# CuzImSlymi/Apertis-LLM

Hardware: AMD Instinct MI355X
Metric: train tokens/sec/node (seq=4096) (higher is better)
Workload: dtype bf16

## Files before the change

apertis_llm_amd/_lib.py:

```python
import ctypes
import os
import threading

_HERE = os.path.dirname(os.path.abspath(__file__))
LIB_PATH = os.environ.get("APERTIS_HIP_LIB") or os.path.join(_HERE, "libapertis_hip.so")

F32, BF16 = 0, 1
ACT_NONE, ACT_GELU, ACT_RELU, ACT_SILU = 0, 1, 2, 3
ACT_SAVE_GRAD, ACT_MUL_SAVED = 0x100, 0x200
ACT_INTERLEAVED = 0x400


class ApertisHipError(RuntimeError):
    pass


_lock = threading.Lock()
_lib = None

_vp, _i64, _i32, _f32, _u64 = ctypes.c_void_p, ctypes.c_int64, ctypes.c_int, ctypes.c_float, ctypes.c_uint64
_f64 = ctypes.c_double

ABI_VERSION = (4 << 16) | 12
SIGNATURES = {
    "apertis_abi_version": (ctypes.c_int, []),
    "apertis_arch": (ctypes.c_char_p, []),
    "apertis_strerror": (ctypes.c_char_p, [_i32]),
    "apertis_scan_chunk_len": (_i64, [_i64, _i64, _i64]),
    "apertis_scan_num_chunks": (_i64, [_i64, _i64, _i64]),
    "apertis_selective_scan_fwd": (_i32, [_vp, _vp, _vp, _i64, _vp, _i64, _vp, _vp, _i64, _vp, _vp, _vp,
                                          _i64, _i64, _i64, _i64, _i32, _i32, _i32, _vp]),
    "apertis_selective_scan_bwd": (_i32, [_vp, _vp, _vp, _i64, _vp, _i64, _vp, _i64, _vp, _vp, _i64, _vp, _i64,
                                          _vp, _vp, _vp, _vp, _vp, _i64, _i64, _i64, _i64, _i32, _i32, _i32, _vp]),
    "apertis_ssm_gate_fwd": (_i32, [_vp, _i64, _vp, _i64, _vp, _i64, _vp, _vp, _i64, _i64, _i64, _i32, _i32, _vp]),
    "apertis_ssm_gate_bwd": (_i32, [_vp, _i64, _vp, _i64, _vp, _i64, _vp, _i64, _vp, _vp, _i64, _vp, _i64, _vp, _i64,
                                    _vp, _vp, _i64, _i64, _i32, _i32, _vp]),
    "apertis_ssm_gate_bwd_blocks": (_i64, [_i64, _i64]),
    "apertis_scan_gate_workspace_bytes": (_i64, [_i64, _i64, _i64]),
    "apertis_scan_gate_chunk_len": (_i64, []),
    "apertis_scan_gate_fwd": (_i32, [_vp, _vp, _vp, _i64, _vp, _i64, _vp, _i64, _vp, _i64, _vp, _vp, _vp, _i64, _vp, _vp, _vp,
                                     _vp, ctypes.c_uint32, _i64, _i64, _i64, _i64, _i32, _i32, _i32, _vp]),
    "apertis_scan_gate_bwd": (_i32, [_vp, _vp, _vp, _i64, _vp, _i64, _vp, _i64, _vp, _i64, _vp, _vp, _i64, _vp, _vp, _i64, _vp,
                                     _i64, _i64, _vp, _i64, _vp, _i64, _vp, _vp, _vp, _vp, _vp, _vp, ctypes.c_uint32, _i64, _i64,
                                     _i64, _i64, _i32, _i32, _i32, _vp]),
    "apertis_scan_lean_fwd": (_i32, [_vp, _vp, _vp, _i64, _vp, _i64, _vp, _i64, _vp, _i64, _vp, _vp, _vp, _i64, _vp, _vp, _vp, _vp,
                                     _i64, _i64, _i64, _i64, _i32, _vp]),
    "apertis_scan_lean_fwd_dt": (_i32, [_vp, _i64, _vp, _vp, _i64, _vp, _vp, _vp, _i64, _vp, _i64, _vp, _i64, _vp, _i64, _vp, _vp, _vp,
                                        _i64, _vp, _vp, _vp, _vp, _i64, _i64, _i64, _i64, _i32, _vp]),
    "apertis_scan_lean_bwd": (_i32, [_vp, _vp, _vp, _i64, _vp, _i64, _vp, _i64, _vp, _i64, _vp, _vp, _i64, _vp, _vp, _i64, _vp, _i64,
                                     _i64, _vp, _i64, _vp, _i64, _vp, _vp, _vp, _vp, _vp, _vp, _i64, _i64, _i64, _i64, _i32, _vp]),
    "apertis_scan_lookback_workspace_bytes": (_i64, [_i64, _i64, _i64]),
    "apertis_scan_lookback_fwd": (_i32, [_vp, _vp, _vp, _i64, _vp, _i64, _vp, _i64, _vp, _i64, _vp, _vp, _vp, _i64, _vp, _vp, _vp, _vp,
                                         ctypes.c_uint32, _i64, _i64, _i64, _i64, _i32, _vp]),
    "apertis_scan_lookback_bwd": (_i32, [_vp, _vp, _vp, _i64, _vp, _i64, _vp, _i64, _vp, _i64, _vp, _vp, _i64, _vp, _vp, _i64, _vp,
                                         _i64, _i64, _vp, _i64, _vp, _i64, _vp, _vp, _vp, _vp, _vp, ctypes.c_uint32, _i64, _i64, _i64,
                                         _i64, _i32, _vp]),
    "apertis_ssm_decode_conv": (_i32, [_vp, _i64, _vp, _vp, _vp, _vp, _vp, _i64, _i64, _i64, _i32, _vp]),
    "apertis_ssm_decode_state": (_i32, [_vp, _vp, _vp, _i64, _vp, _i64, _vp, _vp, _i64, _vp, _vp, _vp, _i64, _i64, _i64, _i32,
                                        _i32, _vp]),
    "apertis_ssm_decode_state_dt": (_i32, [_vp, _i64, _vp, _vp, _i64, _vp, _vp, _i64, _vp, _i64, _vp, _vp, _i64, _vp, _vp, _vp, _i64,
                                           _i64, _i64, _i32, _i32, _vp]),
    "apertis_dropout_add_fwd": (_i32, [_vp, _vp, _vp, _i64, _f32, _u64, _i32, _i32, _vp]),
    "apertis_dropout_bwd": (_i32, [_vp, _vp, _i64, _f32, _u64, _i32, _i32, _vp]),
    "apertis_dwconv_silu_fwd": (_i32, [_vp, _i64, _vp, _vp, _vp, _i64, _i64, _i64, _i64, _i64, _i32, _vp]),
    "apertis_dwconv_silu_bwd": (_i32, [_vp, _i64, _vp, _vp, _vp, _i64, _vp, _i64, _vp, _vp, _vp, _vp, _i64, _i64, _i64,
                                       _i64, _i32, _vp]),
    "apertis_dwconv_silu_bwd2": (_i32, [_vp, _i64, _vp, _vp, _vp, _i64, _vp, _i64, _vp, _i64, _vp, _vp, _vp, _vp, _i64, _i64, _i64,
                                        _i64, _i32, _vp]),
    "apertis_dwconv_bwd_blocks": (_i64, [_i64, _i64, _i64]),
    "apertis_moe_gate_topk_fwd": (_i32, [_vp, _vp, _vp, _vp, _i64, _i64, _i64, _vp]),
    "apertis_decode_pre_conv": (_i32, [_vp, _vp, _vp, _vp, _i64, _i64, _i64, _i64, _i32, _vp]),
    "apertis_decode_pre_state": (_i32, [_vp, _i64, _i64, _i64, _i64, _vp, _vp, _i64, _vp, _vp, _vp, _vp, _vp, _i64, _i64, _i64, _i64,
                                        _i32, _i32, _vp]),
    "apertis_decode_dense_gemv": (_i32, [_vp, _vp, _i64, _vp, _vp, _i64, _i64, _i64, _vp]),
    "apertis_decode_post": (_i32, [_vp, _vp, _i64, _vp, _vp, _i64, _i64, _i64, _i32, _vp]),
    "apertis_decode_inproj": (_i32, [_vp, _vp, _vp, _i64, _vp, _vp, _vp, _f32, _vp, _vp, _vp, _i64, _vp, _vp, _vp, _i64, _vp, _i64, _i64, _i64,
                                     _i64, _vp]),
    "apertis_moe_enter_small": (_i32, [_vp, _vp, _vp, _vp, _f32, _vp, _vp, _vp, _vp, _f32, _vp, _vp, _vp, _vp, _vp, _vp, _vp, _vp, _vp, _vp,
                                       _vp, _vp, _f32, _vp, _vp, _vp, _i64, _i64, _i64, _i64, _i32, _i32, _vp]),
    "apertis_moe_route_small": (_i32, [_vp, _vp, _vp, _vp, _vp, _vp, _vp, _vp, _vp, _vp, _vp, _f32, _vp, _vp, _vp, _i64, _i64, _i64, _i64,
                                       _i32, _i32, _vp]),
    "apertis_moe_gate_topk_bwd": (_i32, [_vp, _vp, _vp, _vp, _vp, _i64, _i64, _i64, _vp]),
    "apertis_skinny_linear_fwd": (_i32, [_vp, _vp, _vp, _vp, _i64, _i64, _i64, _i32, _vp]),
    "apertis_skinny_linear_bwd": (_i32, [_vp, _vp, _vp, _vp, _vp, _vp, _i64, _i64, _i64, _i32, _vp]),
    "apertis_skinny_linear_bwd_blocks": (_i64, [_i64]),
    "apertis_moe_plan_workspace_bytes": (_i64, [_i64, _i64, _i64]),
    "apertis_moe_plan": (_i32, [_vp, _vp, _vp, _i64, _vp, _vp, _vp, _vp, _vp, _i64, _i64, _i64, _vp]),
    "apertis_moe_gather_ln_fwd": (_i32, [_vp, _vp, _vp, _vp, _vp, _f32, _vp, _vp, _vp, _i64, _i64, _i64, _i32, _i32, _vp]),
    "apertis_moe_gather_ln_bwd": (_i32, [_vp, _vp, _vp, _vp, _vp, _vp, _vp, _vp, _vp, _vp, _vp, _vp, _i64, _i64, _i64,
                                         _i32, _i32, _vp]),
    "apertis_moe_gather_ln_bwd_blocks": (_i64, [_i64]),
    "apertis_layernorm_fwd": (_i32, [_vp, _vp, _vp, _f32, _vp, _vp, _vp, _i64, _i64, _i32, _i32, _vp]),
    "apertis_layernorm_bwd": (_i32, [_vp, _vp, _vp, _vp, _vp, _vp, _vp, _vp, _f32, _u64, _vp, _vp, _vp, _i64, _i64, _i32, _i32, _vp]),
    "apertis_layernorm_combine_bwd": (_i32, [_vp, _vp, _vp, _vp, _vp, _vp, _vp, _f32, _u64, _vp, _vp, _vp, _vp, _vp, _vp, _vp, _vp,
                                             _i64, _i64, _i64, _i32, _i32, _vp]),
    "apertis_dropout_add_layernorm_fwd": (_i32, [_vp, _vp, _vp, _i64, _vp, _vp, _vp, _f32, _vp, _vp, _vp, _vp, _i64, _i64, _f32,
                                                 _u64, _i32, _i32, _vp]),
    "apertis_dropout_add_layernorm_router_fwd": (_i32, [_vp, _vp, _vp, _vp, _f32, _vp, _vp, _vp, _vp, _vp, _vp, _f32, _vp, _vp, _vp,
                                                        _vp, _vp, _i64, _i64, _i64, _f32, _u64, _i32, _i32, _vp]),
    "apertis_layernorm_bwd_blocks": (_i64, [_i64, _i64]),
    "apertis_moe_combine_fwd": (_i32, [_vp, _vp, _vp, _vp, _i64, _i64, _i64, _i32, _i32, _i32, _vp]),
    "apertis_moe_combine_bwd": (_i32, [_vp, _vp, _vp, _vp, _vp, _vp, _vp, _vp, _i64, _i64, _i64, _i64, _i64,
                                       _i32, _i32, _vp]),
    "apertis_grouped_gemm_nt": (_i32, [_vp, _vp, _vp, _vp, _vp, _vp, _vp, _i64, _i64, _i64, _i64, _i64, _i32, _f32, _u64,
                                       _i32, _i32, _vp]),
    "apertis_grouped_gemm_nt_saves_grad": (_i32, [_i64, _i64, _i64, _i64, _i64, _i32, _i32, _i32]),
    "apertis_grouped_gemm_nt_q": (_i32, [_vp, _vp, _vp, _vp, _vp, _vp, _vp, _i64, _i64, _i64, _i64, _i64, _i32, _f32, _u64,
                                         _i32, _i32, _vp, _vp]),
    "apertis_grouped_gemm_tn_workspace_bytes": (_i64, [_i64, _i32]),
    "apertis_grouped_gemm_tn_dense_variant": (_i32, [_i64, _i64]),
    "apertis_grouped_gemm_tn_pair": (_i32, [_vp, _vp, _vp, _vp, _i64, _i64, _vp, _vp, _vp, _vp, _i64, _i64, _vp, _i64, _i64,
                                            _vp, _i64, _i32, _vp]),
    "apertis_grouped_gemm_tn_pair_q": (_i32, [_vp, _vp, _vp, _vp, _i64, _i64, _vp, _vp, _vp, _vp, _i64, _i64, _vp, _i64, _i64,
                                              _vp, _i64, _i32, _i32, _vp]),
    "apertis_grouped_gemm_tn_q": (_i32, [_vp, _vp, _vp, _vp, _vp, _i64, _i64, _i64, _i64, _vp, _i64, _i32, _i32, _vp]),
    "apertis_cast_transpose": (_i32, [_vp, _vp, _vp, _i64, _i64, _i64, _i64, _i64, _i32, _vp]),
    "apertis_weight_prep_entry_bytes": (_i64, []),
    "apertis_weight_prep": (_i32, [_vp, _i64, _i64, _vp]),
    "apertis_grouped_gemm_tn": (_i32, [_vp, _vp, _vp, _vp, _vp, _i64, _i64, _i64, _i64, _vp, _i64, _i32, _vp]),
    "apertis_moe_gate_topk_aux_fwd": (_i32, [_vp, _vp, _vp, _vp, _vp, _vp, _vp, _i64, _i64, _i64, _f32, _f32, _vp]),
    "apertis_moe_gate_topk_aux_bwd": (_i32, [_vp, _vp, _vp, _vp, _vp, _vp, _vp, _f32, _f32, _vp, _i64, _i64, _i64, _vp]),
    "apertis_moe_gate_topk_noisy_aux_fwd": (_i32, [_vp, _vp, _f32, _u64, _vp, _vp, _vp, _vp, _vp, _vp, _i64, _i64, _i64, _f32,
                                                   _f32, _vp]),
    "apertis_moe_gate_topk_noisy_aux_bwd": (_i32, [_vp, _vp, _vp, _vp, _vp, _vp, _vp, _f32, _f32, _vp, _f32, _u64, _vp, _vp, _vp,
                                                   _i64, _i64, _i64, _vp]),
    "apertis_moe_gate_aux_blocks": (_i64, [_i64]),
    "apertis_router_fwd": (_i32, [_vp, _vp, _vp, _f32, _vp, _vp, _vp, _vp, _vp, _i64, _i64, _i64, _i32, _vp]),
    "apertis_router_bwd": (_i32, [_vp, _vp, _vp, _vp, _vp, _vp, _vp, _vp, _vp, _vp, _vp, _i64, _i64, _i64, _i32, _vp]),
    "apertis_router_bwd_rows": (_i32, [_vp, _vp, _vp, _vp, _vp, _vp, _vp, _vp, _vp, _vp, _i64, _vp, _vp, _vp, _i64, _i64, _i64,
                                       _i32, _vp]),
    "apertis_router_bwd_blocks": (_i64, [_i64]),
    "apertis_boundary_router_bwd": (_i32, [_vp, _vp, _vp, _vp, _vp, _vp, _vp, _f32, _u64, _vp, _vp, _vp, _vp, _vp, _vp, _vp, _vp, _vp,
                                           _i64, _vp, _vp, _vp, _vp, _i64, _i64, _i64, _i32, _i32, _vp]),
    "apertis_tiny_linear_fwd": (_i32, [_vp, _i64, _vp, _vp, _vp, _i64, _i64, _i64, _i32, _vp]),
    "apertis_tiny_linear_bwd": (_i32, [_vp, _i64, _vp, _vp, _vp, _i64, _vp, _vp, _i64, _i64, _i64, _i32, _vp]),
    "apertis_tiny_linear_bwd_pad": (_i32, [_vp, _i64, _vp, _vp, _vp, _i64, _vp, _vp, _i64, _i64, _i64, _i64, _i32, _vp]),
    "apertis_tiny_linear_bwd_blocks": (_i64, [_i64]),
    "apertis_cross_entropy_fwd": (_i32, [_vp, _vp, _vp, _vp, _i64, _i64, _i64, _i64, _i64, _i64, _i32, _vp]),
    "apertis_cross_entropy_bwd": (_i32, [_vp, _vp, _vp, _vp, _vp, _i64, _i64, _i64, _i64, _i64, _i64, _i32, _vp]),
    "apertis_cross_entropy_fwd_bwd": (_i32, [_vp, _vp, _vp, _vp, _vp, _vp, _i64, _i64, _i64, _i64, _i64, _i64, _i32, _vp]),
    "apertis_colsum_f32": (_i32, [_vp, _vp, _i64, _i64, _vp]),
    "apertis_act_dropout_bwd": (_i32, [_vp, _vp, _vp, _vp, _i64, _i64, _i64, _i32, _f32, _u64, _i32, _vp]),
    "apertis_opt_chunk_elems": (_i64, []),
    "apertis_grad_sumsq": (_i32, [_vp, _vp, _vp, _i64, _vp, _vp]),
    "apertis_clip_coef": (_i32, [_vp, _i64, _f32, _vp, _vp, _vp]),
    "apertis_adamw_step": (_i32, [_vp, _vp, _vp, _i64, _f64, _f64, _f64, _f64, _f64, _i64, _vp, _vp]),
    "apertis_rope_qk_fwd": (_i32, [_vp, _i64, _vp, _i64, _vp, _i64, _vp, _vp, _i64, _vp, _vp, _i64, _i64, _i64, _i32, _vp]),
    "apertis_rope_qk_bwd": (_i32, [_vp, _i64, _vp, _i64, _vp, _i64, _vp, _vp, _i64, _vp, _vp, _i64, _i64, _i64, _i32, _vp]),
    "apertis_attention_fwd": (_i32, [_vp, _i64, _vp, _i64, _vp, _i64, _vp, _vp, _i64, _vp, _i64, _i64, _i64, _i64, _f32, _u64,
                                     _i32, _vp]),
    "apertis_attention_bwd_workspace_bytes": (_i64, [_i64, _i64, _i64]),
    "apertis_attention_bwd": (_i32, [_vp, _i64, _vp, _i64, _vp, _i64, _vp, _i64, _vp, _i64, _vp, _vp, _vp, _vp, _vp, _vp, _i64,
                                     _i64, _i64, _i64, _i64, _f32, _u64, _i32, _vp]),
    "apertis_rope_kv_append": (_i32, [_vp, _i64, _vp, _i64, _vp, _i64, _vp, _vp, _i64, _i64, _vp, _i64, _vp, _i64, _i64, _vp, _i64,
                                      _i64, _i64, _i64, _i64, _i64, _i32, _vp]),
    "apertis_attention_decode_splits": (_i64, [_i64, _i64, _i64, _i64]),
    "apertis_attention_decode_workspace_bytes": (_i64, [_i64, _i64, _i64, _i64]),
    "apertis_attention_decode": (_i32, [_vp, _i64, _vp, _i64, _i64, _vp, _i64, _i64, _i64, _vp, _i64, _vp, _i64, _vp, _i64, _i64,
                                        _i64, _i64, _i64, _i32, _vp]),
    "apertis_rope_kv_append_at": (_i32, [_vp, _i64, _vp, _i64, _vp, _i64, _vp, _vp, _i64, _vp, _i64, _vp, _vp, _i64, _vp, _i64, _i64,
                                         _vp, _i64, _i64, _i64, _i64, _i64, _i32, _vp]),
    "apertis_attention_decode_at": (_i32, [_vp, _i64, _vp, _i64, _i64, _vp, _i64, _i64, _i64, _vp, _vp, _i64, _vp, _i64, _vp, _i64,
                                           _i64, _i64, _i64, _i32, _vp]),
    "apertis_rope_kv_append_chunk": (_i32, [_vp, _i64, _i64, _vp, _i64, _i64, _vp, _i64, _i64, _vp, _vp, _i64, _i64, _vp, _vp, _i64,
                                            _i64, _vp, _i64, _i64, _i64, _i64, _i64, _i64, _i64, _i32, _vp]),
    "apertis_attention_chunk_splits": (_i64, [_i64, _i64, _i64, _i64, _i64]),
    "apertis_attention_chunk_workspace_bytes": (_i64, [_i64, _i64, _i64, _i64, _i64]),
    "apertis_attention_chunk": (_i32, [_vp, _i64, _vp, _i64, _i64, _vp, _i64, _i64, _i64, _vp, _i64, _vp, _i64, _vp, _i64, _i64,
                                       _i64, _i64, _i64, _i64, _i32, _vp]),
    "apertis_token_counts": (_i32, [_vp, _i64, _i64, _i64, _i64, _vp, _vp, _vp]),
    "apertis_sample_next": (_i32, [_vp, _i64, _i32, _i64, _i64, _vp, _f32, _i32, _f32, _i64, _f32, _u64, _vp, _i64, _vp, _vp, _vp,
                                   _i64, _i64, _vp, _vp, _i64, _i64, _vp, _vp, _vp, _vp, _vp]),
}


class _Lib:

    def __init__(self, cdll):
        self._cdll = cdll

    def __getattr__(self, name):
        if name not in SIGNATURES:
            raise AttributeError(name)
        try:
            fn = getattr(self._cdll, name)
        except AttributeError:
            raise ApertisHipError(f"{LIB_PATH} does not export {name}: rebuild with "
                                  "`python -m apertis_llm_amd.build --force`") from None
        fn.restype, fn.argtypes = SIGNATURES[name]
        setattr(self, name, fn)
        return fn


def load():
    global _lib
    if _lib is not None:
        return _lib
    with _lock:
        if _lib is not None:
            return _lib
        if not os.path.exists(LIB_PATH):
            raise ApertisHipError(
                f"{LIB_PATH} not found: build it with `python -m apertis_llm_amd.build` "
                "(hipcc --offload-arch=gfx950). There is no CPU or eager fallback.")
        cdll = ctypes.CDLL(LIB_PATH)
        try:
            got = int(cdll.apertis_abi_version())
        except AttributeError:
            got = -1
        if got != ABI_VERSION:
            raise ApertisHipError(f"{LIB_PATH} has ABI version {got >> 16}.{got & 0xffff} but this binding needs "
                                  f"{ABI_VERSION >> 16}.{ABI_VERSION & 0xffff}: rebuild with `python -m apertis_llm_amd.build --force`")
        _lib = _Lib(cdll)
    return _lib


def check(rc, what):
    if rc != 0:
        msg = load().apertis_strerror(int(rc)).decode()
        raise ApertisHipError(f"{what} failed: {msg} (code {rc})")


def ptr(t):
    return None if t is None else t.data_ptr()


_raw_stream = None


def stream_ptr():
    global _raw_stream
    if _raw_stream is None:
        import torch
        get_dev, get_raw = getattr(torch._C, "_cuda_getDevice", None), getattr(torch._C, "_cuda_getCurrentRawStream", None)
        if get_dev is not None and get_raw is not None:
            _raw_stream = lambda: get_raw(get_dev())
        else:
            _raw_stream = lambda: torch.cuda.current_stream().cuda_stream
    return _raw_stream()


def dtype_code(t):
    import torch
    if t.dtype == torch.float32:
        return F32
    if t.dtype == torch.bfloat16:
        return BF16
    raise ApertisHipError(f"unsupported dtype {t.dtype}: kernels take float32 or bfloat16")
```

apertis_llm_amd/csrc/layernorm.hip:

```cpp
#include "row_common.h"

namespace {

template <typename TX, typename TO, int IT>
__global__ void __launch_bounds__(256)
gather_ln_fwd_k(const TX *__restrict__ x, const int32_t *__restrict__ row_token,
                const int32_t *__restrict__ offsets, const float *__restrict__ gamma,
                const float *__restrict__ beta, float eps, TO *__restrict__ xg,
                float *__restrict__ mean_o, float *__restrict__ rstd_o, int64_t max_rows, int H, int E) {
  if constexpr (IT <= 4) __builtin_assume(H > 256 * (IT - 1));
  const int lane = threadIdx.x & 63;
  const int64_t r = (int64_t)blockIdx.x * 4 + (threadIdx.x >> 6);
  if (r >= max_rows || (offsets && r >= offsets[E])) return;
  const int e = offsets ? expert_of_row(offsets, E, (int)r) : 0;
  const TX *src = x + (row_token ? (int64_t)row_token[r] : r) * H;
  float4 v[IT];
#pragma unroll
  for (int i = 0; i < IT; ++i) {
    int c = (lane + 64 * i) * 4;
    v[i] = c < H ? load4s<TX>(src + c) : make_float4(0.f, 0.f, 0.f, 0.f);
  }
  float mean, rstd;
  row_stats<IT>(v, lane, H, eps, mean, rstd);
  const float *ga = gamma + (int64_t)e * H, *be = beta + (int64_t)e * H;
// ... 511 lines not shown
    g4[i] = c < H ? load4<float>(gamma + c) : make_float4(0, 0, 0, 0);
    b4[i] = c < H ? load4<float>(beta + c) : make_float4(0, 0, 0, 0);
  }
  __syncthreads();
  typedef typename raw4<TX>::type raw_t;
  raw_t cur[IT], nxt[IT];
  auto fetch = [&](raw_t (&o)[IT], int64_t r) {
#pragma unroll
    for (int i = 0; i < IT; ++i) {
      const int c = (lane + 64 * i) * 4;
      o[i] = (c < H && r < T) ? raw_load(x + r * H + c) : raw_t{};
    }
  };
  if (wave < T) fetch(cur, wave);
  for (int64_t r = wave; r < T; r += nw) {
    fetch(nxt, r + nw);
    float4 v[IT];
#pragma unroll
    for (int i = 0; i < IT; ++i) {
      v[i] = raw_to_f4(cur[i]);
    }
    float mean, rstd;
    row_stats<IT>(v, lane, H, eps, mean, rstd);
#pragma unroll
    for (int i = 0; i < IT; ++i) cur[i] = nxt[i];
#pragma unroll
    for (int i = 0; i < IT; ++i)
      v[i] = make_float4((v[i].x - mean) * rstd * g4[i].x + b4[i].x, (v[i].y - mean) * rstd * g4[i].y + b4[i].y,
                         (v[i].z - mean) * rstd * g4[i].z + b4[i].z, (v[i].w - mean) * rstd * g4[i].w + b4[i].w);
    float acc[NN];
#pragma unroll
    for (int n = 0; n < NN; ++n) {
      float a = 0.f;
#pragma unroll
      for (int i = 0; i < IT; ++i) {
        const float4 wn = lane + 64 * i < Q ? sW[n * Q + lane + 64 * i] : make_float4(0, 0, 0, 0);
        a += (v[i].x * wn.x + v[i].y * wn.y) + (v[i].z * wn.z + v[i].w * wn.w);
      }
      acc[n] = wave_sum(a);
    }
    if (lane < NN) {
      float o = 0.f;
#pragma unroll
      for (int n = 0; n < NN; ++n) if (lane == n) o = acc[n];
      logits[r * NN + lane] = o + (b ? b[lane] : 0.f);
    }
    if (lane == 0) { mean_o[r] = mean; rstd_o[r] = rstd; }
  }
}

template <typename TX, typename TO, int IT, int NN>
__global__ void __launch_bounds__(256)
dropadd_ln_router_fwd_k(const TO *__restrict__ blk, const TX *__restrict__ res, const float *__restrict__ gamma,
                        const float *__restrict__ beta, float eps, TX *__restrict__ y, TO *__restrict__ xn,
                        float *__restrict__ mean_o, float *__restrict__ rstd_o, const float *__restrict__ rgamma,
                        const float *__restrict__ rbeta, float reps, const float *__restrict__ W, const float *__restrict__ rb,
                        float *__restrict__ logits, float *__restrict__ rmean_o, float *__restrict__ rrstd_o, int64_t T, int H,
                        float drop_p, uint64_t seed) {
  if constexpr (IT <= 4) __builtin_assume(H > 256 * (IT - 1));
  extern __shared__ __attribute__((aligned(16))) char smem[];
  const int Q = H / 4;
  float4 *sW = reinterpret_cast<float4 *>(smem);
  float4 *sG = sW + NN * Q, *sB = sG + Q, *sRG = sB + Q, *sRB = sRG + Q;
  const int lane = threadIdx.x & 63;
  for (int i = threadIdx.x; i < NN * Q; i += 256) sW[i] = reinterpret_cast<const float4 *>(W)[i];
  for (int i = threadIdx.x; i < Q; i += 256) {
    sG[i] = reinterpret_cast<const float4 *>(gamma)[i]; sB[i] = reinterpret_cast<const float4 *>(beta)[i];
    sRG[i] = reinterpret_cast<const float4 *>(rgamma)[i]; sRB[i] = reinterpret_cast<const float4 *>(rbeta)[i];
  }
  __syncthreads();
  const float ks = drop_p > 0.f ? 1.f / (1.f - drop_p) : 1.f;
  const uint32_t th = (uint32_t)(drop_p * 65536.f);
  typedef typename raw4<TO>::type rawo_t;
  typedef typename raw4<TX>::type rawx_t;
  const int64_t wave = (int64_t)blockIdx.x * 4 + (threadIdx.x >> 6), nw = (int64_t)gridDim.x * 4;
  rawo_t bc[IT], bn[IT];
  rawx_t rc[IT], rn[IT];
  auto fetch = [&](rawo_t (&bo)[IT], rawx_t (&ro)[IT], int64_t r) {
#pragma unroll
    for (int i = 0; i < IT; ++i) {
      const int c = (lane + 64 * i) * 4;
      const bool ok = c < H && r < T;
      bo[i] = ok ? *reinterpret_cast<const rawo_t *>(blk + r * H + c) : rawo_t{};
      ro[i] = ok ? *reinterpret_cast<const rawx_t *>(res + r * H + c) : rawx_t{};
    }
  };
  if (wave < T) fetch(bc, rc, wave);
  for (int64_t r = wave; r < T; r += nw) {
    fetch(bn, rn, r + nw);
    float4 v[IT];
#pragma unroll
    for (int i = 0; i < IT; ++i) {
      const int c = (lane + 64 * i) * 4;
      if (c < H) {
        const float4 a = raw_to_f4(bc[i]), rr = raw_to_f4(rc[i]);
        float e[4] = {a.x, a.y, a.z, a.w};
        if (drop_p > 0.f) {
          bool keep[4];
          drop_keep4(seed, (uint64_t)r * (uint64_t)H + (uint64_t)c, th, keep);
#pragma unroll
          for (int j = 0; j < 4; ++j) e[j] = keep[j] ? e[j] * ks : 0.f;
        }
        v[i] = make_float4(rr.x + e[0], rr.y + e[1], rr.z + e[2], rr.w + e[3]);
        store4<TX>(y + r * H + c, v[i]);
        v[i] = make_float4(to_f32(from_f32<TX>(v[i].x)), to_f32(from_f32<TX>(v[i].y)), to_f32(from_f32<TX>(v[i].z)), to_f32(from_f32<TX>(v[i].w)));
      } else {
        v[i] = make_float4(0.f, 0.f, 0.f, 0.f);
      }
    }
    float mean, rstd;
    row_stats<IT>(v, lane, H, eps, mean, rstd);
#pragma unroll
    for (int i = 0; i < IT; ++i) {
      const int c = (lane + 64 * i) * 4;
      if (c < H) {
        const float4 g4 = sG[lane + 64 * i], b4 = sB[lane + 64 * i];
        const float4 o = make_float4((v[i].x - mean) * rstd * g4.x + b4.x, (v[i].y - mean) * rstd * g4.y + b4.y,
                                     (v[i].z - mean) * rstd * g4.z + b4.z, (v[i].w - mean) * rstd * g4.w + b4.w);
        store4<TO>(xn + r * H + c, o);
        v[i] = make_float4(to_f32(from_f32<TO>(o.x)), to_f32(from_f32<TO>(o.y)), to_f32(from_f32<TO>(o.z)), to_f32(from_f32<TO>(o.w)));
      }
    }
    if (lane == 0) { mean_o[r] = mean; rstd_o[r] = rstd; }
    float rmean, rrstd;
    row_stats<IT>(v, lane, H, reps, rmean, rrstd);
#pragma unroll
    for (int i = 0; i < IT; ++i) {
      const bool in = lane + 64 * i < Q;
      const float4 g4 = in ? sRG[lane + 64 * i] : make_float4(0, 0, 0, 0), b4 = in ? sRB[lane + 64 * i] : make_float4(0, 0, 0, 0);
      v[i] = make_float4((v[i].x - rmean) * rrstd * g4.x + b4.x, (v[i].y - rmean) * rrstd * g4.y + b4.y,
                         (v[i].z - rmean) * rrstd * g4.z + b4.z, (v[i].w - rmean) * rrstd * g4.w + b4.w);
    }
    float acc[NN];
#pragma unroll
    for (int n = 0; n < NN; ++n) {
      float a = 0.f;
#pragma unroll
      for (int i = 0; i < IT; ++i) {
        const float4 wn = lane + 64 * i < Q ? sW[n * Q + lane + 64 * i] : make_float4(0, 0, 0, 0);
        a += (v[i].x * wn.x + v[i].y * wn.y) + (v[i].z * wn.z + v[i].w * wn.w);
      }
      acc[n] = wave_sum(a);
    }
    if (lane < NN) {
      float o = 0.f;
#pragma unroll
      for (int n = 0; n < NN; ++n) if (lane == n) o = acc[n];
      logits[r * NN + lane] = o + (rb ? rb[lane] : 0.f);
    }
    if (lane == 0) { rmean_o[r] = rmean; rrstd_o[r] = rrstd; }
#pragma unroll
    for (int i = 0; i < IT; ++i) { bc[i] = bn[i]; rc[i] = rn[i]; }
  }
}

typedef float v2f __attribute__((ext_vector_type(2)));
__device__ __forceinline__ v2f pk_fma2(v2f a, v2f b, v2f c) { return __builtin_elementwise_fma(a, b, c); }

template <typename TX, int IT, int NN, int MODE>
__global__ void __launch_bounds__(256, MODE == 1 ? 2 : 1)
router_bwd3_k(const TX *__restrict__ x, const float *__restrict__ gamma, const float *__restrict__ beta,
              const float *__restrict__ mean_i, const float *__restrict__ rstd_i, const float *__restrict__ W,
              const float *__restrict__ dlogits, const TX *__restrict__ dres, const TX *__restrict__ grows,
              const int32_t *__restrict__ slot_of, int KS, TX *__restrict__ dx,
              float *__restrict__ part, int64_t T, int H) {
  if constexpr (IT <= 4) __builtin_assume(H > 256 * (IT - 1));
  typedef typename raw4<TX>::type raw_t;
  extern __shared__ __attribute__((aligned(16))) char smem[];
  float4 *sW = reinterpret_cast<float4 *>(smem);
  float4 *red = sW + NN * (H / 4);
  __shared__ float redb[4][SK_MAXN];
  const int lane = threadIdx.x & 63, wv = threadIdx.x >> 6, Q = H / 4;
  for (int i = threadIdx.x; i < NN * Q; i += 256) sW[i] = reinterpret_cast<const float4 *>(W)[i];
  float4 aw[NN][IT], ag[IT], ab[IT], g4[IT], b4[IT];
  float abias = 0.f;
#pragma unroll
  for (int i = 0; i < IT; ++i) {
    const int c = (lane + 64 * i) * 4;
    g4[i] = c < H ? load4<float>(gamma + c) : make_float4(0, 0, 0, 0);
    b4[i] = c < H ? load4<float>(beta + c) : make_float4(0, 0, 0, 0);
    ag[i] = make_float4(0, 0, 0, 0); ab[i] = make_float4(0, 0, 0, 0);
#pragma unroll
    for (int n = 0; n < NN; ++n) aw[n][i] = make_float4(0, 0, 0, 0);
  }
  __syncthreads();
  const int64_t wave = (int64_t)blockIdx.x * 4 + wv, nw = (int64_t)gridDim.x * 4;
  raw_t xc[IT], rc[IT], xn_[IT], rn_[IT];
  raw_t gc[2][IT], gn_[2][IT];
  int sc[2] = {-1, -1}, sn[2] = {-1, -1};
  const bool gath = MODE != 2 && grows != nullptr;
  auto fetch_slots = [&](int64_t r) -> int { return (gath && r < T && lane < KS) ? slot_of[r * KS + lane] : -1; };
  auto slots_of = [&](int v, int (&so)[2]) {
    so[0] = __builtin_amdgcn_readlane(v, 0);
    so[1] = __builtin_amdgcn_readlane(v, 1);
  };
  int slv_n = -1, slv_n2 = -1;
  auto fetch = [&](raw_t (&xo)[IT], raw_t (&ro)[IT], raw_t (&go)[2][IT], const int (&so)[2], int64_t r) {
#pragma unroll
    for (int i = 0; i < IT; ++i) {
      const int c = (lane + 64 * i) * 4;
      const bool ok = c < H && r < T;
      xo[i] = ok ? raw_load(x + r * H + c) : raw_t{};
      ro[i] = (MODE != 2 && ok && dres) ? raw_load(dres + r * H + c) : raw_t{};
#pragma unroll
      for (int k = 0; k < 2; ++k)
        go[k][i] = (gath && ok && so[k] >= 0) ? raw_load(grows + (int64_t)so[k] * H + c) : raw_t{};
    }
  };
  auto fetch_meta = [&](int64_t r) -> float {
    if (r >= T) return 0.f;
    const float *p = lane < NN ? dlogits + r * NN + lane : (lane == NN ? mean_i + r : rstd_i + r);
    return lane < NN + 2 ? *p : 0.f;
  };
  auto lane_val = [](float v, int l) { return __builtin_bit_cast(float, __builtin_amdgcn_readlane(__builtin_bit_cast(int, v), l)); };
  float meta = 0.f, meta_next = 0.f;
  if (wave < T) {
    slots_of(fetch_slots(wave), sc);
    slv_n = fetch_slots(wave + nw);
    fetch(xc, rc, gc, sc, wave);
    meta = fetch_meta(wave);
  }
  for (int64_t r = wave; r < T; r += nw) {
    slv_n2 = fetch_slots(r + 2 * nw);
    slots_of(slv_n, sn);
    fetch(xn_, rn_, gn_, sn, r + nw);
    meta_next = fetch_meta(r + nw);
    float g[NN];
#pragma unroll
    for (int n = 0; n < NN; ++n) g[n] = lane_val(meta, n);
    if (MODE != 1 && lane < NN) abias += meta;
    const float mean = lane_val(meta, NN), rstd = lane_val(meta, NN + 1);
    float4 xh[IT], dn[IT];
    float s1 = 0.f, s2 = 0.f;
#pragma unroll
    for (int i = 0; i < IT; ++i) {
      const bool in = lane + 64 * i < Q;
      const float4 xv = raw_to_f4(xc[i]);
      const v2f mm = {-mean, -mean}, rs = {rstd, rstd};
      v2f xh0 = in ? ((v2f){xv.x, xv.y} + mm) * rs : (v2f){0.f, 0.f}, xh1 = in ? ((v2f){xv.z, xv.w} + mm) * rs : (v2f){0.f, 0.f};
      xh[i] = make_float4(xh0.x, xh0.y, xh1.x, xh1.y);
      const v2f g0 = {g4[i].x, g4[i].y}, g1 = {g4[i].z, g4[i].w};
      const v2f xn0 = pk_fma2(xh0, g0, (v2f){b4[i].x, b4[i].y}), xn1 = pk_fma2(xh1, g1, (v2f){b4[i].z, b4[i].w});
      v2f d0 = {0.f, 0.f}, d1 = {0.f, 0.f};
#pragma unroll
      for (int n = 0; n < NN; ++n) {
        const float4 wn = in ? sW[n * Q + lane + 64 * i] : make_float4(0, 0, 0, 0);
        const v2f gn = {g[n], g[n]};
        if constexpr (MODE != 2) { d0 = pk_fma2(gn, (v2f){wn.x, wn.y}, d0); d1 = pk_fma2(gn, (v2f){wn.z, wn.w}, d1); }
        if constexpr (MODE != 1) {
          v2f a0 = {aw[n][i].x, aw[n][i].y}, a1 = {aw[n][i].z, aw[n][i].w};
          a0 = pk_fma2(gn, xn0, a0); a1 = pk_fma2(gn, xn1, a1);
          aw[n][i] = make_float4(a0.x, a0.y, a1.x, a1.y);
        }
      }
      if constexpr (MODE == 2) continue;
      v2f ag0 = pk_fma2(d0, xh0, (v2f){ag[i].x, ag[i].y}), ag1 = pk_fma2(d1, xh1, (v2f){ag[i].z, ag[i].w});
      ag[i] = make_float4(ag0.x, ag0.y, ag1.x, ag1.y);
      const v2f ab0 = (v2f){ab[i].x, ab[i].y} + d0, ab1 = (v2f){ab[i].z, ab[i].w} + d1;
      ab[i] = make_float4(ab0.x, ab0.y, ab1.x, ab1.y);
      const v2f dn0 = d0 * g0, dn1 = d1 * g1;
      dn[i] = make_float4(dn0.x, dn0.y, dn1.x, dn1.y);
      s1 += (dn[i].x + dn[i].y) + (dn[i].z + dn[i].w);
      s2 += (dn[i].x * xh[i].x + dn[i].y * xh[i].y) + (dn[i].z * xh[i].z + dn[i].w * xh[i].w);
    }
    if constexpr (MODE != 2) {
    const float m1 = wave_sum(s1) * inv_h(H), m2 = wave_sum(s2) * inv_h(H);
#pragma unroll
    for (int i = 0; i < IT; ++i) {
      const int c = (lane + 64 * i) * 4;
      if (c < H) {
        float4 rr = raw_to_f4(rc[i]);
        if (gath) {
          float4 ga = make_float4(0, 0, 0, 0);
#pragma unroll
          for (int k = 0; k < 2; ++k)
            if (sc[k] >= 0) { const float4 gv = raw_to_f4(gc[k][i]); ga.x += gv.x; ga.y += gv.y; ga.z += gv.z; ga.w += gv.w; }
          rr.x += to_f32(from_f32<TX>(ga.x)); rr.y += to_f32(from_f32<TX>(ga.y));
          rr.z += to_f32(from_f32<TX>(ga.z)); rr.w += to_f32(from_f32<TX>(ga.w));
        }
        store4<TX>(dx + r * H + c, make_float4(rstd * (dn[i].x - m1 - xh[i].x * m2) + rr.x, rstd * (dn[i].y - m1 - xh[i].y * m2) + rr.y,
                                                rstd * (dn[i].z - m1 - xh[i].z * m2) + rr.z, rstd * (dn[i].w - m1 - xh[i].w * m2) + rr.w));
      }
    }
    }
#pragma unroll
    for (int i = 0; i < IT; ++i) { xc[i] = xn_[i]; rc[i] = rn_[i]; gc[0][i] = gn_[0][i]; gc[1][i] = gn_[1][i]; }
    sc[0] = sn[0]; sc[1] = sn[1];
    slv_n = slv_n2;
    meta = meta_next;
  }
  if (MODE != 1 && lane < NN) redb[wv][lane] = abias;
  for (int turn = 1; turn < 4; ++turn) {
    __syncthreads();
    if (wv == turn) {
#pragma unroll
      for (int i = 0; i < IT; ++i) {
        const int cq = lane + 64 * i;
        if (cq < Q) {
          if constexpr (MODE != 1) {
#pragma unroll
            for (int n = 0; n < NN; ++n) red[n * Q + cq] = aw[n][i];
          }
          if constexpr (MODE != 2) { red[NN * Q + cq] = ag[i]; red[(NN + 1) * Q + cq] = ab[i]; }
        }
      }
    }
// ... 711 lines not shown
  const size_t lds3 = (size_t)(2 * N + 2) * H * sizeof(float);
  const bool split = N * ((H + 255) / 256) >= 16;
  if (dtype_x == APERTIS_BF16) {
#define ROUTER_BWD(TXT, MODE_) { launch_lds(router_bwd3_k<TXT, IT, NN, MODE_>, grid, block, lds3, st, (const TXT *)x, gamma, beta, mean, rstd, W, dlogits, (const TXT *)dres, (const TXT *)grows, slot_of, (int)KS, (TXT *)dx, part, T, (int)H); }
    SKINNY_N(N, SKINNY_IT(H, { if (split) { ROUTER_BWD(bf16_t, 1) ROUTER_BWD(bf16_t, 2) } else ROUTER_BWD(bf16_t, 0) }));
  } else if (dtype_x == APERTIS_F32) {
    SKINNY_N(N, SKINNY_IT(H, { if (split) { ROUTER_BWD(float, 1) ROUTER_BWD(float, 2) } else ROUTER_BWD(float, 0) }));
#undef ROUTER_BWD
  } else return APERTIS_ERR_ARG;
  const int64_t cols = N * H + N + 2 * H;
  hipLaunchKernelGGL(fold_rows_k, dim3((unsigned)ceil_div64(cols, 64)), dim3(1024), 0, st, part, grads, nblk, cols);
  return apertis_check_launch();
}

extern "C" int apertis_router_bwd(const void *x, const float *gamma, const float *beta, const float *mean, const float *rstd,
                                  const float *W, const float *dlogits, const void *dres, void *dx, float *part,
                                  float *grads, int64_t T, int64_t H, int64_t N, int dtype_x, void *stream) {
  return apertis_router_bwd_rows(x, gamma, beta, mean, rstd, W, dlogits, dres, nullptr, nullptr, 0, dx, part, grads, T, H, N,
                                 dtype_x, stream);
}

extern "C" int apertis_decode_inproj(const void *blk, const int32_t *slot_of, const float *wk, int64_t KK, const float *res,
                                     const float *gamma, const float *beta, float eps, float *y, const void *xn, const void *W,
                                     int64_t ldw, void *xz, const float *pre, void *conv_state, int64_t kconv, void *gated,
                                     int64_t S, int64_t H, int64_t N, int64_t Dn, void *stream) {
  if (!W) return APERTIS_ERR_ARG;
  if (xn ? false : (!blk || !res || !gamma || !beta || !y || (slot_of && (!wk || KK < 1)))) return APERTIS_ERR_ARG;
  if (pre ? (!conv_state || !gated || N != 2 * Dn || Dn < 1) : !xz) return APERTIS_ERR_ARG;
  if (S < 1 || S > 16 || H < 512 || H % 8 || H > 1024 || N < 4 || N % 4 || ldw < H || ldw % 8) return APERTIS_ERR_UNSUPPORTED;
  if (pre && (kconv < 2 || kconv > 16)) return APERTIS_ERR_UNSUPPORTED;
  hipStream_t st = (hipStream_t)stream;
  dim3 grid((unsigned)ceil_div64(N, 16)), block(256);
#define DL_GO(LN_) { launch_lds(decode_ln_inproj_k<IT, LN_>, grid, block, (LN_) ? (size_t)S * H * 2 : (size_t)0, st, (const bf16_t *)blk, \
                                        slot_of, wk, (int)KK, res, gamma, beta, eps, y, (const bf16_t *)xn, (const bf16_t *)W, (int)ldw, \
                                        (bf16_t *)xz, pre, (bf16_t *)conv_state, (int)kconv, (bf16_t *)gated, (int)Dn, (int)S, (int)H, (int)N); }
  if (xn) { SKINNY_IT(H, DL_GO(false)); }
  else { SKINNY_IT(H, DL_GO(true)); }
#undef DL_GO
  return apertis_check_launch();
}

extern "C" int apertis_moe_enter_small(const void *blk, const void *res, const float *gamma, const float *beta, float eps, void *y,
                                       void *xn, const float *rgamma, const float *rbeta, float reps, const float *W,
                                       const float *rb, float *logits, float *gates, int32_t *idx, float *w,
                                       int32_t *expert_offsets, int32_t *row_token, int32_t *row_k, int32_t *slot_of,
                                       const float *lgamma, const float *lbeta, float leps, void *xg, float *mean, float *rstd,
                                       int64_t S, int64_t H, int64_t E, int64_t K, int dtype_x, int dtype_y, void *stream) {
  if (!blk || !res || !gamma || !beta || !y || !rgamma || !rbeta || !W || !logits || !gates || !idx || !w || !expert_offsets ||
      !row_token || !row_k || !slot_of || !lgamma || !lbeta || !xg || !mean || !rstd)
    return APERTIS_ERR_ARG;
  if (S < 1 || S > 16 || (E != 4 && E != 8) || K < 1 || K > E || E * K > 16) return APERTIS_ERR_UNSUPPORTED;
  if (H <= 0 || H % 4 || H > 1024) return APERTIS_ERR_UNSUPPORTED;
  if (dtype_x != APERTIS_F32 || (dtype_y != APERTIS_BF16 && dtype_y != APERTIS_F32)) return APERTIS_ERR_UNSUPPORTED;
  hipStream_t st = (hipStream_t)stream;
  dim3 grid(1), block(64 * (unsigned)(E * K));
  const size_t lds = (size_t)(3 * E + 4) * H * sizeof(float) + (size_t)S * H * (dtype_y == APERTIS_BF16 ? 2 : 4);
  if (lds + 4096 > 160 * 1024) return APERTIS_ERR_UNSUPPORTED;
#define ES_GO(TOT, NN_) { launch_lds(moe_enter_small_k<float, TOT, IT, NN_>, grid, block, lds, st, (const TOT *)blk, (const float *)res, gamma, beta, eps, (float *)y, (TOT *)xn, rgamma, rbeta, \
                       reps, W, rb, logits, gates, idx, w, expert_offsets, row_token, row_k, slot_of, lgamma, lbeta, leps, (TOT *)xg, \
                       mean, rstd, (int)S, (int)K, (int)H); }
  if (dtype_y == APERTIS_BF16) { SKINNY_IT(H, { if (E == 4) ES_GO(bf16_t, 4) else ES_GO(bf16_t, 8) }); }
  else { SKINNY_IT(H, { if (E == 4) ES_GO(float, 4) else ES_GO(float, 8) }); }
#undef ES_GO
  return apertis_check_launch();
}

extern "C" int apertis_moe_route_small(const float *logits, float *gates, int32_t *idx, float *w, int32_t *expert_offsets,
                                       int32_t *row_token, int32_t *row_k, int32_t *slot_of, const void *x, const float *gamma,
                                       const float *beta, float eps, void *xg, float *mean, float *rstd, int64_t S, int64_t H,
                                       int64_t E, int64_t K, int dtype_x, int dtype_xg, void *stream) {
  if (!logits || !gates || !idx || !w || !expert_offsets || !row_token || !row_k || !slot_of || !x || !gamma || !beta || !xg ||
      !mean || !rstd || S < 0)
    return APERTIS_ERR_ARG;
  if (S < 1 || S > 64 || (E != 4 && E != 8 && E != 16) || K < 1 || K > E || K > MAXK || E * K > 16) return APERTIS_ERR_UNSUPPORTED;
  if (check_H(H) || H > 1024) return APERTIS_ERR_UNSUPPORTED;
  hipStream_t st = (hipStream_t)stream;
  dim3 grid(1), block(64 * (unsigned)(E * K));
#define RS_GO(EC_) hipLaunchKernelGGL((moe_route_small_k<TA, TB, IT, EC_>), grid, block, 0, st, logits, gates, idx, w, expert_offsets, \
                                      row_token, row_k, slot_of, (const TA *)x, gamma, beta, eps, (TB *)xg, mean, rstd, (int)S, (int)E, \
                                      (int)K, (int)H)
  DISPATCH_2T(dtype_x, dtype_xg, SKINNY_IT(H, { if (E == 4) RS_GO(4); else if (E == 8) RS_GO(8); else RS_GO(16); }));
#undef RS_GO
  return apertis_check_launch();
}

extern "C" int apertis_boundary_router_bwd(const void *y, const float *gamma, const float *mean, const float *rstd, const void *dres,
                                           void *dx, void *dblk, float drop_p, uint64_t seed, const void *xn, const float *rgamma,
                                           const float *rbeta, const float *rmean, const float *rrstd, const float *W,
                                           const float *dlogits, const void *grows, const int32_t *slot_of, int64_t KS,
                                           float *part, float *rgrads, float *dgamma, float *dbeta, int64_t T, int64_t H,
                                           int64_t N, int dtype_x, int dtype_g, void *stream) {
  if (!y || !gamma || !mean || !rstd || !dx || !dblk || !xn || !rgamma || !rbeta || !rmean || !rrstd || !W || !dlogits || !part ||
      !rgrads || !dgamma || !dbeta || T < 0)
    return APERTIS_ERR_ARG;
  if (drop_p < 0.f || drop_p >= 1.f) return APERTIS_ERR_ARG;
  if (grows && (!slot_of || KS < 1)) return APERTIS_ERR_ARG;
  if (grows && KS > 2) return APERTIS_ERR_UNSUPPORTED;
  if (H <= 0 || H % 4 || H > 1024 || N < 1 || N > 8) return APERTIS_ERR_UNSUPPORTED;
  if (dtype_x != APERTIS_F32 || (dtype_g != APERTIS_BF16 && dtype_g != APERTIS_F32)) return APERTIS_ERR_UNSUPPORTED;
  hipStream_t st = (hipStream_t)stream;
  const int64_t nblk = apertis_router_bwd_blocks(T), cols = N * H + N + 2 * H;
  float *part_ln = part + nblk * cols;
  dim3 grid((unsigned)nblk), block(256);
  const size_t ldsf = (size_t)(N + 2 + 8 + 2) * H * sizeof(float), lds3 = (size_t)(2 * N + 2) * H * sizeof(float);
#define BR_BWD(TGT) { \
    launch_lds(boundary_router_bwd_k<float, TGT, IT, NN>, grid, block, ldsf, st, (const float *)y, gamma, mean, rstd, (const float *)dres, (float *)dx, (TGT *)dblk, drop_p, seed, \
                       (const TGT *)xn, rgamma, rbeta, rmean, rrstd, W, dlogits, (const TGT *)grows, slot_of, (int)KS, part, part_ln, T, (int)H); \
    launch_lds(router_bwd3_k<TGT, IT, NN, 2>, grid, block, lds3, st, (const TGT *)xn, rgamma, rbeta, rmean, rrstd, W, dlogits, (const TGT *)nullptr, \
                       (const TGT *)nullptr, (const int32_t *)nullptr, 0, (TGT *)nullptr, part, T, (int)H); }
  if (dtype_g == APERTIS_BF16) { SKINNY_N(N, SKINNY_IT(H, BR_BWD(bf16_t))); }
  else { SKINNY_N(N, SKINNY_IT(H, BR_BWD(float))); }
#undef BR_BWD
  hipLaunchKernelGGL(fold_rows_k, dim3((unsigned)ceil_div64(cols, 64)), dim3(1024), 0, st, part, rgrads, nblk, cols);
  ln_fold(part_ln, nblk, H, false, dgamma, dbeta, st);
  return apertis_check_launch();
}

extern "C" int apertis_dropout_add_layernorm_fwd(const void *blk, const int32_t *slot_of, const float *wk, int64_t K,
                                                 const void *res, const float *gamma, const float *beta, float eps, void *y,
                                                 void *xn, float *mean, float *rstd, int64_t T, int64_t H, float drop_p,
                                                 uint64_t seed, int dtype_x, int dtype_y, void *stream) {
  if (!blk || !res || !gamma || !beta || !y || !xn || !mean || !rstd || T < 0 || drop_p < 0.f || drop_p >= 1.f)
    return APERTIS_ERR_ARG;
  if (slot_of && (!wk || K < 1 || K > MAXK)) return APERTIS_ERR_ARG;
  if (check_H(H)) return APERTIS_ERR_UNSUPPORTED;
  if (T == 0) return APERTIS_OK;
  hipStream_t st = (hipStream_t)stream;
  dim3 grid((unsigned)ceil_div64(T, 4)), block(256);
  DISPATCH_2T(dtype_x, dtype_y, DISPATCH_IT(H, hipLaunchKernelGGL((dropadd_ln_fwd_k<TA, TB, IT>), grid, block, 0, st,
      (const TB *)blk, slot_of, wk, (int)K, (const TA *)res, gamma, beta, eps, (TA *)y, (TB *)xn, mean, rstd, T, (int)H, drop_p,
      seed)));
  return apertis_check_launch();
}

extern "C" int apertis_dropout_add_layernorm_router_fwd(const void *blk, const void *res, const float *gamma, const float *beta,
                                                        float eps, void *y, void *xn, float *mean, float *rstd,
                                                        const float *rgamma, const float *rbeta, float reps, const float *W,
                                                        const float *rb, float *logits, float *rmean, float *rrstd, int64_t T,
                                                        int64_t H, int64_t N, float drop_p, uint64_t seed, int dtype_x,
                                                        int dtype_y, void *stream) {
  if (!blk || !res || !gamma || !beta || !y || !xn || !mean || !rstd || !rgamma || !rbeta || !W || !logits || !rmean || !rrstd ||
      T < 0 || drop_p < 0.f || drop_p >= 1.f)
    return APERTIS_ERR_ARG;
  if (H <= 0 || H % 4 || H > 1024 || (N != 2 && N != 4 && N != 8)) return APERTIS_ERR_UNSUPPORTED;
  if (T == 0) return APERTIS_OK;
  hipStream_t st = (hipStream_t)stream;
  const size_t lds = (size_t)(N + 4) * H * sizeof(float);
  dim3 grid((unsigned)std::min<int64_t>(ceil_div64(T, 4), 1024)), block(256);
#define BR_GO(NN_) { launch_lds(dropadd_ln_router_fwd_k<TA, TB, IT, NN_>, grid, block, lds, st, (const TB *)blk, (const TA *)res, gamma, beta, eps, (TA *)y, (TB *)xn, mean, rstd, rgamma, rbeta, reps, W, rb, logits, rmean, rrstd, T, (int)H, drop_p, seed); }
  DISPATCH_2T(dtype_x, dtype_y, SKINNY_IT(H, { if (N == 2) BR_GO(2) else if (N == 4) BR_GO(4) else BR_GO(8) }));
#undef BR_GO
  return apertis_check_launch();
}
```

apertis_llm_amd/model.py:

```python
import functools
import inspect
import json
import logging
import math
import os
from pathlib import Path
from typing import Any, Dict, List, Optional, Tuple, Union

import torch
import torch.nn as nn
import torch.nn.functional as F

from . import ops
from .multimodal import UnifiedMultimodalEncoder

logger = logging.getLogger(__name__)


def _on_input_device(fn):
    @functools.wraps(fn)
    def wrapper(self, *args, **kwargs):
        t = next((a for a in (*args, *kwargs.values()) if isinstance(a, torch.Tensor)), None)
        if t is None or not t.is_cuda or t.device.index == torch.cuda.current_device():
            return fn(self, *args, **kwargs)
        with ops.device_guard(t):
            return fn(self, *args, **kwargs)
    return wrapper


class ApertisConfig:

    def __init__(self, vocab_size: int = 32000, hidden_size: int = 768, num_hidden_layers: int = 12,
                 num_attention_heads: int = 12, intermediate_size: int = 3072, hidden_act: str = "gelu",
                 hidden_dropout_prob: float = 0.1, attention_probs_dropout_prob: float = 0.1,
                 max_position_embeddings: int = 2048, type_vocab_size: int = 2, initializer_range: float = 0.02,
                 layer_norm_eps: float = 1e-12, pad_token_id: int = 0, bos_token_id: int = 1, eos_token_id: int = 2,
                 unk_token_id: int = 3, position_embedding_type: str = "rotary", use_cache: bool = True,
                 classifier_dropout: float = None, model_type: str = "apertis", tie_word_embeddings: bool = True,
                 rope_theta: float = 10000.0, sliding_window: Optional[int] = None,
                 attention_type: str = "standard_mha", ssm_d_inner: Optional[int] = None, ssm_d_state: int = 16,
                 ssm_dt_rank: Union[int, str] = "auto", ssm_conv_kernel: int = 4, use_flash_attention: bool = False,
                 use_expert_system: bool = False, num_experts: int = 8, experts_per_token: int = 2,
                 multimodal: bool = False, image_size: int = 224, vision_embed_dim: int = 768,
                 vision_patch_size: int = 16, vision_layers: int = 12, vision_heads: int = 12,
                 output_attentions: bool = False, output_hidden_states: bool = False,
                 load_balancing_loss_coef: float = 0.01, expert_capacity_factor: float = 1.25,
                 noisy_routing_alpha: float = 0.1, expert_dropout_prob: float = 0.1,
                 router_z_loss_coef: float = 0.001, expert_output_gating: bool = False,
                 use_noisy_top_k_routing: bool = True, use_expert_capacity_limit: bool = True,
                 use_expert_dropout: bool = True, use_router_z_loss: bool = True,
                 use_load_balancing_loss: bool = True, use_rmsnorm: bool = False, use_swiglu: bool = False,
                 **kwargs):
        given = dict(locals())
        for name in ("vocab_size", "hidden_size", "num_hidden_layers", "num_attention_heads", "hidden_act",
                     "intermediate_size", "hidden_dropout_prob", "attention_probs_dropout_prob",
                     "max_position_embeddings", "type_vocab_size", "initializer_range", "layer_norm_eps",
                     "pad_token_id", "bos_token_id", "eos_token_id", "unk_token_id", "position_embedding_type",
                     "use_cache", "classifier_dropout", "model_type", "tie_word_embeddings", "rope_theta",
                     "sliding_window", "attention_type", "ssm_d_state"):
            setattr(self, name, given[name])
        derived = num_attention_heads * ssm_d_state
        if attention_type == "selective_ssm":
            if ssm_d_inner is not None and ssm_d_inner != derived:
                logger.warning("ssm_d_inner=%s overridden by num_attention_heads*ssm_d_state=%s", ssm_d_inner, derived)
            self.ssm_d_inner = derived
        else:
            self.ssm_d_inner = 2 * hidden_size if ssm_d_inner is None else ssm_d_inner
        self.ssm_dt_rank = math.ceil(hidden_size / 16) if ssm_dt_rank == "auto" else int(ssm_dt_rank)
        for name in ("ssm_conv_kernel", "use_flash_attention", "use_expert_system", "num_experts",
                     "experts_per_token", "multimodal", "image_size", "vision_embed_dim", "vision_patch_size",
                     "vision_layers", "vision_heads", "output_attentions", "output_hidden_states",
                     "load_balancing_loss_coef", "expert_capacity_factor", "noisy_routing_alpha",
                     "expert_dropout_prob", "router_z_loss_coef", "expert_output_gating", "use_noisy_top_k_routing",
                     "use_expert_capacity_limit", "use_expert_dropout", "use_router_z_loss",
                     "use_load_balancing_loss", "use_rmsnorm", "use_swiglu"):
            setattr(self, name, given[name])
        if not use_expert_system:
            self.num_experts = 0
            self.experts_per_token = 0
        else:
            self.experts_per_token = min(num_experts, experts_per_token) if num_experts > 0 else 0
        for key, value in kwargs.items():
            if not hasattr(self, key):
                logger.warning("Ignoring unknown config parameter: %s=%s", key, value)

    @classmethod
    def from_dict(cls, config_dict: Dict[str, Any]):
        params = inspect.signature(cls.__init__).parameters
        keep = {k: v for k, v in config_dict.items() if (k in params and k != "self") or k == "kwargs"}
        if keep.get("ssm_dt_rank") == "auto":
            keep["ssm_dt_rank"] = math.ceil(keep.get("hidden_size", 768) / 16)
        return cls(**keep)

    def to_dict(self) -> Dict[str, Any]:
        return self.__dict__

    @classmethod
    def from_pretrained(cls, model_name_or_path: str):
        if os.path.isfile(model_name_or_path) and model_name_or_path.endswith(".json"):
            path = model_name_or_path
        else:
            path = os.path.join(model_name_or_path, "config.json")
            if not os.path.exists(path) and os.path.isdir(model_name_or_path):
                parent = os.path.join(Path(model_name_or_path).parent, "config.json")
                if os.path.exists(parent):
                    path = parent
        if not os.path.exists(path):
            raise FileNotFoundError(f"Config file not found. Looked for: '{path}' based on input '{model_name_or_path}'")
        with open(path, "r", encoding="utf-8") as f:
            return cls.from_dict(json.load(f))

    def save_pretrained(self, save_directory: str):
        os.makedirs(save_directory, exist_ok=True)
        with open(os.path.join(save_directory, "config.json"), "w", encoding="utf-8") as f:
            json.dump(self.to_dict(), f, indent=2)


def _activation_module(name: str) -> nn.Module:
    if name == "relu":
        return nn.ReLU()
    if name in ("silu", "swish"):
        return nn.SiLU()
    if name != "gelu":
        logger.warning("Unsupported activation %s; using GELU", name)
    return nn.GELU()


def _activation_name(name: str) -> str:
    return name if name in ("gelu", "relu", "silu", "swish") else "gelu"


def _compute_dtype(t: torch.Tensor) -> torch.dtype:
    if torch.is_autocast_enabled():
        dt = torch.get_autocast_dtype("cuda")
        return torch.bfloat16 if dt in (torch.bfloat16, torch.float16) else dt
    return t.dtype if t.dtype in (torch.float32, torch.bfloat16) else torch.float32


class HipLayerNorm(nn.LayerNorm):

    def forward(self, x):
        H = x.shape[-1]
        if x.is_cuda and H % 4 == 0 and H <= 4096 and x.dtype in (torch.float32, torch.bfloat16):
            return ops.layer_norm(x, self.weight, self.bias, self.eps, out_dtype=_compute_dtype(x))
        return super().forward(x)

    def forward_pass(self, x):
        H = x.shape[-1]
        if x.is_cuda and H % 4 == 0 and H <= 4096 and x.dtype in (torch.float32, torch.bfloat16):
            return ops.layer_norm_pass(x, self.weight, self.bias, self.eps, out_dtype=_compute_dtype(x))
        return self.forward(x), x


def _norm_pass(norm, x):
    return norm.forward_pass(x) if isinstance(norm, HipLayerNorm) else (norm(x), x)


class _LazyCombine:
    __slots__ = ("yr", "w", "plan", "shape", "dtype")

    def __init__(self, yr, w, plan, shape, dtype):
        self.yr, self.w, self.plan, self.shape, self.dtype = yr, w, plan, shape, dtype

    def materialise(self):
        return ops.moe_combine(self.yr, self.w, self.plan, out_dtype=self.dtype).reshape(self.shape)


class _StackedPast(list):

    def __init__(self, conv_all, state_all, heads, d_state):
        NL, B = conv_all.shape[0], conv_all.shape[1]
        super().__init__((conv_all[l], state_all[l].view(B, heads, d_state)) for l in range(NL))
        self.conv_all, self.state_all = conv_all, state_all
        self._offs = None

    def offsets(self, NL, B):
        if self._offs is None:
            self._offs = (torch.arange(NL + 1, device=self.conv_all.device, dtype=torch.int32) * B).contiguous()
        return self._offs


class _Pending:
    __slots__ = ("out", "res", "drop")

    def __init__(self, out, res, drop):
        self.out, self.res, self.drop = out, res, drop

    def resolve(self):
        out = self.out.materialise() if isinstance(self.out, _LazyCombine) else self.out
        return _dropout_add(self.drop, out, self.res)


def _enter_block(norm, h, router=None):
    if isinstance(h, _Pending):
        out, res = h.out, h.res
        H = res.shape[-1]
        cd = _compute_dtype(res)
        lazy = out if isinstance(out, _LazyCombine) else None
        if (isinstance(norm, HipLayerNorm) and res.is_cuda and tuple(out.shape) == tuple(res.shape) and H % 4 == 0 and
                H <= 4096 and res.dtype in (torch.float32, torch.bfloat16) and
                (res.dtype == torch.float32 or cd == res.dtype) and (lazy is None or lazy.dtype == lazy.yr.dtype == cd)):
            if (router is not None and lazy is None and isinstance(router[0], nn.LayerNorm) and H <= 1024 and
                    router[1].weight.shape[0] in (2, 4, 8) and cd in (torch.float32, torch.bfloat16)):
                rn, rl = router
                y, xn, logits = ops.dropout_add_layer_norm_router(out, res, norm.weight, norm.bias, norm.eps, h.drop.p,
                                                                  h.drop.training, rn.weight, rn.bias, rn.eps, rl.weight,
                                                                  rl.bias, out_dtype=cd)
                xn._apertis_router_logits = logits
                return xn, y
            if lazy is not None:
                y, xn = ops.dropout_add_layer_norm(lazy.yr, res, norm.weight, norm.bias, norm.eps, h.drop.p,
                                                   h.drop.training, out_dtype=cd, combine=(lazy.w, lazy.plan))
            else:
                y, xn = ops.dropout_add_layer_norm(out, res, norm.weight, norm.bias, norm.eps, h.drop.p,
                                                   h.drop.training, out_dtype=cd)
            return xn, y
        h = h.resolve()
    return _norm_pass(norm, h)


def _dropout_add(drop: nn.Dropout, out, residual):
    if out.is_cuda and out.numel() % 4 == 0 and out.shape == residual.shape and \
            out.dtype in (torch.float32, torch.bfloat16) and residual.dtype in (torch.float32, torch.bfloat16) and \
            (residual.dtype == torch.float32 or out.dtype == residual.dtype):
        return ops.dropout_add(out, residual, drop.p, drop.training)
    return drop(out) + residual


DECODE_GRAPH = os.environ.get("APERTIS_DECODE_GRAPH", "1") == "1"
DECODE_GRAPH_MIN_STEPS = 24
DECODE_PREPASS = os.environ.get("APERTIS_DECODE_PREPASS", "1") == "1"


def _mfma_linear(x, weight, bias=None):
    K = weight.shape[1]
    if x.is_cuda and K % 8 == 0 and weight.shape[0] % 8 == 0:
        return ops.linear_mfma(x, weight, bias, compute_dtype=_compute_dtype(x))
    if getattr(weight, "_apertis_prep", None) is not None:
        raise ops.ApertisHipError(f"prepared-weight placeholder {tuple(weight.shape)} on the stock linear path")
    return F.linear(x, weight, bias)


class RMSNorm(nn.Module):

    def __init__(self, hidden_size: int, eps: float = 1e-6):
        super().__init__()
        self.hidden_size, self.eps = hidden_size, eps
        self.scale = nn.Parameter(torch.ones(hidden_size))

    def forward(self, x):
        rms = x.norm(p=2, dim=-1, keepdim=True) * (self.hidden_size ** -0.5)
        return self.scale * (x / (rms + self.eps))


class RotaryEmbedding(nn.Module):

    def __init__(self, dim: int, max_position_embeddings: int = 2048, base: float = 10000):
        super().__init__()
        if dim % 2:
            raise ValueError(f"RoPE dimension must be even, got {dim}")
        self.dim, self.max_position_embeddings, self.base = dim, max_position_embeddings, base
        inv = 1.0 / (base ** (torch.arange(0, dim, 2, dtype=torch.float32) / dim))
        ang = torch.outer(torch.arange(max_position_embeddings, dtype=torch.float32), inv)
        self.register_buffer("inv_freq", inv, persistent=False)
        self.register_buffer("cos_cached", ang.cos(), persistent=False)
        self.register_buffer("sin_cached", ang.sin(), persistent=False)

    def forward(self, x, position_ids=None):
        B, L, _ = x.shape
        if position_ids is None:
            position_ids = torch.arange(L, device=x.device).unsqueeze(0)
        cos, sin = self.cos_cached[position_ids], self.sin_cached[position_ids]
        pairs = x.float().reshape(B, L, -1, 2)
        a, b = pairs[..., 0], pairs[..., 1]
        return torch.stack((a * cos - b * sin, a * sin + b * cos), dim=-1).reshape(B, L, self.dim).type_as(x)


class SelectiveLinearAttention(nn.Module):

    def __init__(self, config: ApertisConfig):
        super().__init__()
        self.hidden_size = config.hidden_size
        self.num_heads = config.num_attention_heads
        self.d_state = config.ssm_d_state
        self.d_inner = self.num_heads * self.d_state
        self.dt_rank = config.ssm_dt_rank
        self.conv_kernel_size = config.ssm_conv_kernel
        self.in_proj_x = nn.Linear(self.hidden_size, self.d_inner, bias=False)
        self.in_proj_z = nn.Linear(self.hidden_size, self.d_inner, bias=False)
        self.conv1d = nn.Conv1d(self.d_inner, self.d_inner, self.conv_kernel_size, groups=self.d_inner,
                                padding=self.conv_kernel_size - 1)
        self.x_param_proj = nn.Linear(self.d_inner, self.dt_rank + 2 * self.d_inner, bias=False)
        self.dt_proj_head = nn.Linear(self.dt_rank, self.num_heads, bias=True)
        nn.init.uniform_(self.dt_proj_head.bias, a=math.log(1e-3), b=math.log(1e-2))
        self.A_log = nn.Parameter(torch.empty(self.num_heads, self.d_state).uniform_(math.log(0.5), math.log(0.99)))
        self.D = nn.Parameter(torch.ones(self.d_inner))
        self.out_proj = nn.Linear(self.d_inner, self.hidden_size, bias=False)
        self.use_cache = False
        self._pad_idx = None
        self._inplace_cache = False
        self._decode_pre = None

    def _pad_index(self, device):
        Dn, R = self.d_inner, self.dt_rank
        Wb = -(-Dn // 64) * 64
        idx = self._pad_idx
        if idx is None or idx.device != device:
            i = torch.arange(R + 2 * Dn)
            dst = torch.where(i < R, 2 * Wb + i, torch.where(i < R + Dn, i - R, Wb + i - R - Dn))
            idx = self._pad_idx = dst.to(device)
        return idx

    def register_train_prep(self, prep):
        Dn, R = self.d_inner, self.dt_rank
        Wb, Wr = -(-Dn // 64) * 64, -(-R // 64) * 64
        prep.add_stack(("in_proj_xz", id(self)), (self.in_proj_x.weight, self.in_proj_z.weight))
        prep.add_rowmap(("x_param_padded", id(self)), self.x_param_proj.weight, self._pad_index(self.x_param_proj.weight.device),
                        2 * Wb + Wr)
        prep.add_plain(self.out_proj.weight)

    def _padded_param_weight(self):
        w, Dn, R = self.x_param_proj.weight, self.d_inner, self.dt_rank
        Wb, Wr = -(-Dn // 64) * 64, -(-R // 64) * 64
        if w.is_cuda:
            return ops.scatter_rows(w, self._pad_index(w.device), 2 * Wb + Wr), Wb, Wr
        zb = w.new_zeros(Wb - Dn, Dn)
        zr = w.new_zeros(Wr - R, Dn)
        return torch.cat([w[R:R + Dn], zb, w[R + Dn:], zb, w[:R], zr], dim=0), Wb, Wr

    def _stacked_in_proj(self):
        w_xz = ops.prepared_weight(("in_proj_xz", id(self)), (self.in_proj_x.weight, self.in_proj_z.weight))
        if w_xz is None:
            w_xz = ops.cached_prep("in_proj_xz", (self.in_proj_x.weight, self.in_proj_z.weight),
                                   lambda: torch.cat([self.in_proj_x.weight, self.in_proj_z.weight], dim=0))
        return w_xz

    def decode_finish(self, gated, past_key_value):
        self._decode_pre = None
        B = gated.shape[0]
        out = ops.decode_dense_gemv(gated, self.out_proj.weight, self.out_proj.bias)
        if out is None:
            out = _mfma_linear(gated.reshape(B, 1, self.d_inner), self.out_proj.weight, self.out_proj.bias)
        return out.reshape(B, 1, -1), None, tuple(past_key_value)

    @_on_input_device
    def forward(self, hidden_states, attention_mask=None, position_ids=None, past_key_value=None,
                output_attentions: bool = False, use_cache: bool = False):
        self.use_cache = use_cache
        B, L, _ = hidden_states.shape
        Dn, R, kw = self.d_inner, self.dt_rank, self.conv_kernel_size
        conv_prev = ssm_prev = None
        if past_key_value is not None:
            conv_prev, ssm_prev = past_key_value
        have_window = (conv_prev is not None and use_cache and conv_prev.shape[1] == Dn and conv_prev.shape[2] == kw - 1)
        if (self._decode_pre is not None and L == 1 and have_window and hidden_states.is_cuda and hidden_states.dtype == torch.bfloat16
                and not torch.is_grad_enabled() and not output_attentions):
            gated = ops.decode_inproj(self._stacked_in_proj(), self._decode_pre, conv_prev, xn=hidden_states)
            if gated is not None:
                return self.decode_finish(gated, past_key_value)
        xz = _mfma_linear(hidden_states, self._stacked_in_proj())
        if self._decode_pre is not None and not (L == 1 and have_window and ssm_prev is not None and not output_attentions
                                                  and not torch.is_grad_enabled() and hidden_states.is_cuda and kw > 1):
            self._decode_pre = None
            raise ops.ApertisHipError("SelectiveLinearAttention: the model ran this step's cache-only half ahead (_decode_prepass: the "
                                      "SSM state is already updated) but the layer is not on its single-token path")
        Wb, Wr = -(-Dn // 64) * 64, -(-R // 64) * 64
        wp = ops.prepared_weight(("x_param_padded", id(self)), (self.x_param_proj.weight,))
        if wp is None:
            wp, Wb, Wr = ops.cached_prep("x_param_padded", (self.x_param_proj.weight,), self._padded_param_weight)
        if (L == 1 and have_window and ssm_prev is not None and not output_attentions and not torch.is_grad_enabled()
                and hidden_states.is_cuda and kw > 1):
            xz2 = xz.reshape(B, 2 * Dn)
            pre, self._decode_pre = self._decode_pre, None
            if pre is not None:
                gated = ops.decode_post(pre, xz2, conv_prev)
                out = _mfma_linear(gated.reshape(B, 1, Dn), self.out_proj.weight, self.out_proj.bias)
                return out, None, (conv_prev, ssm_prev)
            xc, conv_state = ops.ssm_decode_step(xz2[:, :Dn], conv_prev, self.conv1d.weight, self.conv1d.bias,
                                                 inplace=self._inplace_cache)
            p = _mfma_linear(xc, wp)
            dt_in = p[:, 2 * Wb:2 * Wb + R]
            state = ssm_prev.reshape(B, Dn).float()
            if not (self._inplace_cache and state.data_ptr() == ssm_prev.data_ptr()):
                state = state.clone()
            if ops.tiny_linear_supported(dt_in, R, self.num_heads):
                gated = ops.ssm_decode_state_dt(dt_in, self.dt_proj_head.weight, self.dt_proj_head.bias, self.A_log, p[:, :Dn],
                                                p[:, Wb:Wb + Dn], xc, xz2[:, Dn:], self.D, state)
            else:
                dt_logits = self.dt_proj_head(dt_in).float()
                gated = ops.ssm_decode_state(dt_logits, self.A_log, p[:, :Dn], p[:, Wb:Wb + Dn], xc, xz2[:, Dn:], self.D, state)
            out = _mfma_linear(gated.reshape(B, 1, Dn), self.out_proj.weight)
            return out, None, (conv_state, state.reshape(B, self.num_heads, self.d_state))
        xp, z = ops.split_cols(xz, (Dn, Dn))
        conv_in = xp
        if have_window:
            conv_in = torch.cat([conv_prev.transpose(1, 2).to(xp.dtype), xp], dim=1)
        conv_state = conv_in[:, -(kw - 1):].transpose(1, 2).detach() if use_cache else None
        if hidden_states.is_cuda and ops.DWCONV_PAIR:
            xc_p, xc = ops.dwconv_silu_pair(conv_in, self.conv1d.weight, self.conv1d.bias)
        else:
            xc_p = xc = ops.dwconv_silu(conv_in, self.conv1d.weight, self.conv1d.bias)
        if have_window:
            xc_p, xc = xc_p[:, :L], xc[:, :L]
        p = _mfma_linear(xc_p, wp)
        Btp, Cp, dt_in = ops.split_cols(p, (Wb, Wb, R, Wr - R))[:3]
        h0 = ssm_prev.reshape(B, Dn) if (use_cache and ssm_prev is not None) else None
        two_op = output_attentions or not hidden_states.is_cuda
        tiny = ops.tiny_linear_supported(dt_in, R, self.num_heads)
        if tiny and not two_op:
            res = ops.scan_gate_dt(dt_in, self.dt_proj_head.weight, self.dt_proj_head.bias, self.A_log, Btp, Cp, xc, z, self.D,
                                   h0=h0, delta_softplus=True, return_last=use_cache)
            (gated, h_last), y = (res if use_cache else (res, None)), None
            out = _mfma_linear(gated, self.out_proj.weight)
            cache = (conv_state, h_last.reshape(B, self.num_heads, self.d_state)) if use_cache else None
            return out, None, cache
        if tiny:
            dt_logits = ops.tiny_linear(dt_in, self.dt_proj_head.weight, self.dt_proj_head.bias)
        else:
            dt_logits = self.dt_proj_head(dt_in).float()
        if two_op:
            res = ops.selective_scan(dt_logits, self.A_log, Btp[..., :Dn], Cp[..., :Dn], h0=h0,
                                     delta_softplus=True, y_dtype=torch.float32, return_last=use_cache)
            y, h_last = res if use_cache else (res, None)
            gated = ops.ssm_gate(y, xc, z, self.D)
        else:
            res = ops.scan_gate(dt_logits, self.A_log, Btp, Cp, xc, z, self.D, h0=h0, delta_softplus=True,
                                return_last=use_cache)
            (gated, h_last), y = (res if use_cache else (res, None)), None
        out = _mfma_linear(gated, self.out_proj.weight)
        cache = (conv_state, h_last.reshape(B, self.num_heads, self.d_state)) if use_cache else None
        return out, (y if output_attentions else None), cache


_ZERO_SCALARS = {}


def _zero_scalar(device, dtype):
    key = (device, dtype)
    z = _ZERO_SCALARS.get(key)
    if z is None:
        z = _ZERO_SCALARS[key] = torch.zeros((), device=device, dtype=dtype)
    return z


class AdaptiveExpertSystem(nn.Module):

    _STACKED = (("0.weight", "expert_ln_weight"), ("0.bias", "expert_ln_bias"), ("1.weight", "expert_w1"),
                ("1.bias", "expert_b1"), ("4.weight", "expert_w2"), ("4.bias", "expert_b2"))

    def register_train_prep(self, prep):
        prep.add_plain(self.expert_w1)
        prep.add_plain(self.expert_w2)

    def __init__(self, config: ApertisConfig, activation_function_override: Optional[str] = None):
        super().__init__()
        self.config = config
        self.hidden_size = config.hidden_size
        self.intermediate_size = config.intermediate_size
        self.num_experts = config.num_experts
        self.experts_per_token = config.experts_per_token
        self.load_balancing_loss_coef = config.load_balancing_loss_coef if self.num_experts > 0 else 0.0
        self.expert_capacity_factor = config.expert_capacity_factor
        self.router_z_loss_coef = config.router_z_loss_coef if self.num_experts > 0 else 0.0
        self.noisy_routing_alpha = config.noisy_routing_alpha if self.num_experts > 0 else 0.0
        self.expert_dropout_prob = config.expert_dropout_prob if self.num_experts > 0 else 0.0
        on = self.num_experts > 0
        self.use_noisy_top_k_routing = config.use_noisy_top_k_routing and on
        self.use_expert_capacity_limit = config.use_expert_capacity_limit and on
        self.use_expert_dropout = config.use_expert_dropout and on
        self.use_router_z_loss = config.use_router_z_loss and on
        self.use_load_balancing_loss = config.use_load_balancing_loss and on
        self.router = self.experts = self.w_noise = None
        if not on:
            return
        E, H, I = self.num_experts, self.hidden_size, self.intermediate_size
        self.activation = _activation_name(activation_function_override or config.hidden_act)
        self.hidden_dropout_prob = config.hidden_dropout_prob
        self.router_norm = HipLayerNorm(H, eps=config.layer_norm_eps)
        self.router = nn.Linear(H, E)
        self.experts = True
        k1, k2 = 1.0 / math.sqrt(H), 1.0 / math.sqrt(I)
        self.expert_ln_weight = nn.Parameter(torch.ones(E, H))
        self.expert_ln_bias = nn.Parameter(torch.zeros(E, H))
        self.expert_w1 = nn.Parameter(torch.empty(E, I, H).uniform_(-k1, k1))
        self.expert_b1 = nn.Parameter(torch.empty(E, I).uniform_(-k1, k1))
        self.expert_w2 = nn.Parameter(torch.empty(E, H, I).uniform_(-k2, k2))
        self.expert_b2 = nn.Parameter(torch.empty(E, H).uniform_(-k2, k2))
        if config.use_noisy_top_k_routing:
            self.w_noise = nn.Parameter(torch.zeros(E))
        self._register_state_dict_hook(self._split_experts)
        self._register_load_state_dict_pre_hook(self._stack_experts)

    @staticmethod
    def _split_experts(module, state_dict, prefix, local_metadata):
        for suffix, name in module._STACKED:
            stacked = state_dict.pop(prefix + name)
            for e in range(module.num_experts):
                state_dict[f"{prefix}experts.{e}.{suffix}"] = stacked[e]
        return state_dict

    def _stack_experts(self, state_dict, prefix, *args):
        for suffix, name in self._STACKED:
            keys = [f"{prefix}experts.{e}.{suffix}" for e in range(self.num_experts)]
            if all(k in state_dict for k in keys):
                state_dict[prefix + name] = torch.stack([state_dict.pop(k) for k in keys])

    def init_expert_weights(self, std: float):
        with torch.no_grad():
            self.expert_w1.normal_(0.0, std)
            self.expert_w2.normal_(0.0, std)
            self.expert_b1.zero_()
            self.expert_b2.zero_()
            self.expert_ln_weight.fill_(1.0)
            self.expert_ln_bias.zero_()

    @_on_input_device
    def forward(self, hidden_states, lazy_combine=False, aux_dtype=None):
        aux_dtype = aux_dtype or hidden_states.dtype
        if self.num_experts <= 0 or self.router is None:
            zero = _zero_scalar(hidden_states.device, aux_dtype)
            return hidden_states, zero, zero
        B, L, H = hidden_states.shape
        S, E, K = B * L, self.num_experts, self.experts_per_token
        xf = hidden_states.reshape(S, H)
        pre_logits = getattr(hidden_states, "_apertis_router_logits", None)
        if pre_logits is not None:
            logits = pre_logits.reshape(S, E)
            xf._apertis_rows_link = getattr(hidden_states, "_apertis_rows_link", None)
        elif ops.router_ln_linear_supported(xf, H, E):
            logits, xf = ops.router_ln_linear(xf, self.router_norm.weight, self.router_norm.bias, self.router_norm.eps,
                                              self.router.weight, self.router.bias)
        else:
            xn = self.router_norm(xf)
            if xn.is_cuda and ops.skinny_linear_supported(H, E):
                logits = ops.skinny_linear(xn, self.router.weight, self.router.bias)
            else:
                logits = self.router(xn).float()
        lb_loss = rz_loss = None
        lb_coef = self.load_balancing_loss_coef if (self.use_load_balancing_loss and self.training) else 0.0
        rz_coef = self.router_z_loss_coef if (self.use_router_z_loss and self.training) else 0.0
        noisy = self.use_noisy_top_k_routing and self.training
        cd = _compute_dtype(xf)
        if (not self.training and lb_coef == 0 and rz_coef == 0 and not noisy and logits.is_cuda
                and ops.moe_route_small_supported(logits, xf, K)):
            _g, idx, w, plan, xg = ops.moe_route_small(logits, xf, self.expert_ln_weight, self.expert_ln_bias,
                                                       self.config.layer_norm_eps, K, out_dtype=cd)
            yr = ops.expert_mlp(xg, self.expert_w1, self.expert_b1, self.expert_w2, self.expert_b2, plan.offsets,
                                plan.max_rows, act=self.activation, drop_p=0.0, seed=0, compute_dtype=cd)
            out = _LazyCombine(yr, w, plan, (B, L, H), xf.dtype)
            if not lazy_combine:
                out = out.materialise()
            zero = _zero_scalar(hidden_states.device, aux_dtype)
            return out, zero, zero
        fused_gate = logits.is_cuda and S > 0 and (lb_coef > 0 or rz_coef > 0)
        if noisy and not fused_gate:
            logits = logits + torch.randn_like(logits) * (F.softplus(self.w_noise) * self.noisy_routing_alpha)
        if fused_gate:
            nseed = int(torch.empty((), dtype=torch.int64).random_().item()) if noisy else 0
            idx, w, lb, rz = ops.moe_gate_topk_aux(logits, K, lb_coef, rz_coef, self.w_noise if noisy else None,
                                                   self.noisy_routing_alpha, nseed)
            lb_loss = lb if lb_coef > 0 else None
            rz_loss = rz if rz_coef > 0 else None
        else:
            gates, idx, w = ops.moe_gate_topk(logits, K)
            if lb_coef > 0:
                frac = torch.zeros(E, device=xf.device).index_add_(0, idx.reshape(-1).long(),
                                                                   torch.ones(S * K, device=xf.device)) / S
                lb_loss = lb_coef * E * torch.sum(frac * gates.mean(dim=0))
            if rz_coef > 0:
                rz_loss = rz_coef * torch.mean(torch.logsumexp(logits, dim=-1) ** 2)
        capacity = None
        if self.use_expert_capacity_limit and self.training:
            capacity = max(1, math.floor((S / E) * self.expert_capacity_factor)) if S > 0 else 0
        active = None
        if self.use_expert_dropout and self.training and self.expert_dropout_prob > 0:
            n_drop = min(math.floor(E * self.expert_dropout_prob), E - 1)
            if n_drop > 0:
                active = torch.ones(E, dtype=torch.bool)
                active[torch.randperm(E)[:n_drop]] = False
                active = active.to(xf.device)
        cd = _compute_dtype(xf)
        plan = ops.moe_plan(idx, w, E, capacity, active)
        xg = ops.moe_gather_ln(xf, self.expert_ln_weight, self.expert_ln_bias, plan, self.config.layer_norm_eps,
                               out_dtype=cd)
        p_drop = self.hidden_dropout_prob if self.training else 0.0
        seed = int(torch.empty((), dtype=torch.int64).random_().item()) if p_drop > 0 else 0
        yr = ops.expert_mlp(xg, self.expert_w1, self.expert_b1, self.expert_w2, self.expert_b2, plan.offsets,
                            plan.max_rows, act=self.activation, drop_p=p_drop, seed=seed,
                            compute_dtype=cd)
        out = _LazyCombine(yr, w, plan, (B, L, H), xf.dtype)
        if not lazy_combine:
            out = out.materialise()
        if lb_loss is None or rz_loss is None:
            zero = _zero_scalar(hidden_states.device, aux_dtype)
            lb_loss = zero if lb_loss is None else lb_loss
            rz_loss = zero if rz_loss is None else rz_loss
        return out, lb_loss.to(aux_dtype), rz_loss.to(aux_dtype)


class StateTrackingRecurrentCell(nn.Module):

    def __init__(self, hidden_size: int):
        super().__init__()
        raise NotImplementedError("StateTrackingRecurrentCell is dead code in the reference and is not part of "
                                  "the MI355X hot path")


class ApertisAttention(nn.Module):
    def __init__(self, config: ApertisConfig):
        super().__init__()
        self.config = config
        self.hidden_size = config.hidden_size
        self.num_attention_heads = config.num_attention_heads
        self.attention_head_size = self.hidden_size // self.num_attention_heads
        if config.attention_type in ("selective_ssm", "selective_linear"):
            self.attention_mechanism_impl = SelectiveLinearAttention(config)
            self._ssm = True
        else:
            if config.attention_type != "standard_mha":
                logger.error("Unsupported attention_type '%s'; using 'standard_mha'", config.attention_type)
                config.attention_type = "standard_mha"
            bias = config.attention_probs_dropout_prob == 0.0
            self.q_proj = nn.Linear(self.hidden_size, self.hidden_size, bias=bias)
            self.k_proj = nn.Linear(self.hidden_size, self.hidden_size, bias=bias)
            self.v_proj = nn.Linear(self.hidden_size, self.hidden_size, bias=bias)
            self.out_proj = nn.Linear(self.hidden_size, self.hidden_size, bias=bias)
            self.attention_mechanism_impl = None
            self._ssm = False
        norm = RMSNorm if config.use_rmsnorm else HipLayerNorm
        self.pre_norm = norm(config.hidden_size, eps=config.layer_norm_eps)
        self.output_dropout = nn.Dropout(config.hidden_dropout_prob)
        self.attention_dropout = nn.Dropout(config.attention_probs_dropout_prob)
        self.rope = None
        if config.position_embedding_type == "rotary" and not self._ssm:
            self.rope = RotaryEmbedding(config.hidden_size, config.max_position_embeddings, config.rope_theta)

    def _decode_entry(self, h, past_kv, use_c, output_att):
        impl = self.attention_mechanism_impl
        if (impl._decode_pre is None or not isinstance(h, _Pending) or past_kv is None or not use_c or output_att
                or not isinstance(self.pre_norm, HipLayerNorm) or torch.is_grad_enabled() or self.training):
            return None
        out, res = h.out, h.res
        if res.shape[1] != 1 or not res.is_cuda:
            return None
        lazy = out if isinstance(out, _LazyCombine) else None
        conv_prev = past_kv[0]
        if lazy is not None:
            if not (lazy.yr.dtype == torch.bfloat16 == lazy.dtype):
                return None
            bnd = (lazy.yr, res, self.pre_norm.weight, self.pre_norm.bias, self.pre_norm.eps, (lazy.w, lazy.plan))
        elif isinstance(out, torch.Tensor) and tuple(out.shape) == tuple(res.shape) and out.dtype == torch.bfloat16:
            bnd = (out, res, self.pre_norm.weight, self.pre_norm.bias, self.pre_norm.eps, None)
        else:
            return None
        if res.shape[0] > 4 or conv_prev.dim() != 3:
            return None
        r = ops.decode_inproj(impl._stacked_in_proj(), impl._decode_pre, conv_prev, boundary=bnd)
        if r is None:
            return None
        y, gated = r
        return y, impl.decode_finish(gated, past_kv)

    def _fused_ok(self, q, att_mask, past_kv, output_att):
        if not (ops.ATTN_FUSED and q.is_cuda and past_kv is None and not output_att
                and ops.attention_supported(q, self.num_attention_heads)):
            return False
        if att_mask is None:
            return True
        if not isinstance(att_mask, _AttnMask):
            return False
        kv = att_mask.key_valid
        return att_mask.fused_ok and (kv is None or tuple(kv.shape) == tuple(q.shape[:2]))

    def _fused_attention(self, q, k, v, att_mask, pos_ids, use_c):
        key_valid, default_pos = (att_mask.key_valid, att_mask.default_pos) if att_mask is not None else (None, False)
        if self.rope is not None:
            q, k = ops.rope_qk(q, k, None if default_pos else pos_ids, self.rope.cos_cached, self.rope.sin_cached)
        cache = (k, v) if use_c else None
        ctxv = ops.causal_attention(q, k, v, self.num_attention_heads, key_valid, self.attention_dropout.p, self.training)
        return self.out_proj(ctxv), cache

    def _decode_ok(self, q, att_mask, past_kv, output_att, use_c):
        step = isinstance(past_kv, ops.KVLayer) and past_kv.cache.step_active
        ok = (isinstance(past_kv, ops.KVLayer) and ops.ATTN_FUSED and ops.ATTN_DECODE_FUSED and q.is_cuda
              and q.shape[1] == 1 and use_c and not output_att and not self.training and not torch.is_grad_enabled()
              and isinstance(att_mask, _AttnMask) and att_mask.decode_ok
              and (att_mask.step_cache is past_kv.cache if step else att_mask.pos_host is not None)
              and ops.attention_decode_supported(q, self.num_attention_heads))
        if step:
            cache = past_kv.cache
            if not (ok and q.dtype == cache.dtype and q.shape[0] == cache.k[0].shape[0]):
                raise ops.ApertisHipError("a KVCache whose device step state is active takes single-token inference steps on the "
                                          "decode kernels only (its host lengths are stale): KVCache.step_state_end() first")
            return True
        if not ok:
            return False
        cache, kv = past_kv.cache, att_mask.key_valid
        n = cache.lengths[past_kv.layer]
        return (q.dtype == cache.dtype and n < cache.capacity and q.shape[0] == cache.k[0].shape[0]
                and (kv is None or tuple(kv.shape) == (q.shape[0], n + 1)))

    def _decode_attention(self, q, k, v, att_mask, past_kv):
        cache, layer = past_kv.cache, past_kv.layer
        cos, sin = (self.rope.cos_cached, self.rope.sin_cached) if self.rope is not None else (None, None)
        if cache.step_active:
            q = ops.kv_append_rope_at(q, k, v, cache, layer, cos, sin)
            ctxv = ops.attention_decode_at(q, cache, layer, self.num_attention_heads)
        else:
            q = ops.kv_append_rope(q, k, v, cache, layer, att_mask.pos_host, cos, sin)
            ctxv = ops.attention_decode(q, cache, layer, self.num_attention_heads, att_mask.key_valid)
        return self.out_proj(ctxv.unsqueeze(1)), cache

    def _chunk_ok(self, q, att_mask, past_kv, output_att, use_c):
        if not (isinstance(past_kv, ops.KVLayer) and past_kv.cache.multi_token and not past_kv.cache.step_active
                and ops.ATTN_FUSED and ops.ATTN_DECODE_FUSED and q.is_cuda and q.shape[1] > 1 and use_c and not output_att
                and not self.training and not torch.is_grad_enabled()
                and isinstance(att_mask, _AttnMask) and att_mask.decode_ok and att_mask.pos_host is not None
                and ops.attention_decode_supported(q, self.num_attention_heads)):
            return False
        cache, kv = past_kv.cache, att_mask.key_valid
        n = cache.lengths[past_kv.layer]
        return (q.dtype == cache.dtype and n + q.shape[1] <= cache.capacity and q.shape[0] == cache.k[0].shape[0]
                and att_mask.pos_host == n and (kv is None or tuple(kv.shape) == (q.shape[0], n + q.shape[1])))

    def _chunk_attention(self, q, k, v, att_mask, past_kv):
        cache, layer = past_kv.cache, past_kv.layer
        cos, sin = (self.rope.cos_cached, self.rope.sin_cached) if self.rope is not None else (None, None)
        q = ops.kv_append_rope_chunk(q, k, v, cache, layer, att_mask.pos_host, cos, sin)
        ctxv = ops.attention_chunk(q, cache, layer, self.num_attention_heads, att_mask.key_valid)
        return self.out_proj(ctxv), cache

    def _heads(self, t):
        B, L, _ = t.shape
        return t.view(B, L, self.num_attention_heads, self.attention_head_size).transpose(1, 2)

    def forward(self, hidden_s, att_mask=None, pos_ids=None, past_kv=None, output_att=False, use_c=False, defer=False):
        fused = self._decode_entry(hidden_s, past_kv, use_c, output_att) if self._ssm else None
        if fused is not None:
            hidden_s, (out, proxy, cache) = fused
        else:
            x, hidden_s = _enter_block(self.pre_norm, hidden_s)
        if fused is not None:
            pass
        elif self._ssm:
            out, proxy, cache = self.attention_mechanism_impl(x, attention_mask=att_mask, position_ids=pos_ids,
                                                              past_key_value=past_kv, output_attentions=output_att,
                                                              use_cache=use_c)
        elif self._decode_ok(q := self.q_proj(x), att_mask, past_kv, output_att, use_c):
            out, cache = self._decode_attention(q, self.k_proj(x), self.v_proj(x), att_mask, past_kv)
            proxy = None
        elif self._chunk_ok(q, att_mask, past_kv, output_att, use_c):
            out, cache = self._chunk_attention(q, self.k_proj(x), self.v_proj(x), att_mask, past_kv)
            proxy = None
        elif self._fused_ok(q, att_mask, past_kv, output_att):
            out, cache = self._fused_attention(q, self.k_proj(x), self.v_proj(x), att_mask, pos_ids, use_c)
            proxy = None
        else:
            if isinstance(att_mask, _AttnMask):
                att_mask = att_mask.additive()
            k, v = self.k_proj(x), self.v_proj(x)
            if self.rope is not None:
                q, k = self.rope(q, pos_ids), self.rope(k, pos_ids)
            if use_c and past_kv is not None:
                k, v = torch.cat([past_kv[0], k], dim=1), torch.cat([past_kv[1], v], dim=1)
            cache = (k, v) if use_c else None
            qh, kh, vh = self._heads(q), self._heads(k), self._heads(v)
            Lq, Lk = qh.shape[2], kh.shape[2]
            if att_mask is None and Lq > 1:
                i = torch.arange(Lq, device=x.device).unsqueeze(1) + (Lk - Lq)
                att_mask = torch.zeros(Lq, Lk, device=x.device, dtype=qh.dtype).masked_fill_(
                    i < torch.arange(Lk, device=x.device).unsqueeze(0), torch.finfo(qh.dtype).min)
            if output_att:
                scores = qh @ kh.transpose(-1, -2) / math.sqrt(self.attention_head_size)
                probs = F.softmax(scores + att_mask if att_mask is not None else scores, dim=-1)
                proxy = probs
                ctxv = self.attention_dropout(probs) @ vh
            else:
                proxy = None
                ctxv = F.scaled_dot_product_attention(qh, kh, vh, attn_mask=att_mask,
                                                      dropout_p=self.attention_dropout.p if self.training else 0.0)
            out = self.out_proj(ctxv.transpose(1, 2).reshape(x.shape[0], Lq, self.hidden_size))
        if defer:
            return _Pending(out, hidden_s, self.output_dropout), proxy, cache
        return _dropout_add(self.output_dropout, out, hidden_s), proxy, cache


class SwiGLUFFN(nn.Module):

    def __init__(self, config: ApertisConfig, intermediate_size: Optional[int] = None):
        super().__init__()
        self.config = config
        self.hidden_size = config.hidden_size
        self.intermediate_size = intermediate_size if intermediate_size is not None else config.intermediate_size
        self.ffn_dim = max(256, -(-int(self.intermediate_size * 2 / 3) // 256) * 256)
        self.w_gate = nn.Linear(self.hidden_size, self.ffn_dim, bias=False)
        self.w_up = nn.Linear(self.hidden_size, self.ffn_dim, bias=False)
        self.w_down = nn.Linear(self.ffn_dim, self.hidden_size, bias=False)
        self.dropout = nn.Dropout(config.hidden_dropout_prob)

    def forward(self, x):
        return self.dropout(self.w_down(F.silu(self.w_gate(x)) * self.w_up(x)))


class ApertisFeedForward(nn.Module):
    def __init__(self, config: ApertisConfig):
        super().__init__()
        self.config = config
        norm = RMSNorm if config.use_rmsnorm else HipLayerNorm
        self.pre_norm = norm(config.hidden_size, eps=config.layer_norm_eps)
        self.is_expert_system = False
        if config.use_swiglu:
            self.ffn = SwiGLUFFN(config)
        elif config.use_expert_system and config.num_experts > 0:
            self.ffn = AdaptiveExpertSystem(config, activation_function_override=config.hidden_act)
            self.is_expert_system = True
        else:
            self.ffn = nn.Sequential(nn.Linear(config.hidden_size, config.intermediate_size),
                                     _activation_module(config.hidden_act), nn.Dropout(config.hidden_dropout_prob),
                                     nn.Linear(config.intermediate_size, config.hidden_size))
        self.output_dropout = nn.Dropout(config.hidden_dropout_prob)

    def register_train_prep(self, prep):
        if isinstance(self.ffn, nn.Sequential):
            prep.add_plain(self.ffn[0].weight)
            prep.add_plain(self.ffn[3].weight)

    def _dense_ffn(self, x):
        if isinstance(self.ffn, nn.Sequential) and x.is_cuda and x.dtype in (torch.float32, torch.bfloat16):
            lin1, _act, drop, lin2 = self.ffn
            H = x.shape[-1]
            xf = x.reshape(-1, H)
            T = xf.shape[0]
            if T >= 1 and lin1.bias is not None and lin2.bias is not None:
                cd = _compute_dtype(xf)
                p_drop = drop.p if self.training else 0.0
                seed = int(torch.empty((), dtype=torch.int64).random_().item()) if p_drop > 0 else 0
                out = ops.expert_mlp(xf.to(cd), lin1.weight.unsqueeze(0), lin1.bias.unsqueeze(0), lin2.weight.unsqueeze(0),
                                     lin2.bias.unsqueeze(0), ops.dense_offsets(T, xf.device), T,
                                     act=_activation_name(self.config.hidden_act), drop_p=p_drop, seed=seed, compute_dtype=cd)
                return out.reshape(*x.shape[:-1], lin2.weight.shape[0])
        return self.ffn(x)

    def forward(self, hidden_s, defer=False):
        router = None
        if self.is_expert_system and self.ffn.router is not None and self.ffn.num_experts > 0:
            router = (self.ffn.router_norm, self.ffn.router)
            small = self._small_entry(hidden_s, defer)
            if small is not None:
                return small
        x, hidden_s = _enter_block(self.pre_norm, hidden_s, router=router)
        if self.is_expert_system:
            out, lb, rz = self.ffn(x, lazy_combine=defer and not os.environ.get("APERTIS_NO_LAZY_COMBINE"),
                                   aux_dtype=hidden_s.dtype)
        else:
            out = self._dense_ffn(x)
            lb = rz = _zero_scalar(hidden_s.device, hidden_s.dtype)
        if defer:
            return _Pending(out, hidden_s, self.output_dropout), lb, rz
        return _dropout_add(self.output_dropout, out, hidden_s), lb, rz


def _ffn_small_entry(self, h, defer):
    f = self.ffn
    if not (isinstance(h, _Pending) and not isinstance(h.out, _LazyCombine) and not self.training and not f.training
            and isinstance(self.pre_norm, HipLayerNorm) and isinstance(f.router_norm, nn.LayerNorm)
            and h.res.is_cuda and _compute_dtype(h.res) == h.out.dtype
            and ops.moe_enter_small_supported(h.out, h.res, f.num_experts, f.experts_per_token)):
        return None
    B, L, H = h.res.shape
    cd = h.out.dtype
    y, _logits, w, plan, xg = ops.moe_enter_small(h.out, h.res, self.pre_norm.weight, self.pre_norm.bias, self.pre_norm.eps,
                                                  f.router_norm.weight, f.router_norm.bias, f.router_norm.eps, f.router.weight,
                                                  f.router.bias, f.expert_ln_weight, f.expert_ln_bias, f.config.layer_norm_eps,
                                                  f.experts_per_token)
    yr = ops.expert_mlp(xg, f.expert_w1, f.expert_b1, f.expert_w2, f.expert_b2, plan.offsets, plan.max_rows, act=f.activation,
                        drop_p=0.0, seed=0, compute_dtype=cd)
    out = _LazyCombine(yr, w, plan, (B, L, H), cd)
    zero = _zero_scalar(y.device, y.dtype)
    if defer and not os.environ.get("APERTIS_NO_LAZY_COMBINE"):
        return _Pending(out, y, self.output_dropout), zero, zero
    out = out.materialise()
    if defer:
        return _Pending(out, y, self.output_dropout), zero, zero
    return _dropout_add(self.output_dropout, out, y), zero, zero


ApertisFeedForward._small_entry = _ffn_small_entry


class _AttnMask:
    __slots__ = ("key_valid", "fused_ok", "default_pos", "_make", "_additive", "decode_ok", "pos_host", "step_cache")

    def __init__(self, key_valid, fused_ok, default_pos, make_additive, decode_ok=False, pos_host=None, step_cache=None):
        self.key_valid, self.fused_ok, self.default_pos = key_valid, fused_ok, default_pos
        self._make, self._additive = make_additive, None
        self.decode_ok, self.pos_host, self.step_cache = decode_ok, pos_host, step_cache

    def additive(self):
        if self._make is not None:
            self._additive, self._make = self._make(), None
        return self._additive


class ApertisLayer(nn.Module):
    def __init__(self, config: ApertisConfig):
        super().__init__()
        self.config = config
        self.attention = ApertisAttention(config)
        self.feed_forward = ApertisFeedForward(config)

    def forward(self, hidden_s, att_mask=None, pos_ids=None, past_kv=None, output_att=False, use_c=False, defer=False):
        x, att_w, cache = self.attention(hidden_s, att_mask, pos_ids, past_kv, output_att, use_c, defer=True)
        x, lb, rz = self.feed_forward(x, defer=defer)
        return x, att_w, cache, lb, rz


class ApertisModel(nn.Module):
    def __init__(self, config: ApertisConfig):
        super().__init__()
        self.config = config
        self.padding_idx = config.pad_token_id
        self.vocab_size = config.vocab_size
        self.token_embeddings = nn.Embedding(config.vocab_size, config.hidden_size, self.padding_idx)
        self.abs_pos_embeddings = None
        if config.position_embedding_type == "absolute":
            self.abs_pos_embeddings = nn.Embedding(config.max_position_embeddings, config.hidden_size)
        self.multimodal_encoder = None
        self.vision_projection = nn.Identity()
        if config.multimodal:
            self.multimodal_encoder = UnifiedMultimodalEncoder(config)
            if config.vision_embed_dim != config.hidden_size:
                self.vision_projection = nn.Linear(config.vision_embed_dim, config.hidden_size)
        self.layers = nn.ModuleList([ApertisLayer(config) for _ in range(config.num_hidden_layers)])
        norm = RMSNorm if config.use_rmsnorm else HipLayerNorm
        self.final_post_norm = norm(config.hidden_size, eps=config.layer_norm_eps)
        self.embed_dropout = nn.Dropout(config.hidden_dropout_prob)
        self.apply(self._init_weights)
        self.gradient_checkpointing = False

    def _init_weights(self, module):
        std = self.config.initializer_range
        if isinstance(module, nn.Linear):
            module.weight.data.normal_(0.0, std)
            if module.bias is not None:
                module.bias.data.zero_()
        elif isinstance(module, nn.Embedding):
            module.weight.data.normal_(0.0, std)
            if module.padding_idx is not None:
                module.weight.data[module.padding_idx].zero_()
        elif isinstance(module, nn.LayerNorm):
            if module.bias is not None:
                module.bias.data.zero_()
            if module.weight is not None:
                module.weight.data.fill_(1.0)
        elif isinstance(module, RMSNorm):
            module.scale.data.fill_(1.0)
        elif isinstance(module, AdaptiveExpertSystem) and module.router is not None:
            module.init_expert_weights(std)
        if isinstance(module, SelectiveLinearAttention):
            nn.init.uniform_(module.dt_proj_head.bias, a=math.log(1e-3), b=math.log(1e-2))

    def gradient_checkpointing_enable(self):
        self.gradient_checkpointing = True

    def get_input_embeddings(self):
        return self.token_embeddings

    def set_input_embeddings(self, embs):
        self.token_embeddings = embs

    def resize_token_embeddings(self, new_num_tokens: int) -> nn.Embedding:
        old = self.token_embeddings
        new = nn.Embedding(new_num_tokens, self.config.hidden_size, self.padding_idx, device=old.weight.device,
                           dtype=old.weight.dtype)
        self._init_weights(new)
        n = min(old.num_embeddings, new_num_tokens)
        new.weight.data[:n] = old.weight.data[:n]
        self.token_embeddings = new
        self.config.vocab_size = self.vocab_size = new_num_tokens
        if self.padding_idx is not None and self.padding_idx >= new_num_tokens:
            self.padding_idx = 0
            self.token_embeddings.padding_idx = 0
        return self.token_embeddings

    def _prepare_decoder_attention_mask(self, attention_mask, input_shape, inputs_embeds, past_len):
        if attention_mask is None or bool(torch.all(attention_mask.bool())):
            return None
        B, Lq = input_shape
        allow = None
        if Lq > 1:
            Lk = past_len + Lq
            causal = torch.ones(Lk, Lk, dtype=torch.bool, device=inputs_embeds.device).tril()[past_len:]
            allow = causal[None, None] & attention_mask[:, None, None, :].bool()
        elif past_len > 0:
            allow = attention_mask[:, None, None, :].bool()
        if allow is None:
            return None
        return (1.0 - allow.to(inputs_embeds.dtype)) * torch.finfo(inputs_embeds.dtype).min

    def _attention_mask(self, attention_mask, input_shape, inputs_embeds, past_len, default_pos, pos_host=None, step_cache=None):
        if step_cache is not None:
            return _AttnMask(None, False, False, None, True, None, step_cache)
        default_pos = default_pos and past_len == 0
        if attention_mask is None:
            return _AttnMask(None, True, default_pos, None, True, pos_host)
        valid = attention_mask.bool()
        all_valid, col0 = torch.stack((valid.all(), valid[:, 0].all())).tolist()
        if all_valid:
            return _AttnMask(None, True, default_pos, None, True, pos_host)
        return _AttnMask(attention_mask, bool(col0) and past_len == 0, default_pos,
                         lambda: self._prepare_decoder_attention_mask(attention_mask, input_shape, inputs_embeds, past_len),
                         bool(col0), pos_host)

    @_on_input_device
    def forward(self, input_ids=None, attention_mask=None, position_ids=None, past_key_values=None,
                inputs_embeds=None, pixel_values=None, use_cache=None, output_attentions=None,
                output_hidden_states=None, return_dict=None):
        cfg = self.config
        use_c = cfg.use_cache if use_cache is None else use_cache
# ... 677 lines not shown
```

apertis_llm_amd/ops/__init__.py:

```python
import sys as _sys
import types as _types

from . import _base, prep, gemm, norm, ssm, scan, decode, moe, loss, attention, sample

_MODULES = (_base, prep, gemm, norm, ssm, scan, decode, moe, loss, attention, sample)
_FORWARDED = {
    "SCAN_SINGLE_PASS": scan, "SCAN_LEAN": scan, "SCAN_LEAN_BWD": scan, "SCAN_LOOKBACK": scan, "SCAN_DT_FUSED": scan,
    "SCAN_LOOKBACK_MIN_WGS": scan,
    "DWCONV_PAIR": ssm,
    "FUSE_ACT_BWD": moe, "SAVE_ACT_GRAD": moe, "ROWS_GRADIENT": moe, "NT2I": moe,
    "FUSE_ROUTER_BOUNDARY_BWD": norm, "FUSED_ROUTER_BWD_CALLS": norm, "FUSE_COMBINE_BWD": norm,
    "GEMM_DYNAMIC_QUEUE": gemm, "TN_DYNAMIC_QUEUE": gemm, "DENSE_WGRAD_WIDE": gemm, "_splitk_depth": gemm,
    "TRAIN_PREP": prep, "WEIGHT_EPOCH": prep, "_ACTIVE_TRAIN_PREP": prep, "_prep_scope_depth": prep,
    "_TIMER": _base,
    "ATTN_FUSED": attention, "ATTN_DECODE_FUSED": attention, "ATTN_DECODE_GRAPH": attention,
    "SAMPLE_FUSED": sample, "SAMPLE_UNIFORMS": sample,
}
for _m in _MODULES:
    for _k, _v in vars(_m).items():
        if _k.startswith("__") or _k in _FORWARDED or isinstance(_v, _types.ModuleType):
            continue
        globals()[_k] = _v
from .._lib import ApertisHipError, check, dtype_code, ptr, stream_ptr


class _OpsPackage(_types.ModuleType):
    def __getattr__(self, name):
        owner = _FORWARDED.get(name)
        if owner is not None:
            return getattr(owner, name)
        raise AttributeError(f"module {self.__name__!r} has no attribute {name!r}")

    def __setattr__(self, name, value):
        owner = _FORWARDED.get(name)
        if owner is not None:
            setattr(owner, name, value)
        else:
            super().__setattr__(name, value)

    def __dir__(self):
        return sorted(set(super().__dir__()) | set(_FORWARDED))


_sys.modules[__name__].__class__ = _OpsPackage
```

apertis_llm_amd/ops/gemm.py:

```python
import os as _os

import torch

from .. import _lib
from .._lib import ApertisHipError, check, dtype_code, ptr, stream_ptr
from ._base import _apply, _f32, _grad_wanted, _launch, _require_gpu, _rows, _slot_of
from .prep import cast_transpose


class _SkinnyLinear(torch.autograd.Function):
    @staticmethod
    def forward(ctx, x, weight, bias):
        _require_gpu(x, weight, bias)
        lib = _lib.load()
        x = x.contiguous()
        T, K = x.shape
        N = weight.shape[0]
        w = _f32(weight)
        b = None if bias is None else _f32(bias)
        y = torch.empty(T, N, device=x.device, dtype=torch.float32)
        check(lib.apertis_skinny_linear_fwd(ptr(x), ptr(w), ptr(b), ptr(y), T, K, N, dtype_code(x), stream_ptr()),
              "apertis_skinny_linear_fwd")
        ctx.save_for_backward(x, w)
        ctx.cfg = (weight.dtype, None if bias is None else bias.dtype)
# ... 18 lines not shown

class _TinyLinear(torch.autograd.Function):
    @staticmethod
    def forward(ctx, x, weight, bias):
        _require_gpu(x, weight, bias)
        lib = _lib.load()
        K, N = x.shape[-1], weight.shape[0]
        ctx.slot = _slot_of(x)
        x3 = x if x.dim() == 3 else x.reshape(1, -1, K)
        xr, ldx = _rows(x3, K)
        T = x.numel() // K
        w = _f32(weight)
        b = None if bias is None else _f32(bias)
        y = torch.empty(*x.shape[:-1], N, device=x.device, dtype=torch.float32)
        check(lib.apertis_tiny_linear_fwd(ptr(xr), ldx, ptr(w), ptr(b), ptr(y), T, K, N, dtype_code(xr), stream_ptr()),
              "apertis_tiny_linear_fwd")
        ctx.save_for_backward(xr, w)
        ctx.cfg = (ldx, T, tuple(x.shape), weight.dtype, None if bias is None else bias.dtype)
        return y

    @staticmethod
    def backward(ctx, dy):
        lib = _lib.load()
        xr, w = ctx.saved_tensors
        ldx, T, xshape, wdt, bdt = ctx.cfg
        N, K = w.shape
        dy = dy.float().contiguous()
        if ctx.slot is not None and ctx.slot[0].widths[ctx.slot[1]] == K:
            dx, Kp = ctx.slot[0].out(ctx.slot[1], xshape[:-1], xr.dtype, xr.device)
            dxp = dx
        else:
            Kp = -(-K // 8) * 8
            dxp = torch.empty(*xshape[:-1], Kp, device=xr.device, dtype=xr.dtype)
            dx = dxp[..., :K]
        nblk = lib.apertis_tiny_linear_bwd_blocks(T)
        part = torch.empty(nblk, N * K + N, device=xr.device, dtype=torch.float32)
        out = torch.empty(N * K + N, device=xr.device, dtype=torch.float32)
        check(lib.apertis_tiny_linear_bwd(ptr(xr), ldx, ptr(w), ptr(dy), ptr(dxp), Kp, ptr(part), ptr(out), T, K, N,
                                          dtype_code(xr), stream_ptr()), "apertis_tiny_linear_bwd")
        return dx, out[:N * K].reshape(N, K).to(wdt), (out[N * K:].to(bdt) if bdt is not None else None)


def tiny_linear_supported(x, K, N):
    return x.is_cuda and x.dtype in (torch.float32, torch.bfloat16) and 1 <= K <= 64 and 1 <= N <= 16


def tiny_linear(x, weight, bias=None):
    return _TinyLinear.apply(x, weight, bias)


def skinny_linear_supported(K, N):
    return N in (2, 4, 8, 16) and K % 4 == 0 and K <= 1024 and (N <= 8 or K <= 256)


def skinny_linear(x, weight, bias=None):
    return _SkinnyLinear.apply(x, weight, bias)


_SPLITK_ROWS = 1024


_splitk_cache = {}


DENSE_WGRAD_WIDE = _os.environ.get("APERTIS_DENSE_WGRAD_WIDE", "1") == "1"


def _splitk_depth(N, K):
    tiles = -(-N // 128) * -(-K // 128)
    return _SPLITK_ROWS if tiles <= 8 else 2 * _SPLITK_ROWS


def _splitk_offsets(rows, G, depth, device):
    key = (rows, G, depth, str(device))
    t = _splitk_cache.get(key)
    if t is None:
        t = torch.tensor([min(i * depth, rows) for i in range(G + 1)], dtype=torch.int32, device=device)
        _splitk_cache[key] = t
    return t


_dense_offsets_cache = {}


def _dense_offsets(rows, device):
    key = (rows, str(device))
    t = _dense_offsets_cache.get(key)
    if t is None:
        t = torch.tensor([0, rows], dtype=torch.int32, device=device)
        _dense_offsets_cache[key] = t
    return t


class _RowsWork:
    __slots__ = ("offsets", "E", "per_row")

    def __init__(self, offsets, E, per_row):
        self.offsets, self.E, self.per_row = offsets, E, per_row

    def __call__(self):
        return float(self.offsets[self.E].item()) * self.per_row


GEMM_DYNAMIC_QUEUE = False


TN_DYNAMIC_QUEUE = _os.environ.get("APERTIS_TN_QUEUE", "0") == "1"


_NT_QUEUE = {}


def _nt_queue(device):
    key = (device, torch.cuda.current_stream(device).cuda_stream)
    q = _NT_QUEUE.get(key)
    if q is None:
        q = _NT_QUEUE[key] = torch.zeros(512, device=device, dtype=torch.int32)
    return q


def _launch_nt(name, lib, args, work, device, detail=None, nbytes=0.0):
    if GEMM_DYNAMIC_QUEUE:
        _launch(name, lib.apertis_grouped_gemm_nt_q, args[:-1] + (ptr(_nt_queue(device)), args[-1]), work, detail, nbytes)
    else:
        _launch(name, lib.apertis_grouped_gemm_nt, args, work, detail, nbytes)


_ACTS = {None: _lib.ACT_NONE, "none": _lib.ACT_NONE, "gelu": _lib.ACT_GELU, "relu": _lib.ACT_RELU,
         "silu": _lib.ACT_SILU, "swish": _lib.ACT_SILU}


_TN_WS = {}


def _tn_workspace(E, n_problems, device, max_rows=None):
    if max_rows is not None and max_rows // max(E, 1) < 2048:
        return None, 0
    nbytes = _lib.load().apertis_grouped_gemm_tn_workspace_bytes(E, n_problems)
    if nbytes <= 0:
        return None, 0
    key = (device, torch.cuda.current_stream(device).cuda_stream)
    buf = _TN_WS.get(key)
    if buf is None or buf.numel() < nbytes:
        buf = _TN_WS[key] = torch.empty(nbytes, device=device, dtype=torch.uint8)
    return buf, nbytes


def _dense_tag(E, rows, N, K, esize):
    if E != 1:
        return None, 0.0
    return f"rows={rows} N={N} K={K}", float(rows) * (N + K) * esize + float(N) * K * esize


class _GroupedLinear(torch.autograd.Function):
    @staticmethod
    def forward(ctx, x, weight, bias, offsets, max_rows, act, drop_p, seed, compute_dtype):
        _require_gpu(x, weight, bias, offsets)
        lib = _lib.load()
        E, N, K = weight.shape
        if x.dtype != compute_dtype:
            x = x.to(compute_dtype)
        x = x.contiguous()
        if x.shape[1] != K:
            raise ApertisHipError(f"grouped_linear: x {tuple(x.shape)} vs weight {tuple(weight.shape)}")
        need_grad = _grad_wanted(ctx, 3)
        if compute_dtype == torch.float32 and weight.dtype == torch.float32 and weight.is_contiguous():
            wc = weight.detach()
            wt = cast_transpose(weight, compute_dtype, want_plain=False)[1] if need_grad else None
        else:
            wc, wt = cast_transpose(weight, compute_dtype, want_transposed=need_grad, cache=not need_grad)
        bf = None if bias is None else _f32(bias)
        code = dtype_code(x)
        act_code = _ACTS[act]
        out = torch.empty(x.shape[0], N, device=x.device, dtype=compute_dtype)
        pre = torch.empty_like(out) if (act_code != _lib.ACT_NONE and need_grad) else None
        _launch_nt("apertis_grouped_gemm_nt" if E > 1 else "apertis_grouped_gemm_nt[dense]", lib,
                (ptr(x), ptr(wc), ptr(bf), ptr(offsets), ptr(out), ptr(pre), None, max_rows, N, K, wc.shape[-1], E, act_code,
                 float(drop_p), int(seed), code, code, stream_ptr()), _RowsWork(offsets, E, 2.0 * N * K), x.device,
                *_dense_tag(E, max_rows, N, K, x.element_size()))
        ctx.save_for_backward(x, wt, pre, offsets)
        ctx.cfg = (E, N, K, max_rows, act_code, float(drop_p), int(seed), bias is not None, weight.dtype)
        return out

    @staticmethod
    def backward(ctx, dout):
        lib = _lib.load()
        x, wt, pre, offsets = ctx.saved_tensors
        E, N, K, max_rows, act_code, drop_p, seed, has_bias, wdtype = ctx.cfg
        code = dtype_code(x)
        dout = dout.to(x.dtype).contiguous()
        if act_code != _lib.ACT_NONE:
            dpre = torch.empty_like(dout)
            check(lib.apertis_act_dropout_bwd(ptr(dout), ptr(pre), ptr(dpre), ptr(offsets), max_rows, N, E, act_code,
                                              drop_p, seed, code, stream_ptr()), "apertis_act_dropout_bwd")
        else:
            dpre = dout
        dx = dw = db = None
        if ctx.needs_input_grad[0]:
            dx = torch.empty_like(x)
            _launch_nt("apertis_grouped_gemm_nt" if E > 1 else "apertis_grouped_gemm_nt[dense]", lib,
                    (ptr(dpre), ptr(wt), None, ptr(offsets), ptr(dx), None, None, max_rows, K, N, wt.shape[-1], E, _lib.ACT_NONE,
                     0.0, 0, code, code, stream_ptr()), _RowsWork(offsets, E, 2.0 * N * K), dpre.device,
                    *_dense_tag(E, max_rows, K, N, x.element_size()))
        if ctx.needs_input_grad[1] or ctx.needs_input_grad[2]:
            if (E == 1 and max_rows >= 4 * _SPLITK_ROWS and DENSE_WGRAD_WIDE and x.dtype == torch.bfloat16 and not has_bias
                    and lib.apertis_grouped_gemm_tn_dense_variant(N, K) >= 0):
                dw = torch.empty(1, N, K, device=x.device, dtype=torch.float32)
                ws, ws_bytes = _tn_workspace(1, 1, x.device, max_rows)
                _launch("apertis_grouped_gemm_tn[dense]", lib.apertis_grouped_gemm_tn,
                        (ptr(dpre), ptr(x), ptr(offsets), ptr(dw), None, max_rows, N, K, 1, ptr(ws), ws_bytes, code, stream_ptr()),
                        2.0 * max_rows * N * K, f"rows={max_rows} M={N} N={K}", float(max_rows) * (N + K) * x.element_size())
                db = None
            elif E == 1 and max_rows >= 4 * _SPLITK_ROWS:
                depth = _splitk_depth(N, K)
                G = -(-max_rows // depth)
                soffs = _splitk_offsets(max_rows, G, depth, x.device)
                part = torch.empty(G, N, K, device=x.device, dtype=torch.float32)
                bpart = torch.empty(G, N, device=x.device, dtype=torch.float32) if has_bias else None
                _launch("apertis_grouped_gemm_tn[dense]", lib.apertis_grouped_gemm_tn,
                        (ptr(dpre), ptr(x), ptr(soffs), ptr(part), ptr(bpart), max_rows, N, K, G, None, 0, code, stream_ptr()),
                        2.0 * max_rows * N * K, f"rows={max_rows} M={N} N={K}",
                        float(max_rows) * (N + K) * x.element_size() + 4.0 * G * N * K)
                dw = torch.empty(1, N, K, device=x.device, dtype=torch.float32)
                check(lib.apertis_colsum_f32(ptr(part), ptr(dw), G, N * K, stream_ptr()), "apertis_colsum_f32")
                db = None
                if has_bias:
                    db = torch.empty(1, N, device=x.device, dtype=torch.float32)
                    check(lib.apertis_colsum_f32(ptr(bpart), ptr(db), G, N, stream_ptr()), "apertis_colsum_f32")
            else:
                dw = torch.empty(E, N, K, device=x.device, dtype=torch.float32)
                db = torch.empty(E, N, device=x.device, dtype=torch.float32) if has_bias else None
                ws, ws_bytes = _tn_workspace(E, 1, x.device, max_rows)
                _launch("apertis_grouped_gemm_tn" if E > 1 else "apertis_grouped_gemm_tn[dense]", lib.apertis_grouped_gemm_tn_q,
                        (ptr(dpre), ptr(x), ptr(offsets), ptr(dw), ptr(db), max_rows, N, K, E, ptr(ws), ws_bytes, code,
                         int(GEMM_DYNAMIC_QUEUE and TN_DYNAMIC_QUEUE), stream_ptr()), _RowsWork(offsets, E, 2.0 * N * K))
            dw = dw.to(wdtype)
        return dx, dw, db, None, None, None, None, None, None


def grouped_linear(x, weight, bias, offsets, max_rows, act=None, drop_p=0.0, seed=0, compute_dtype=None):
    return _apply(_GroupedLinear, x, weight, bias, offsets, max_rows, act, drop_p, seed, compute_dtype or x.dtype)


class _ScatterRows(torch.autograd.Function):
    @staticmethod
    def forward(ctx, w, dst_idx, rows_out):
        out = w.new_zeros(rows_out, *w.shape[1:])
        out.index_copy_(0, dst_idx, w.detach())
        ctx.save_for_backward(dst_idx)
        return out

    @staticmethod
    def backward(ctx, g):
        (dst_idx,) = ctx.saved_tensors
        return g.index_select(0, dst_idx), None, None


def scatter_rows(w, dst_idx, rows_out):
    return _ScatterRows.apply(w, dst_idx, rows_out)


def dense_offsets(rows, device):
    return _dense_offsets(rows, device)


def linear_mfma(x, weight, bias=None, act=None, compute_dtype=None):
    lead = x.shape[:-1]
    x2 = x.reshape(-1, x.shape[-1])
    M = x2.shape[0]
    offsets = _dense_offsets(M, x.device)
    out = grouped_linear(x2, weight.unsqueeze(0), None if bias is None else bias.unsqueeze(0), offsets, M, act, 0.0, 0,
                         compute_dtype or x.dtype)
    return out.reshape(*lead, weight.shape[0])
```

apertis_llm_amd/ops/norm.py:

```python
import os as _os

import torch

from .. import _lib
from .._lib import check, dtype_code, ptr, stream_ptr
from ._base import _RowsGrad, _f32, _require_gpu


class _RouterLN(torch.autograd.Function):

    @staticmethod
    def forward(ctx, x, ln_w, ln_b, eps, weight, bias):
        _require_gpu(x, ln_w, ln_b, weight, bias)
        lib = _lib.load()
        x = x.contiguous()
        T, H = x.shape
        N = weight.shape[0]
        g, be = _f32(ln_w), _f32(ln_b)
        w = _f32(weight)
        b = None if bias is None else _f32(bias)
        logits = torch.empty(T, N, device=x.device, dtype=torch.float32)
        mean = torch.empty(T, device=x.device, dtype=torch.float32)
        rstd = torch.empty(T, device=x.device, dtype=torch.float32)
        check(lib.apertis_router_fwd(ptr(x), ptr(g), ptr(be), float(eps), ptr(w), ptr(b), ptr(logits), ptr(mean), ptr(rstd),
                                     T, H, N, dtype_code(x), stream_ptr()), "apertis_router_fwd")
        ctx.save_for_backward(x, g, be, mean, rstd, w)
        ctx.cfg = (ln_w.dtype, ln_b.dtype, weight.dtype, None if bias is None else bias.dtype)
        ctx.link = _RowsGrad()
        return logits, x.view_as(x), ctx.link

    @staticmethod
    def backward(ctx, dlogits, dpass, _dlink=None):
        lib = _lib.load()
        x, g, be, mean, rstd, w = ctx.saved_tensors
        T, H = x.shape
        N = w.shape[0]
        rows, slot_of, KS = ctx.link.take()
        if dpass is not None and rows is not None and dpass.stride() == (0,) * dpass.dim():
            dpass = None
        if dlogits is None:
            if rows is not None:
                dense = torch.empty_like(x)
                check(lib.apertis_moe_combine_fwd(ptr(rows), ptr(slot_of), None, ptr(dense), T, H, KS, 0, dtype_code(rows),
                                                  dtype_code(dense), stream_ptr()), "apertis_moe_combine_fwd(scatter)")
                dpass = dense if dpass is None else dpass + dense
            return dpass, None, None, None, None, None
        dlogits = dlogits.float().contiguous()
        if dpass is not None:
            dpass = dpass.to(x.dtype).contiguous()
        dx = torch.empty_like(x)
        nblk = lib.apertis_router_bwd_blocks(T)
        cols = N * H + N + 2 * H
        part = torch.empty(nblk, cols, device=x.device, dtype=torch.float32)
        out = torch.empty(cols, device=x.device, dtype=torch.float32)
        check(lib.apertis_router_bwd_rows(ptr(x), ptr(g), ptr(be), ptr(mean), ptr(rstd), ptr(w), ptr(dlogits), ptr(dpass),
                                          ptr(rows), ptr(slot_of), KS, ptr(dx), ptr(part), ptr(out), T, H, N, dtype_code(x),
                                          stream_ptr()), "apertis_router_bwd_rows")
        gdt, bedt, wdt, bdt = ctx.cfg
        dW, db = out[:N * H].reshape(N, H), out[N * H:N * H + N]
        dg, dbe = out[N * H + N:N * H + N + H], out[N * H + N + H:]
        return dx, dg.to(gdt), dbe.to(bedt), None, dW.to(wdt), (db.to(bdt) if bdt is not None else None)


def router_ln_linear_supported(x, H, N):
    return x.is_cuda and x.dtype in (torch.float32, torch.bfloat16) and N in (2, 4, 8) and H % 4 == 0 and H <= 1024


def router_ln_linear(x, ln_weight, ln_bias, eps, weight, bias=None):
    logits, xp, link = _RouterLN.apply(x, ln_weight, ln_bias, eps, weight, bias)
    xp._apertis_rows_link = link
    return logits, xp


class _LayerNorm(torch.autograd.Function):
    @staticmethod
    def forward(ctx, x, weight, bias, eps, out_dtype):
        _require_gpu(x, weight, bias)
        lib = _lib.load()
        shape = x.shape
        H = shape[-1]
        x2 = x.reshape(-1, H).contiguous()
        T = x2.shape[0]
        g = _f32(weight)
        b = _f32(bias)
        y = torch.empty(T, H, device=x.device, dtype=out_dtype)
        mean = torch.empty(T, device=x.device, dtype=torch.float32)
        rstd = torch.empty(T, device=x.device, dtype=torch.float32)
        check(lib.apertis_layernorm_fwd(ptr(x2), ptr(g), ptr(b), float(eps), ptr(y), ptr(mean), ptr(rstd), T, H,
                                        dtype_code(x2), dtype_code(y), stream_ptr()), "apertis_layernorm_fwd")
        ctx.save_for_backward(x2, g, mean, rstd)
        ctx.shape = shape
        ctx.pdtypes = (weight.dtype, bias.dtype)
        return y.reshape(shape)

    @staticmethod
    def backward(ctx, dy, dres=None):
        lib = _lib.load()
        x2, g, mean, rstd = ctx.saved_tensors
        T, H = x2.shape
        if dy is None:
            return dres, None, None, None, None
        dy2 = dy.reshape(T, H).contiguous()
        if dres is not None:
            dres = dres.reshape(T, H).to(x2.dtype).contiguous()
        dx = torch.empty(T, H, device=x2.device, dtype=x2.dtype)
        nw = lib.apertis_layernorm_bwd_blocks(T, H)
        part = torch.empty(nw, 2, H, device=x2.device, dtype=torch.float32)
        dg = torch.empty(H, device=x2.device, dtype=torch.float32)
        db = torch.empty(H, device=x2.device, dtype=torch.float32)
        check(lib.apertis_layernorm_bwd(ptr(x2), ptr(g), ptr(mean), ptr(rstd), ptr(dy2), ptr(dres), ptr(dx), None, 0.0, 0,
                                        ptr(part), ptr(dg), ptr(db), T, H, dtype_code(x2), dtype_code(dy2), stream_ptr()),
              "apertis_layernorm_bwd")
        return dx.reshape(ctx.shape), dg.to(ctx.pdtypes[0]), db.to(ctx.pdtypes[1]), None, None


class _LayerNormPass(_LayerNorm):

    @staticmethod
    def forward(ctx, x, weight, bias, eps, out_dtype):
        y = _LayerNorm.forward(ctx, x, weight, bias, eps, out_dtype)
        return y, x.view_as(x)


class _DropoutAddLN(torch.autograd.Function):

    @staticmethod
    def forward(ctx, blk, res, weight, bias, eps, p, seed, out_dtype, wk=None, plan=None):
        _require_gpu(blk, res, weight, bias)
        lib = _lib.load()
        shape = res.shape
        H = shape[-1]
        blk2 = blk.reshape(-1, H).to(out_dtype).contiguous()
        res2 = res.reshape(-1, H).contiguous()
        T = res2.shape[0]
        wf = None if plan is None else wk.float().contiguous()
        g = _f32(weight)
        b = _f32(bias)
        y = torch.empty_like(res2)
        xn = torch.empty(T, H, device=res.device, dtype=out_dtype)
        mean = torch.empty(T, device=res.device, dtype=torch.float32)
        rstd = torch.empty(T, device=res.device, dtype=torch.float32)
        check(lib.apertis_dropout_add_layernorm_fwd(ptr(blk2), None if plan is None else ptr(plan.slot_of), ptr(wf),
                                                    0 if plan is None else plan.K, ptr(res2), ptr(g), ptr(b), float(eps), ptr(y),
                                                    ptr(xn), ptr(mean), ptr(rstd), T, H, float(p), int(seed), dtype_code(res2),
                                                    dtype_code(xn), stream_ptr()), "apertis_dropout_add_layernorm_fwd")
        if plan is None:
            ctx.save_for_backward(y, g, mean, rstd)
        else:
            ctx.save_for_backward(y, g, mean, rstd, blk2, wf)
        ctx.plan = plan
        ctx.cfg = (shape, float(p), int(seed), weight.dtype, bias.dtype, blk.dtype, out_dtype, tuple(blk.shape))
        return y.reshape(shape), xn.reshape(shape)

    @staticmethod
    def _to_inputs(ctx, dblk):
        lib = _lib.load()
        shape, _p, _seed, _wdt, _bdt, blkdt, _odt, blkshape = ctx.cfg
        plan = ctx.plan
        if plan is None:
            return dblk.reshape(shape).to(blkdt), None
        yr, wf = ctx.saved_tensors[4], ctx.saved_tensors[5]
        H = yr.shape[1]
        dyr = torch.empty_like(yr)
        dw = torch.zeros(plan.S, plan.K, device=yr.device, dtype=torch.float32)
        check(lib.apertis_moe_combine_bwd(ptr(dblk), ptr(yr), ptr(plan.row_token), ptr(plan.row_k), ptr(plan.offsets),
                                          ptr(wf), ptr(dyr), ptr(dw), plan.max_rows, plan.S, H, plan.K, plan.E,
                                          dtype_code(dblk), dtype_code(yr), stream_ptr()), "apertis_moe_combine_bwd")
        return dyr.reshape(blkshape).to(blkdt), dw

    @staticmethod
    def backward(ctx, dy, dxn):
        lib = _lib.load()
        y, g, mean, rstd = ctx.saved_tensors[:4]
        shape, p, seed, wdt, bdt, blkdt, odt, _ = ctx.cfg
        T, H = y.shape
        if dxn is None:
            dy2 = dy.reshape(T, H).contiguous()
            dblk = torch.empty(T, H, device=y.device, dtype=odt)
            check(lib.apertis_dropout_bwd(ptr(dy2), ptr(dblk), dy2.numel(), p, seed, dtype_code(dy2), dtype_code(dblk), stream_ptr()),
                  "apertis_dropout_bwd")
            dblk_in, dwk = _DropoutAddLN._to_inputs(ctx, dblk)
            return dblk_in, dy, None, None, None, None, None, None, dwk, None
        dxn2 = dxn.reshape(T, H).to(odt).contiguous()
        dres = None if dy is None else dy.reshape(T, H).to(y.dtype).contiguous()
        dx = torch.empty_like(y)
        nw = lib.apertis_layernorm_bwd_blocks(T, H)
        part = torch.empty(nw, 2, H, device=y.device, dtype=torch.float32)
        dg = torch.empty(H, device=y.device, dtype=torch.float32)
        db = torch.empty(H, device=y.device, dtype=torch.float32)
        plan = ctx.plan
        if plan is not None and FUSE_COMBINE_BWD and plan.K <= 2:
            yr, wf = ctx.saved_tensors[4], ctx.saved_tensors[5]
            dyr = torch.empty_like(yr)
            dw = torch.zeros(plan.S, plan.K, device=yr.device, dtype=torch.float32)
            rc = lib.apertis_layernorm_combine_bwd(ptr(y), ptr(g), ptr(mean), ptr(rstd), ptr(dxn2), ptr(dres), ptr(dx), p, seed,
                                                   ptr(part), ptr(dg), ptr(db), ptr(plan.slot_of), ptr(wf), ptr(yr), ptr(dyr), ptr(dw),
                                                   T, H, plan.K, dtype_code(y), dtype_code(dxn2), stream_ptr())
            if rc != -2:
                check(rc, "apertis_layernorm_combine_bwd")
                blkdt, blkshape = ctx.cfg[5], ctx.cfg[7]
                return dyr.reshape(blkshape).to(blkdt), dx.reshape(shape), dg.to(wdt), db.to(bdt), None, None, None, None, dw, None
        dblk = torch.empty(T, H, device=y.device, dtype=odt)
        check(lib.apertis_layernorm_bwd(ptr(y), ptr(g), ptr(mean), ptr(rstd), ptr(dxn2), ptr(dres), ptr(dx), ptr(dblk), p, seed,
                                        ptr(part), ptr(dg), ptr(db), T, H, dtype_code(y), dtype_code(dxn2), stream_ptr()),
              "apertis_layernorm_bwd")
        dblk_in, dwk = _DropoutAddLN._to_inputs(ctx, dblk)
        return dblk_in, dx.reshape(shape), dg.to(wdt), db.to(bdt), None, None, None, None, dwk, None


class _DropoutAddLNRouter(torch.autograd.Function):

    @staticmethod
    def forward(ctx, blk, res, weight, bias, eps, p, seed, out_dtype, r_ln_w, r_ln_b, r_eps, r_w, r_b):
        _require_gpu(blk, res, weight, bias, r_ln_w, r_ln_b, r_w, r_b)
        lib = _lib.load()
        shape = res.shape
        H = shape[-1]
        N = r_w.shape[0]
        blk2 = blk.reshape(-1, H).to(out_dtype).contiguous()
        res2 = res.reshape(-1, H).contiguous()
        T = res2.shape[0]
        dev = res.device
        g, b = _f32(weight), _f32(bias)
        rg, rbe = _f32(r_ln_w), _f32(r_ln_b)
        rw = _f32(r_w)
        rbias = None if r_b is None else _f32(r_b)
        y = torch.empty_like(res2)
        xn = torch.empty(T, H, device=dev, dtype=out_dtype)
        mean, rstd = torch.empty(T, device=dev, dtype=torch.float32), torch.empty(T, device=dev, dtype=torch.float32)
        rmean, rrstd = torch.empty(T, device=dev, dtype=torch.float32), torch.empty(T, device=dev, dtype=torch.float32)
        logits = torch.empty(T, N, device=dev, dtype=torch.float32)
        check(lib.apertis_dropout_add_layernorm_router_fwd(ptr(blk2), ptr(res2), ptr(g), ptr(b), float(eps), ptr(y), ptr(xn),
                                                           ptr(mean), ptr(rstd), ptr(rg), ptr(rbe), float(r_eps), ptr(rw),
                                                           ptr(rbias), ptr(logits), ptr(rmean), ptr(rrstd), T, H, N, float(p),
                                                           int(seed), dtype_code(res2), dtype_code(xn), stream_ptr()),
              "apertis_dropout_add_layernorm_router_fwd")
        ctx.save_for_backward(y, g, mean, rstd, xn, rg, rbe, rmean, rrstd, rw)
        ctx.plan = None
        ctx.cfg = (shape, float(p), int(seed), weight.dtype, bias.dtype, blk.dtype, out_dtype, tuple(blk.shape))
        ctx.rcfg = (r_ln_w.dtype, r_ln_b.dtype, r_w.dtype, None if r_b is None else r_b.dtype)
        ctx.link = _RowsGrad()
        ctx.set_materialize_grads(False)
        return y.reshape(shape), xn.reshape(shape), logits, ctx.link

    @staticmethod
    def backward(ctx, dy, dxn, dlogits, _dlink=None):
        lib = _lib.load()
        y, g, mean, rstd, xn, rg, rbe, rmean, rrstd, rw = ctx.saved_tensors
        T, H = y.shape
        N = rw.shape[0]
        rows, slot_of, KS = ctx.link.take()
        if dxn is not None and rows is not None and dxn.stride() == (0,) * dxn.dim():
            dxn = None
        r_grads = (None, None, None, None, None)
        if (dlogits is not None and dxn is None and FUSE_ROUTER_BOUNDARY_BWD and y.dtype == torch.float32 and
                (rows is None or KS <= 2)):
            shape, p, seed, wdt, bdt, blkdt, odt, _ = ctx.cfg
            dres = None if dy is None else dy.reshape(T, H).to(y.dtype).contiguous()
            dx = torch.empty_like(y)
            dblk = torch.empty(T, H, device=y.device, dtype=odt)
            nblk = lib.apertis_router_bwd_blocks(T)
            cols = N * H + N + 2 * H
            part = torch.empty(nblk * (cols + 2 * H), device=y.device, dtype=torch.float32)
            out = torch.empty(cols, device=y.device, dtype=torch.float32)
            dg = torch.empty(H, device=y.device, dtype=torch.float32)
            db = torch.empty(H, device=y.device, dtype=torch.float32)
            rc = lib.apertis_boundary_router_bwd(ptr(y), ptr(g), ptr(mean), ptr(rstd), ptr(dres), ptr(dx), ptr(dblk), p, seed,
                                                 ptr(xn), ptr(rg), ptr(rbe), ptr(rmean), ptr(rrstd), ptr(rw),
                                                 ptr(dlogits.float().contiguous()), ptr(rows), ptr(slot_of), KS or 0, ptr(part),
                                                 ptr(out), ptr(dg), ptr(db), T, H, N, dtype_code(y), dtype_code(xn), stream_ptr())
            if rc != -2:
                check(rc, "apertis_boundary_router_bwd")
                global FUSED_ROUTER_BWD_CALLS
                FUSED_ROUTER_BWD_CALLS += 1
                gdt, bedt, rwdt, rbdt = ctx.rcfg
                r_grads = (out[N * H + N:N * H + N + H].to(gdt), out[N * H + N + H:].to(bedt), None,
                           out[:N * H].reshape(N, H).to(rwdt), (out[N * H:N * H + N].to(rbdt) if rbdt is not None else None))
                dblk_in, _ = _DropoutAddLN._to_inputs(ctx, dblk)
                return (dblk_in, dx.reshape(shape), dg.to(wdt), db.to(bdt), None, None, None, None) + r_grads
        if dlogits is not None:
            dres = None if dxn is None else dxn.reshape(T, H).to(xn.dtype).contiguous()
            dxn_t = torch.empty_like(xn)
            nblk = lib.apertis_router_bwd_blocks(T)
            cols = N * H + N + 2 * H
            part = torch.empty(nblk, cols, device=y.device, dtype=torch.float32)
            out = torch.empty(cols, device=y.device, dtype=torch.float32)
            check(lib.apertis_router_bwd_rows(ptr(xn), ptr(rg), ptr(rbe), ptr(rmean), ptr(rrstd), ptr(rw),
                                              ptr(dlogits.float().contiguous()), ptr(dres), ptr(rows), ptr(slot_of), KS,
                                              ptr(dxn_t), ptr(part), ptr(out), T, H, N, dtype_code(xn), stream_ptr()),
                  "apertis_router_bwd_rows")
            gdt, bedt, wdt, bdt = ctx.rcfg
            r_grads = (out[N * H + N:N * H + N + H].to(gdt), out[N * H + N + H:].to(bedt), None,
                       out[:N * H].reshape(N, H).to(wdt), (out[N * H:N * H + N].to(bdt) if bdt is not None else None))
            dxn = dxn_t
        elif rows is not None:
            dense = torch.empty_like(xn)
            check(lib.apertis_moe_combine_fwd(ptr(rows), ptr(slot_of), None, ptr(dense), T, H, KS, 0, dtype_code(rows),
                                              dtype_code(dense), stream_ptr()), "apertis_moe_combine_fwd(scatter)")
            dxn = dense if dxn is None else dxn.reshape(T, H) + dense
        base = _DropoutAddLN.backward(ctx, dy, dxn)
        return base[:8] + r_grads


def dropout_add_layer_norm_router(blk, residual, weight, bias, eps, p, training, r_ln_w, r_ln_b, r_eps, r_w, r_b, out_dtype=None):
    p = float(p) if training else 0.0
    seed = int(torch.empty((), dtype=torch.int64).random_().item()) if p > 0 else 0
    y, xn, logits, link = _DropoutAddLNRouter.apply(blk, residual, weight, bias, eps, p, seed, out_dtype or residual.dtype,
                                                    r_ln_w, r_ln_b, r_eps, r_w, r_b)
    xn._apertis_rows_link = link
    return y, xn, logits


def dropout_add_layer_norm(blk, residual, weight, bias, eps, p, training, out_dtype=None, combine=None):
    p = float(p) if training else 0.0
    seed = int(torch.empty((), dtype=torch.int64).random_().item()) if p > 0 else 0
    wk, plan = combine if combine is not None else (None, None)
    return _DropoutAddLN.apply(blk, residual, weight, bias, eps, p, seed, out_dtype or residual.dtype, wk, plan)


def layer_norm(x, weight, bias, eps, out_dtype=None):
    return _LayerNorm.apply(x, weight, bias, eps, out_dtype or x.dtype)


def layer_norm_pass(x, weight, bias, eps, out_dtype=None):
    return _LayerNormPass.apply(x, weight, bias, eps, out_dtype or x.dtype)


FUSE_ROUTER_BOUNDARY_BWD = not _os.environ.get("APERTIS_NO_FUSE_ROUTER_BWD")
FUSE_COMBINE_BWD = _os.environ.get("APERTIS_FUSE_COMBINE_BWD", "1") == "1"


FUSED_ROUTER_BWD_CALLS = 0
```

include/apertis_hip.h:

```cpp
#ifndef APERTIS_HIP_H
#define APERTIS_HIP_H

#include <stdint.h>

#ifdef __cplusplus
extern "C" {
#endif

#define APERTIS_OK 0
#define APERTIS_ERR_ARG (-1)
#define APERTIS_ERR_UNSUPPORTED (-2)
#define APERTIS_ERR_LAUNCH (-3)

#define APERTIS_F32 0
#define APERTIS_BF16 1

#define APERTIS_ACT_NONE 0
#define APERTIS_ACT_GELU 1
#define APERTIS_ACT_RELU 2
#define APERTIS_ACT_SILU 3
#define APERTIS_ACT_SAVE_GRAD 0x100
#define APERTIS_ACT_MUL_SAVED 0x200
#define APERTIS_ACT_INTERLEAVED 0x400

// ... 85 lines not shown
int apertis_ssm_decode_state(const float *dt_logits, const float *A_log, const void *Bt, int64_t bt_rs, const void *C,
                             int64_t c_rs, const void *xc, const void *z, int64_t z_rs, const float *D, float *state,
                             void *out, int64_t B, int64_t h, int64_t N, int dtype, int delta_softplus, void *stream);
int apertis_ssm_decode_state_dt(const void *dt_in, int64_t dt_rs, const float *W_dt, const float *b_dt, int64_t R,
                                const float *A_log, const void *Bt, int64_t bt_rs, const void *C, int64_t c_rs, const void *xc,
                                const void *z, int64_t z_rs, const float *D, float *state, void *out, int64_t B, int64_t h,
                                int64_t N, int dtype, int delta_softplus, void *stream);

int apertis_dropout_add_fwd(const void *x, const void *res, void *y, int64_t n, float drop_p,
                            uint64_t seed, int dtype_x, int dtype_res, void *stream);
int apertis_dropout_bwd(const void *g, void *dx, int64_t n, float drop_p, uint64_t seed,
                        int dtype_g, int dtype_x, void *stream);

int apertis_dwconv_silu_fwd(const void *x, int64_t x_rs, const float *w, const float *bias,
                            void *out, int64_t out_rs, int64_t B, int64_t L, int64_t Dn,
                            int64_t k, int dtype_io, void *stream);
int apertis_dwconv_silu_bwd(const void *x, int64_t x_rs, const float *w, const float *bias,
                            const void *dout, int64_t dout_rs, void *dx, int64_t dx_rs,
                            float *dw_part ,
                            float *db_part ,
                            float *dw , float *db ,
                            int64_t B, int64_t L, int64_t Dn, int64_t k, int dtype_io,
                            void *stream);
int64_t apertis_dwconv_bwd_blocks(int64_t B, int64_t L, int64_t Dn);
int apertis_dwconv_silu_bwd2(const void *x, int64_t x_rs, const float *w, const float *bias,
                             const void *dout, int64_t dout_rs, const void *dout2, int64_t dout2_rs,
                             void *dx, int64_t dx_rs, float *dw_part, float *db_part, float *dw,
                             float *db, int64_t B, int64_t L, int64_t Dn, int64_t k, int dtype_io,
                             void *stream);

int apertis_moe_gate_topk_fwd(const float *logits, float *gates, int32_t *idx, float *w,
                              int64_t S, int64_t E, int64_t K, void *stream);
int apertis_moe_gate_topk_bwd(const float *gates, const int32_t *idx, const float *dw,
                              const float *dgates, float *dlogits,
                              int64_t S, int64_t E, int64_t K, void *stream);

int apertis_moe_gate_topk_aux_fwd(const float *logits, float *gates, int32_t *idx, float *w,
                                  float *lse, float *part, float *stats, int64_t S, int64_t E,
                                  int64_t K, float lb_coef, float rz_coef, void *stream);
int apertis_moe_gate_topk_aux_bwd(const float *gates, const int32_t *idx, const float *dw,
                                  const float *lse, const float *stats, const float *dlb,
                                  const float *drz, float lb_coef, float rz_coef, float *dlogits,
                                  int64_t S, int64_t E, int64_t K, void *stream);
int apertis_moe_gate_topk_noisy_aux_fwd(const float *logits, const float *w_noise, float alpha,
                                        uint64_t seed, float *gates, int32_t *idx, float *w,
                                        float *lse, float *part, float *stats, int64_t S, int64_t E,
                                        int64_t K, float lb_coef, float rz_coef, void *stream);
int apertis_moe_gate_topk_noisy_aux_bwd(const float *gates, const int32_t *idx, const float *dw,
                                        const float *lse, const float *stats, const float *dlb,
                                        const float *drz, float lb_coef, float rz_coef,
                                        const float *w_noise, float alpha, uint64_t seed,
                                        float *dlogits, float *npart, float *dw_noise, int64_t S,
                                        int64_t E, int64_t K, void *stream);
int64_t apertis_moe_gate_aux_blocks(int64_t S);

int apertis_skinny_linear_fwd(const void *x, const float *W, const float *b, float *y, int64_t T,
                              int64_t K, int64_t N, int dtype_x, void *stream);
int apertis_skinny_linear_bwd(const void *x, const float *W, const float *dy, void *dx,
                              float *part, float *dW_db, int64_t T, int64_t K, int64_t N,
                              int dtype_x, void *stream);
int64_t apertis_skinny_linear_bwd_blocks(int64_t T);

int apertis_router_fwd(const void *x, const float *gamma, const float *beta, float eps,
                       const float *W, const float *b, float *logits, float *mean, float *rstd,
                       int64_t T, int64_t H, int64_t N, int dtype_x, void *stream);
int apertis_router_bwd(const void *x, const float *gamma, const float *beta, const float *mean,
                       const float *rstd, const float *W, const float *dlogits, const void *dres,
                       void *dx, float *part, float *grads, int64_t T, int64_t H, int64_t N,
                       int dtype_x, void *stream);
int apertis_router_bwd_rows(const void *x, const float *gamma, const float *beta, const float *mean,
                            const float *rstd, const float *W, const float *dlogits, const void *dres,
                            const void *grows, const int32_t *slot_of, int64_t KS, void *dx, float *part,
                            float *grads, int64_t T, int64_t H, int64_t N, int dtype_x, void *stream);
int64_t apertis_router_bwd_blocks(int64_t T);
int apertis_boundary_router_bwd(const void *y, const float *gamma, const float *mean, const float *rstd,
                                const void *dres, void *dx, void *dblk, float drop_p, uint64_t seed,
                                const void *xn, const float *rgamma, const float *rbeta, const float *rmean,
                                const float *rrstd, const float *W, const float *dlogits, const void *grows,
                                const int32_t *slot_of, int64_t KS, float *part, float *rgrads, float *dgamma,
                                float *dbeta, int64_t T, int64_t H, int64_t N, int dtype_x, int dtype_g,
                                void *stream);

int apertis_tiny_linear_fwd(const void *x, int64_t ldx, const float *W, const float *b, float *y,
                            int64_t T, int64_t K, int64_t N, int dtype_x, void *stream);
int apertis_tiny_linear_bwd(const void *x, int64_t ldx, const float *W, const float *dy, void *dx,
                            int64_t lddx, float *part, float *dW_db, int64_t T, int64_t K,
                            int64_t N, int dtype_x, void *stream);
int apertis_tiny_linear_bwd_pad(const void *x, int64_t ldx, const float *W, const float *dy, void *dx,
                                int64_t lddx, float *part, float *dW_db, int64_t T, int64_t K,
                                int64_t N, int64_t zero_to, int dtype_x, void *stream);
int64_t apertis_tiny_linear_bwd_blocks(int64_t T);

int apertis_decode_dense_gemv(const void *x, const void *W, int64_t ldw, const float *bias, void *out, int64_t B,
                              int64_t K, int64_t N, void *stream);
int apertis_decode_inproj(const void *blk, const int32_t *slot_of, const float *wk, int64_t KK, const float *res,
                          const float *gamma, const float *beta, float eps, float *y, const void *xn,
                          const void *W, int64_t ldw, void *xz, const float *pre, void *conv_state,
                          int64_t kconv, void *gated, int64_t S, int64_t H, int64_t N, int64_t Dn, void *stream);
int apertis_moe_enter_small(const void *blk, const void *res, const float *gamma, const float *beta,
                            float eps, void *y, void *xn, const float *rgamma, const float *rbeta,
                            float reps, const float *W, const float *rb, float *logits, float *gates,
                            int32_t *idx, float *w, int32_t *expert_offsets, int32_t *row_token,
                            int32_t *row_k, int32_t *slot_of, const float *lgamma, const float *lbeta,
                            float leps, void *xg, float *mean, float *rstd, int64_t S, int64_t H,
                            int64_t E, int64_t K, int dtype_x, int dtype_y, void *stream);
int apertis_moe_route_small(const float *logits, float *gates, int32_t *idx, float *w,
                            int32_t *expert_offsets, int32_t *row_token, int32_t *row_k,
                            int32_t *slot_of, const void *x, const float *gamma, const float *beta,
                            float eps, void *xg, float *mean, float *rstd, int64_t S, int64_t H,
                            int64_t E, int64_t K, int dtype_x, int dtype_xg, void *stream);
int64_t apertis_moe_plan_workspace_bytes(int64_t S, int64_t E, int64_t K);
int apertis_moe_plan(const int32_t *idx, const float *w, const uint8_t *active,
                     int64_t capacity, int32_t *expert_offsets, int32_t *row_token,
                     int32_t *row_k, int32_t *slot_of, void *ws,
                     int64_t S, int64_t E, int64_t K, void *stream);

int apertis_moe_gather_ln_fwd(const void *x, const int32_t *row_token,
                              const int32_t *expert_offsets, const float *gamma,
                              const float *beta, float eps, void *xg, float *mean, float *rstd,
                              int64_t max_rows, int64_t H, int64_t E, int dtype_x, int dtype_out,
                              void *stream);
int apertis_moe_gather_ln_bwd(const void *x, const int32_t *row_token,
                              const int32_t *expert_offsets, const float *gamma,
                              const float *mean, const float *rstd, const void *dxg,
                              void *dxr, float *dgamma, float *dbeta, float *part, int32_t *blk_expert,
                              int64_t max_rows, int64_t H, int64_t E, int dtype_x, int dtype_g,
                              void *stream);
int64_t apertis_moe_gather_ln_bwd_blocks(int64_t max_rows);

int apertis_layernorm_fwd(const void *x, const float *gamma, const float *beta, float eps,
                          void *y, float *mean, float *rstd, int64_t T, int64_t H, int dtype_x,
                          int dtype_y, void *stream);
int apertis_layernorm_bwd(const void *x, const float *gamma, const float *mean,
                          const float *rstd, const void *dy, const void *dres, void *dx,
                          void *dblk, float drop_p, uint64_t seed, float *part,
                          float *dgamma, float *dbeta, int64_t T, int64_t H, int dtype_x,
                          int dtype_g, void *stream);
int apertis_layernorm_combine_bwd(const void *x, const float *gamma, const float *mean, const float *rstd, const void *dy,
                                  const void *dres, void *dx, float drop_p, uint64_t seed, float *part, float *dgamma,
                                  float *dbeta, const int32_t *slot_of, const float *wk, const void *yr, void *dyr, float *dwk,
                                  int64_t T, int64_t H, int64_t K, int dtype_x, int dtype_g, void *stream);
int64_t apertis_layernorm_bwd_blocks(int64_t T, int64_t H);
int apertis_dropout_add_layernorm_fwd(const void *blk, const int32_t *slot_of, const float *wk, int64_t K,
                                      const void *res, const float *gamma,
                                      const float *beta, float eps, void *y, void *xn, float *mean,
                                      float *rstd, int64_t T, int64_t H, float drop_p, uint64_t seed,
                                      int dtype_x, int dtype_y, void *stream);
int apertis_dropout_add_layernorm_router_fwd(const void *blk, const void *res, const float *gamma,
                                             const float *beta, float eps, void *y, void *xn, float *mean,
                                             float *rstd, const float *rgamma, const float *rbeta, float reps,
                                             const float *W, const float *rb, float *logits, float *rmean,
                                             float *rrstd, int64_t T, int64_t H, int64_t N, float drop_p,
                                             uint64_t seed, int dtype_x, int dtype_y, void *stream);

int apertis_moe_combine_fwd(const void *yr, const int32_t *slot_of, const float *wk,
                            void *out, int64_t S, int64_t H, int64_t K, int with_weights,
                            int dtype_yr, int dtype_out, void *stream);
int apertis_moe_combine_bwd(const void *dout, const void *yr, const int32_t *row_token,
                            const int32_t *row_k, const int32_t *expert_offsets,
                            const float *wk, void *dyr, float *dwk, int64_t max_rows,
                            int64_t S, int64_t H, int64_t K, int64_t E, int dtype_dout,
                            int dtype_yr, void *stream);

int apertis_grouped_gemm_nt(const void *A, const void *W, const float *bias,
                            const int32_t *offsets, void *C, void *pre_act,
                            const void *act_bwd_pre,
                            int64_t max_rows, int64_t N, int64_t K, int64_t ldw, int64_t E,
                            int act, float drop_p, uint64_t seed,
                            int dtype, int dtype_out, void *stream);
int apertis_grouped_gemm_nt_saves_grad(int64_t max_rows, int64_t N, int64_t K, int64_t ldw, int64_t E,
                                       int act, int dtype, int dtype_out);
#define APERTIS_NT_QUEUE_INTS 512
int apertis_grouped_gemm_nt_q(const void *A, const void *W, const float *bias,
                              const int32_t *offsets, void *C, void *pre_act,
                              const void *act_bwd_pre,
                              int64_t max_rows, int64_t N, int64_t K, int64_t ldw, int64_t E,
                              int act, float drop_p, uint64_t seed,
                              int dtype, int dtype_out, int32_t *tile_queue, void *stream);
int64_t apertis_grouped_gemm_tn_workspace_bytes(int64_t E, int n_problems);
int apertis_grouped_gemm_tn_dense_variant(int64_t M, int64_t N);
int apertis_grouped_gemm_tn(const void *A, const void *Bm, const int32_t *offsets,
                            float *dW, float *dbias, int64_t max_rows, int64_t M, int64_t N,
                            int64_t E, void *ws, int64_t ws_bytes, int dtype, void *stream);
int apertis_grouped_gemm_tn_pair(const void *A0, const void *B0, float *dW0, float *dbias0,
                                 int64_t M0, int64_t N0, const void *A1, const void *B1,
                                 float *dW1, float *dbias1, int64_t M1, int64_t N1,
                                 const int32_t *offsets, int64_t max_rows, int64_t E,
                                 void *ws, int64_t ws_bytes, int dtype, void *stream);
int apertis_grouped_gemm_tn_q(const void *A, const void *Bm, const int32_t *offsets,
                              float *dW, float *dbias, int64_t max_rows, int64_t M, int64_t N,
                              int64_t E, void *ws, int64_t ws_bytes, int dtype, int item_queue, void *stream);
int apertis_grouped_gemm_tn_pair_q(const void *A0, const void *B0, float *dW0, float *dbias0,
                                   int64_t M0, int64_t N0, const void *A1, const void *B1,
                                   float *dW1, float *dbias1, int64_t M1, int64_t N1,
                                   const int32_t *offsets, int64_t max_rows, int64_t E,
                                   void *ws, int64_t ws_bytes, int dtype, int item_queue, void *stream);
int apertis_cast_transpose(const float *src, void *dst, void *dstT, int64_t E, int64_t R,
                           int64_t C, int64_t ld_dst, int64_t ld_dstT, int dtype_out, void *stream);
int64_t apertis_weight_prep_entry_bytes(void);
int apertis_weight_prep(const void *table, int64_t n_entries, int64_t total_tiles, void *stream);
int apertis_colsum_f32(const float *in, float *out, int64_t rows, int64_t cols, void *stream);
int apertis_act_dropout_bwd(const void *dh, const void *pre_act, void *dpre,
                            const int32_t *offsets, int64_t max_rows, int64_t N, int64_t E,
                            int act, float drop_p, uint64_t seed, int dtype, void *stream);

int apertis_cross_entropy_fwd(const void *logits, const int64_t *labels, float *lse,
                              float *row_loss, int64_t B, int64_t L, int64_t V,
                              int64_t label_stride, int64_t n_pos, int64_t ignore_index, int dtype,
                              void *stream);
int apertis_cross_entropy_bwd(const void *logits, const int64_t *labels, const float *lse,
                              const float *gscale, void *dlogits, int64_t B, int64_t L, int64_t V,
                              int64_t label_stride, int64_t n_pos, int64_t ignore_index, int dtype,
                              void *stream);
int apertis_cross_entropy_fwd_bwd(const void *logits, const int64_t *labels, float *lse, float *row_loss,
                                  const float *gscale, void *dlogits, int64_t B, int64_t L, int64_t V,
                                  int64_t label_stride, int64_t n_pos, int64_t ignore_index, int dtype, void *stream);

typedef struct apertis_opt_tensor {
  float *p, *g, *m, *v;
  int64_t numel;
} apertis_opt_tensor;
int64_t apertis_opt_chunk_elems(void);
int apertis_grad_sumsq(const void *tensors, const int32_t *chunk_tensor, const int32_t *chunk_index,
                       int64_t n_chunks, float *partials, void *stream);
int apertis_clip_coef(const float *partials, int64_t n, float max_norm, float *norm_coef, const int32_t *poison,
                      void *stream);
int apertis_adamw_step(const void *tensors, const int32_t *chunk_tensor, const int32_t *chunk_index,
                       int64_t n_chunks, double lr, double beta1, double beta2, double eps, double weight_decay,
                       int64_t step, const float *norm_coef, void *stream);

int apertis_rope_qk_fwd(const void *q, int64_t q_rs, const void *k, int64_t k_rs, const int64_t *position_ids,
                        int64_t pos_batch_stride, const float *cos_cached, const float *sin_cached, int64_t max_pos,
                        void *q_out, void *k_out, int64_t B, int64_t L, int64_t W, int dtype, void *stream);
int apertis_rope_qk_bwd(const void *dq_out, int64_t dq_rs, const void *dk_out, int64_t dk_rs, const int64_t *position_ids,
                        int64_t pos_batch_stride, const float *cos_cached, const float *sin_cached, int64_t max_pos,
                        void *dq, void *dk, int64_t B, int64_t L, int64_t W, int dtype, void *stream);

int apertis_attention_fwd(const void *q, int64_t q_rs, const void *k, int64_t k_rs, const void *v, int64_t v_rs,
                          const int64_t *key_valid, void *out, int64_t out_rs, float *lse, int64_t B, int64_t L, int64_t H,
                          int64_t D, float dropout_p, uint64_t seed, int dtype, void *stream);
int64_t apertis_attention_bwd_workspace_bytes(int64_t B, int64_t L, int64_t H);
int apertis_attention_bwd(const void *q, int64_t q_rs, const void *k, int64_t k_rs, const void *v, int64_t v_rs,
                          const void *out, int64_t out_rs, const void *dout, int64_t dout_rs, const float *lse,
                          const int64_t *key_valid, float *workspace, void *dq, void *dk, void *dv, int64_t d_rs, int64_t B,
                          int64_t L, int64_t H, int64_t D, float dropout_p, uint64_t seed, int dtype, void *stream);

#define APERTIS_ATTN_DECODE_MAX_SPLITS 64
int apertis_rope_kv_append(const void *q, int64_t q_rs, const void *k, int64_t k_rs, const void *v, int64_t v_rs,
                           const float *cos_cached, const float *sin_cached, int64_t max_pos, int64_t t, void *q_out,
                           int64_t q_out_rs, void *k_cache, int64_t kc_rs, int64_t kc_bs, void *v_cache, int64_t vc_rs,
                           int64_t vc_bs, int64_t cap, int64_t t_cache, int64_t B, int64_t W, int dtype, void *stream);
int64_t apertis_attention_decode_splits(int64_t B, int64_t H, int64_t Lk, int64_t D);
int64_t apertis_attention_decode_workspace_bytes(int64_t B, int64_t H, int64_t D, int64_t splits);
int apertis_attention_decode(const void *q, int64_t q_rs, const void *k_cache, int64_t k_rs, int64_t k_bs, const void *v_cache,
                             int64_t v_rs, int64_t v_bs, int64_t cap, const int64_t *key_valid, int64_t kv_rs, void *out,
                             int64_t out_rs, float *workspace, int64_t B, int64_t Lk, int64_t H, int64_t D, int64_t splits,
                             int dtype, void *stream);
int apertis_rope_kv_append_at(const void *q, int64_t q_rs, const void *k, int64_t k_rs, const void *v, int64_t v_rs,
                              const float *cos_cached, const float *sin_cached, int64_t max_pos, const int64_t *len,
                              int64_t pos_offset, int32_t *err, void *q_out, int64_t q_out_rs, void *k_cache, int64_t kc_rs,
                              int64_t kc_bs, void *v_cache, int64_t vc_rs, int64_t vc_bs, int64_t cap, int64_t B, int64_t W,
                              int dtype, void *stream);
int apertis_attention_decode_at(const void *q, int64_t q_rs, const void *k_cache, int64_t k_rs, int64_t k_bs, const void *v_cache,
                                int64_t v_rs, int64_t v_bs, int64_t cap, const int64_t *len, const int64_t *key_valid,
                                int64_t kv_rs, void *out, int64_t out_rs, float *workspace, int64_t B, int64_t H, int64_t D,
                                int64_t splits, int dtype, void *stream);

int apertis_rope_kv_append_chunk(const void *q, int64_t q_rs, int64_t q_bs, const void *k, int64_t k_rs, int64_t k_bs,
                                 const void *v, int64_t v_rs, int64_t v_bs, const float *cos_cached, const float *sin_cached,
                                 int64_t max_pos, int64_t t0, void *q_out, void *k_cache, int64_t kc_rs, int64_t kc_bs,
                                 void *v_cache, int64_t vc_rs, int64_t vc_bs, int64_t cap, int64_t t_cache0, int64_t B,
                                 int64_t Lq, int64_t W, int dtype, void *stream);
int64_t apertis_attention_chunk_splits(int64_t B, int64_t H, int64_t Lq, int64_t Lk, int64_t D);
int64_t apertis_attention_chunk_workspace_bytes(int64_t B, int64_t H, int64_t Lq, int64_t D, int64_t splits);
int apertis_attention_chunk(const void *q, int64_t q_rs, const void *k_cache, int64_t k_rs, int64_t k_bs, const void *v_cache,
                            int64_t v_rs, int64_t v_bs, int64_t cap, const int64_t *key_valid, int64_t kv_rs, void *out,
                            int64_t out_rs, float *workspace, int64_t B, int64_t Lq, int64_t n, int64_t H, int64_t D,
                            int64_t splits, int dtype, void *stream);

#define APERTIS_SAMPLE_MAX_VOCAB 262144
#define APERTIS_SAMPLE_MAX_ROWS 65535
int apertis_token_counts(const int64_t *tokens, int64_t tok_rs, int64_t B, int64_t L, int64_t V, int32_t *counts, int32_t *err,
                         void *stream);
int apertis_sample_next(const void *logits, int64_t logits_rs, int dtype, int64_t B, int64_t V, int32_t *counts, float penalty,
                        int do_sample, float temperature, int64_t top_k, float top_p, uint64_t seed, const int64_t *step,
                        int64_t step_off, const int64_t *alive_in, int64_t *alive_out, const int64_t *eos, int64_t n_eos,
                        int64_t pad, int64_t *next, const double *uniforms, int64_t u_rs, int64_t u_cols, float *probs_out,
                        float *x_out, double *u_out, int32_t *err, void *stream);

#ifdef __cplusplus
}
#endif
#endif
```

Baseline: 404,800.

## Fuse out-projection GEMM into dropout-add-layernorm-router forward kernel

Adds a persistent HIP kernel that computes the skinny out-projection (gated @ Wo^T) with MFMA into LDS tiles, then applies dropout, the residual add, layernorm and the optional router LN plus logits in the same block. The gated tile for the next iteration and the residual rows are prefetched while the epilogue runs. The model defers the out-projection with a lazy wrapper so the boundary op can take this fused path, and backward reuses the existing LN backward followed by a shared grouped-linear backward. This removes the write and reread of the projection output and one kernel launch, at the cost of a complex kernel that is limited to small H and Dn and uses heavy LDS.

```diff
diff --git a/apertis_llm_amd/_lib.py b/apertis_llm_amd/_lib.py
--- a/apertis_llm_amd/_lib.py
+++ b/apertis_llm_amd/_lib.py
@@ -98,6 +98,9 @@
                                                  _u64, _i32, _i32, _vp]),
     "apertis_dropout_add_layernorm_router_fwd": (_i32, [_vp, _vp, _vp, _vp, _f32, _vp, _vp, _vp, _vp, _vp, _vp, _f32, _vp, _vp, _vp,
                                                         _vp, _vp, _i64, _i64, _i64, _f32, _u64, _i32, _i32, _vp]),
+    "apertis_outproj_dropout_add_layernorm_router_fwd": (_i32, [_vp, _vp, _i64, _vp, _vp, _vp, _f32, _vp, _vp, _vp, _vp, _vp, _vp,
+                                                                _f32, _vp, _vp, _vp, _vp, _vp, _i64, _i64, _i64, _i64, _f32,
+                                                                _u64, _i32, _i32, _vp]),
     "apertis_layernorm_bwd_blocks": (_i64, [_i64, _i64]),
     "apertis_moe_combine_fwd": (_i32, [_vp, _vp, _vp, _vp, _i64, _i64, _i64, _i32, _i32, _i32, _vp]),
     "apertis_moe_combine_bwd": (_i32, [_vp, _vp, _vp, _vp, _vp, _vp, _vp, _vp, _i64, _i64, _i64, _i64, _i64,
diff --git a/apertis_llm_amd/csrc/layernorm.hip b/apertis_llm_amd/csrc/layernorm.hip
--- a/apertis_llm_amd/csrc/layernorm.hip
+++ b/apertis_llm_amd/csrc/layernorm.hip
@@ -687,6 +687,226 @@
 #pragma unroll
     for (int i = 0; i < IT; ++i) { bc[i] = bn[i]; rc[i] = rn[i]; }
   }
+}
+
+constexpr int OPB_WAVES = 16, OPB_NT = 64 * OPB_WAVES, OPB_U = 8;
+typedef __attribute__((ext_vector_type(8))) bf16_t opb_frag;
+typedef __attribute__((ext_vector_type(4))) float opb_acc;
+__host__ __device__ constexpr int opb_tile_rows(int it) { return it <= 3 ? 64 : 32; }
+
+#ifdef APERTIS_BOUNDARY_STAMPS
+__device__ long long g_opb_stamps[4];
+extern "C" int apertis_outproj_boundary_stamps(long long *out) {
+  return hipMemcpyFromSymbol(out, HIP_SYMBOL(g_opb_stamps), sizeof(g_opb_stamps)) == hipSuccess ? APERTIS_OK : APERTIS_ERR_LAUNCH;
+}
+#endif
+
+template <typename TX, int IT, int NN>
+__global__ void __launch_bounds__(OPB_NT)
+outproj_dropadd_ln_router_fwd_k(const bf16_t *__restrict__ gated, const bf16_t *__restrict__ Wo, int ldw, int Dn,
+                                const TX *__restrict__ res, const float *__restrict__ gamma, const float *__restrict__ beta,
+                                float eps, TX *__restrict__ y, bf16_t *__restrict__ xn, float *__restrict__ mean_o,
+                                float *__restrict__ rstd_o, const float *__restrict__ rgamma, const float *__restrict__ rbeta,
+                                float reps, const float *__restrict__ W, const float *__restrict__ rb, float *__restrict__ logits,
+                                float *__restrict__ rmean_o, float *__restrict__ rrstd_o, int64_t T, int H, float drop_p,
+                                uint64_t seed) {
+  typedef bf16_t TO;
+  constexpr int TR = opb_tile_rows(IT), RPW = TR / OPB_WAVES, MT = TR / 16;
+  if constexpr (IT <= 4) __builtin_assume(H > 256 * (IT - 1));
+  extern __shared__ __attribute__((aligned(16))) char smem[];
+  const int Q = H / 4;
+  float4 *sW = reinterpret_cast<float4 *>(smem);
+  float4 *sG = sW + NN * Q, *sB = sG + Q, *sRG = sB + Q, *sRB = sRG + Q;
+  const int nk = (Dn + 31) >> 5;
+  const int gp = nk * 64 + 16;
+  const int ntn = (H + 15) >> 4;
+  const int bp = ntn * 32 + 16;
+  char *sA = smem + (size_t)(NN > 0 ? NN + 4 : 2) * H * sizeof(float);
+  char *sBlk = sA + TR * gp;
+  const int tid = threadIdx.x, lane = tid & 63, wv = __builtin_amdgcn_readfirstlane(tid >> 6);
+  const int frow = lane & 15, fg = lane >> 4;
+  if constexpr (NN > 0)
+    for (int i = tid; i < NN * Q; i += OPB_NT) sW[i] = reinterpret_cast<const float4 *>(W)[i];
+  for (int i = tid; i < Q; i += OPB_NT) {
+    sG[i] = reinterpret_cast<const float4 *>(gamma)[i]; sB[i] = reinterpret_cast<const float4 *>(beta)[i];
+    if constexpr (NN > 0) { sRG[i] = reinterpret_cast<const float4 *>(rgamma)[i]; sRB[i] = reinterpret_cast<const float4 *>(rbeta)[i]; }
+  }
+  const float ks = drop_p > 0.f ? 1.f / (1.f - drop_p) : 1.f;
+  const uint32_t th = (uint32_t)(drop_p * 65536.f);
+  typedef typename raw4<TO>::type rawo_t;
+  typedef typename raw4<TX>::type rawx_t;
+  const int64_t ntiles = (T + TR - 1) / TR;
+
+  const int cpr = nk * 4, nchunk = TR * cpr;
+  uint4 gq[2];
+  auto load_gated = [&](int64_t tile) {
+#pragma unroll
+    for (int j = 0; j < 2; ++j) {
+      const int q = tid + j * OPB_NT;
+      const int row = q / cpr, c = q - row * cpr;
+      const int64_t r = tile * TR + row;
+      gq[j] = make_uint4(0u, 0u, 0u, 0u);
+      if (q < nchunk && r < T && c * 8 < Dn) {
+        typedef __attribute__((ext_vector_type(4))) unsigned u4;
+        const u4 t = __builtin_nontemporal_load(reinterpret_cast<const u4 *>(gated + r * Dn + c * 8));
+        gq[j] = make_uint4(t.x, t.y, t.z, t.w);
+      }
+    }
+  };
+  auto store_gated = [&]() {
+#pragma unroll
+    for (int j = 0; j < 2; ++j) {
+      const int q = tid + j * OPB_NT;
+      const int row = q / cpr, c = q - row * cpr;
+      if (q < nchunk) *reinterpret_cast<uint4 *>(sA + row * gp + c * 16) = gq[j];
+    }
+  };
+  auto load_w1 = [&](int nt, int u) -> opb_frag {
+    const int wrow = nt * 16 + frow, k = u * 32 + fg * 8;
+    const bool ok = wrow < H && k < Dn;
+    const opb_frag t = *reinterpret_cast<const opb_frag *>(Wo + (int64_t)min(wrow, H - 1) * ldw + (k < Dn ? k : 0));
+    const opb_frag zero = {};
+    return ok ? t : zero;
+  };
+  auto fetch_res = [&](rawx_t (&ro)[IT], int64_t r) {
+#pragma unroll
+    for (int i = 0; i < IT; ++i) {
+      const int c = (lane + 64 * i) * 4;
+      ro[i] = (c < H && r < T) ? *reinterpret_cast<const rawx_t *>(res + r * H + c) : rawx_t{};
+    }
+  };
+
+  int64_t tile = blockIdx.x;
+  rawx_t rc[IT], rn[IT];
+  fetch_res(rc, tile * TR + wv);
+  opb_frag a[OPB_U];
+#pragma unroll
+  for (int u = 0; u < OPB_U; ++u) a[u] = load_w1(wv, u);
+  load_gated(tile);
+  store_gated();
+#ifdef APERTIS_BOUNDARY_STAMPS
+  long long st_m = 0, st_r = 0, st_n = 0;
+#endif
+  for (; tile < ntiles; tile += gridDim.x) {
+    __syncthreads();
+#ifdef APERTIS_BOUNDARY_STAMPS
+    const long long t0 = wall_clock64();
+#endif
+    {
+      for (int nt = wv; nt < ntn; nt += OPB_WAVES) {
+        opb_acc acc[MT];
+#pragma unroll
+        for (int m = 0; m < MT; ++m) acc[m] = (opb_acc){0.f, 0.f, 0.f, 0.f};
+        const int ntw = min(nt + OPB_WAVES, ntn - 1);
+#pragma unroll
+        for (int u = 0; u < OPB_U; ++u) {
+          if (u < nk) {
+#pragma unroll
+            for (int m = 0; m < MT; ++m) {
+              const opb_frag b = *reinterpret_cast<const opb_frag *>(sA + (m * 16 + frow) * gp + u * 64 + fg * 16);
+              acc[m] = __builtin_amdgcn_mfma_f32_16x16x32_bf16(a[u], b, acc[m], 0, 0, 0);
+            }
+            a[u] = load_w1(ntw, u);
+          }
+          __builtin_amdgcn_sched_barrier(0);
+        }
+#pragma unroll
+        for (int m = 0; m < MT; ++m) {
+          typedef __attribute__((ext_vector_type(4))) bf16_t bf4;
+          const bf4 o = {(bf16_t)acc[m][0], (bf16_t)acc[m][1], (bf16_t)acc[m][2], (bf16_t)acc[m][3]};
+          *reinterpret_cast<uint2 *>(sBlk + (m * 16 + frow) * bp + (nt * 16 + fg * 4) * 2) = __builtin_bit_cast(uint2, o);
+        }
+      }
+    }
+    __syncthreads();
+#ifdef APERTIS_BOUNDARY_STAMPS
+    const long long t1 = wall_clock64();
+#endif
+    const int64_t tnext = tile + gridDim.x;
+    load_gated(tnext);
+#pragma unroll 1
+    for (int j = 0; j < RPW; ++j) {
+      const int lr = wv + OPB_WAVES * j;
+      const int64_t r = tile * TR + lr;
+      fetch_res(rn, j + 1 < RPW ? r + OPB_WAVES : tnext * TR + wv);
+      if (r < T) {
+        float4 v[IT];
+#pragma unroll
+        for (int i = 0; i < IT; ++i) {
+          const int c = (lane + 64 * i) * 4;
+          if (c < H) {
+            const float4 a = raw_to_f4(*reinterpret_cast<const rawo_t *>(sBlk + lr * bp + c * 2)), rr = raw_to_f4(rc[i]);
+            float e[4] = {a.x, a.y, a.z, a.w};
+            if (drop_p > 0.f) {
+              bool keep[4];
+              drop_keep4(seed, (uint64_t)r * (uint64_t)H + (uint64_t)c, th, keep);
+#pragma unroll
+              for (int jj = 0; jj < 4; ++jj) e[jj] = keep[jj] ? e[jj] * ks : 0.f;
+            }
+            v[i] = make_float4(rr.x + e[0], rr.y + e[1], rr.z + e[2], rr.w + e[3]);
+            store4<TX>(y + r * H + c, v[i]);
+            v[i] = make_float4(to_f32(from_f32<TX>(v[i].x)), to_f32(from_f32<TX>(v[i].y)), to_f32(from_f32<TX>(v[i].z)), to_f32(from_f32<TX>(v[i].w)));
+          } else {
+            v[i] = make_float4(0.f, 0.f, 0.f, 0.f);
+          }
+        }
+        float mean, rstd;
+        row_stats<IT>(v, lane, H, eps, mean, rstd);
+#pragma unroll
+        for (int i = 0; i < IT; ++i) {
+          const int c = (lane + 64 * i) * 4;
+          if (c < H) {
+            const float4 g4 = sG[lane + 64 * i], b4 = sB[lane + 64 * i];
+            const float4 o = make_float4((v[i].x - mean) * rstd * g4.x + b4.x, (v[i].y - mean) * rstd * g4.y + b4.y,
+                                         (v[i].z - mean) * rstd * g4.z + b4.z, (v[i].w - mean) * rstd * g4.w + b4.w);
+            store4<TO>(xn + r * H + c, o);
+            v[i] = make_float4(to_f32(from_f32<TO>(o.x)), to_f32(from_f32<TO>(o.y)), to_f32(from_f32<TO>(o.z)), to_f32(from_f32<TO>(o.w)));
+          }
+        }
+        if (lane == 0) { mean_o[r] = mean; rstd_o[r] = rstd; }
+        if constexpr (NN > 0) {
+          float rmean, rrstd;
+          row_stats<IT>(v, lane, H, reps, rmean, rrstd);
+#pragma unroll
+          for (int i = 0; i < IT; ++i) {
+            const bool in = lane + 64 * i < Q;
+            const float4 g4 = in ? sRG[lane + 64 * i] : make_float4(0, 0, 0, 0), b4 = in ? sRB[lane + 64 * i] : make_float4(0, 0, 0, 0);
+            v[i] = make_float4((v[i].x - rmean) * rrstd * g4.x + b4.x, (v[i].y - rmean) * rrstd * g4.y + b4.y,
+                               (v[i].z - rmean) * rrstd * g4.z + b4.z, (v[i].w - rmean) * rrstd * g4.w + b4.w);
+          }
+          float acc[NN > 0 ? NN : 1];
+#pragma unroll
+          for (int n = 0; n < NN; ++n) {
+            float a = 0.f;
+#pragma unroll
+            for (int i = 0; i < IT; ++i) {
+              const float4 wn = lane + 64 * i < Q ? sW[n * Q + lane + 64 * i] : make_float4(0, 0, 0, 0);
+              a += (v[i].x * wn.x + v[i].y * wn.y) + (v[i].z * wn.z + v[i].w * wn.w);
+            }
+            acc[n] = wave_sum(a);
+          }
+          if (lane < NN) {
+            float o = 0.f;
+#pragma unroll
+            for (int n = 0; n < NN; ++n) if (lane == n) o = acc[n];
+            logits[r * NN + lane] = o + (rb ? rb[lane] : 0.f);
+          }
+          if (lane == 0) { rmean_o[r] = rmean; rrstd_o[r] = rrstd; }
+        }
+      }
+#pragma unroll
+      for (int i = 0; i < IT; ++i) rc[i] = rn[i];
+    }
+    store_gated();
+#pragma unroll
+    for (int u = 0; u < OPB_U; ++u) a[u] = load_w1(wv, u);
+#ifdef APERTIS_BOUNDARY_STAMPS
+    st_m += t1 - t0; st_r += wall_clock64() - t1; ++st_n;
+#endif
+  }
+#ifdef APERTIS_BOUNDARY_STAMPS
+  if (blockIdx.x == 0 && tid == 0) { g_opb_stamps[0] = st_m; g_opb_stamps[1] = st_r; g_opb_stamps[2] = st_n; g_opb_stamps[3] = TR; }
+#endif
 }
 
 typedef float v2f __attribute__((ext_vector_type(2)));
@@ -1704,3 +1924,36 @@
 #undef BR_GO
   return apertis_check_launch();
 }
+
+extern "C" int apertis_outproj_dropout_add_layernorm_router_fwd(const void *gated, const void *w_out, int64_t ldw, const void *res,
+                                                                const float *gamma, const float *beta, float eps, void *y,
+                                                                void *xn, float *mean, float *rstd, const float *rgamma,
+                                                                const float *rbeta, float reps, const float *W, const float *rb,
+                                                                float *logits, float *rmean, float *rrstd, int64_t T, int64_t H,
+                                                                int64_t Dn, int64_t N, float drop_p, uint64_t seed, int dtype_x,
+                                                                int dtype_y, void *stream) {
+  if (!gated || !w_out || !res || !gamma || !beta || !y || !xn || !mean || !rstd || T < 0 || drop_p < 0.f || drop_p >= 1.f)
+    return APERTIS_ERR_ARG;
+  if (N != 0 && (!rgamma || !rbeta || !W || !logits || !rmean || !rrstd)) return APERTIS_ERR_ARG;
+  if (dtype_x != APERTIS_F32 && dtype_x != APERTIS_BF16) return APERTIS_ERR_ARG;
+  if (dtype_y != APERTIS_BF16 || H <= 0 || H % 4 || H > 1024 || Dn < 16 || Dn % 16 || Dn > 32 * OPB_U || ldw < Dn || ldw % 8 ||
+      (N != 0 && N != 2 && N != 4 && N != 8) || (((uintptr_t)gated | (uintptr_t)w_out) & 15))
+    return APERTIS_ERR_UNSUPPORTED;
+  if (T == 0) return APERTIS_OK;
+  hipStream_t st = (hipStream_t)stream;
+  const int TR = opb_tile_rows((int)ceil_div64(H, 256));
+  const size_t aff = (size_t)(N > 0 ? N + 4 : 2) * H * sizeof(float);
+  const size_t per_row = (size_t)ceil_div64(Dn, 32) * 64 + 16 + (size_t)ceil_div64(H, 16) * 32 + 16;
+  const size_t lds = aff + TR * per_row;
+  if (lds > 160 * 1024) return APERTIS_ERR_UNSUPPORTED;
+  static const int ncu = [] {
+    int n = 256, dev_id = 0;
+    if (hipGetDevice(&dev_id) == hipSuccess) hipDeviceGetAttribute(&n, hipDeviceAttributeMultiprocessorCount, dev_id);
+    return n > 0 ? n : 256;
+  }();
+  dim3 grid((unsigned)std::min<int64_t>(ceil_div64(T, TR), ncu)), block(OPB_NT);
+#define OPB_GO(NN_) { launch_lds(outproj_dropadd_ln_router_fwd_k<TA, IT, NN_>, grid, block, lds, st, (const bf16_t *)gated, (const bf16_t *)w_out, (int)ldw, (int)Dn, (const TA *)res, gamma, beta, eps, (TA *)y, (bf16_t *)xn, mean, rstd, rgamma, rbeta, reps, W, rb, logits, rmean, rrstd, T, (int)H, drop_p, seed); }
+  DISPATCH_2T(dtype_x, dtype_y, SKINNY_IT(H, { if (N == 0) OPB_GO(0) else if (N == 2) OPB_GO(2) else if (N == 4) OPB_GO(4) else OPB_GO(8) }));
+#undef OPB_GO
+  return apertis_check_launch();
+}
diff --git a/apertis_llm_amd/model.py b/apertis_llm_amd/model.py
--- a/apertis_llm_amd/model.py
+++ b/apertis_llm_amd/model.py
@@ -166,6 +166,20 @@
         return ops.moe_combine(self.yr, self.w, self.plan, out_dtype=self.dtype).reshape(self.shape)
 
 
+class _LazyLinear:
+    __slots__ = ("x", "weight")
+
+    def __init__(self, x, weight):
+        self.x, self.weight = x, weight
+
+    @property
+    def shape(self):
+        return (*self.x.shape[:-1], self.weight.shape[0])
+
+    def materialise(self):
+        return _mfma_linear(self.x, self.weight)
+
+
 class _StackedPast(list):
 
     def __init__(self, conv_all, state_all, heads, d_state):
@@ -187,7 +201,7 @@
         self.out, self.res, self.drop = out, res, drop
 
     def resolve(self):
-        out = self.out.materialise() if isinstance(self.out, _LazyCombine) else self.out
+        out = self.out.materialise() if isinstance(self.out, (_LazyCombine, _LazyLinear)) else self.out
         return _dropout_add(self.drop, out, self.res)
 
 
@@ -197,11 +211,23 @@
         H = res.shape[-1]
         cd = _compute_dtype(res)
         lazy = out if isinstance(out, _LazyCombine) else None
+        lin = out if isinstance(out, _LazyLinear) else None
         if (isinstance(norm, HipLayerNorm) and res.is_cuda and tuple(out.shape) == tuple(res.shape) and H % 4 == 0 and
                 H <= 4096 and res.dtype in (torch.float32, torch.bfloat16) and
                 (res.dtype == torch.float32 or cd == res.dtype) and (lazy is None or lazy.dtype == lazy.yr.dtype == cd)):
-            if (router is not None and lazy is None and isinstance(router[0], nn.LayerNorm) and H <= 1024 and
-                    router[1].weight.shape[0] in (2, 4, 8) and cd in (torch.float32, torch.bfloat16)):
+            with_router = (router is not None and lazy is None and isinstance(router[0], nn.LayerNorm) and H <= 1024 and
+                           router[1].weight.shape[0] in (2, 4, 8) and cd in (torch.float32, torch.bfloat16))
+            if lin is not None:
+                nr = router[1].weight.shape[0] if with_router else 0
+                if ops.out_proj_boundary_supported(lin.x, lin.weight, res, nr, cd):
+                    rt = (router[0].weight, router[0].bias, router[0].eps, router[1].weight, router[1].bias) if with_router else None
+                    y, xn, logits = ops.out_proj_dropout_add_layer_norm(lin.x, lin.weight, res, norm.weight, norm.bias, norm.eps,
+                                                                        h.drop.p, h.drop.training, router=rt, out_dtype=cd)
+                    if with_router:
+                        xn._apertis_router_logits = logits
+                    return xn, y
+                out = lin.materialise()
+            if with_router:
                 rn, rl = router
                 y, xn, logits = ops.dropout_add_layer_norm_router(out, res, norm.weight, norm.bias, norm.eps, h.drop.p,
                                                                   h.drop.training, rn.weight, rn.bias, rn.eps, rl.weight,
@@ -328,6 +354,11 @@
         zr = w.new_zeros(Wr - R, Dn)
         return torch.cat([w[R:R + Dn], zb, w[R + Dn:], zb, w[:R], zr], dim=0), Wb, Wr
 
+    def _out_proj(self, gated, lazy_out):
+        if lazy_out and ops.FUSE_OUT_PROJ and gated.is_cuda and self.out_proj.bias is None:
+            return _LazyLinear(gated, self.out_proj.weight)
+        return _mfma_linear(gated, self.out_proj.weight)
+
     def _stacked_in_proj(self):
         w_xz = ops.prepared_weight(("in_proj_xz", id(self)), (self.in_proj_x.weight, self.in_proj_z.weight))
         if w_xz is None:
@@ -345,7 +376,7 @@
 
     @_on_input_device
     def forward(self, hidden_states, attention_mask=None, position_ids=None, past_key_value=None,
-                output_attentions: bool = False, use_cache: bool = False):
+                output_attentions: bool = False, use_cache: bool = False, lazy_out: bool = False):
         self.use_cache = use_cache
         B, L, _ = hidden_states.shape
         Dn, R, kw = self.d_inner, self.dt_rank, self.conv_kernel_size
@@ -411,7 +442,7 @@
             res = ops.scan_gate_dt(dt_in, self.dt_proj_head.weight, self.dt_proj_head.bias, self.A_log, Btp, Cp, xc, z, self.D,
                                    h0=h0, delta_softplus=True, return_last=use_cache)
             (gated, h_last), y = (res if use_cache else (res, None)), None
-            out = _mfma_linear(gated, self.out_proj.weight)
+            out = self._out_proj(gated, lazy_out)
             cache = (conv_state, h_last.reshape(B, self.num_heads, self.d_state)) if use_cache else None
             return out, None, cache
         if tiny:
@@ -427,7 +458,7 @@
             res = ops.scan_gate(dt_logits, self.A_log, Btp, Cp, xc, z, self.D, h0=h0, delta_softplus=True,
                                 return_last=use_cache)
             (gated, h_last), y = (res if use_cache else (res, None)), None
-        out = _mfma_linear(gated, self.out_proj.weight)
+        out = self._out_proj(gated, lazy_out)
         cache = (conv_state, h_last.reshape(B, self.num_heads, self.d_state)) if use_cache else None
         return out, (y if output_attentions else None), cache
 
@@ -640,6 +671,8 @@
         if (impl._decode_pre is None or not isinstance(h, _Pending) or past_kv is None or not use_c or output_att
                 or not isinstance(self.pre_norm, HipLayerNorm) or torch.is_grad_enabled() or self.training):
             return None
+        if isinstance(h.out, _LazyLinear):
+            h.out = h.out.materialise()
         out, res = h.out, h.res
         if res.shape[1] != 1 or not res.is_cuda:
             return None
@@ -745,7 +778,7 @@
         elif self._ssm:
             out, proxy, cache = self.attention_mechanism_impl(x, attention_mask=att_mask, position_ids=pos_ids,
                                                               past_key_value=past_kv, output_attentions=output_att,
-                                                              use_cache=use_c)
+                                                              use_cache=use_c, lazy_out=defer)
         elif self._decode_ok(q := self.q_proj(x), att_mask, past_kv, output_att, use_c):
             out, cache = self._decode_attention(q, self.k_proj(x), self.v_proj(x), att_mask, past_kv)
             proxy = None
@@ -863,8 +896,13 @@
 def _ffn_small_entry(self, h, defer):
     f = self.ffn
     if not (isinstance(h, _Pending) and not isinstance(h.out, _LazyCombine) and not self.training and not f.training
-            and isinstance(self.pre_norm, HipLayerNorm) and isinstance(f.router_norm, nn.LayerNorm)
-            and h.res.is_cuda and _compute_dtype(h.res) == h.out.dtype
+            and isinstance(self.pre_norm, HipLayerNorm) and isinstance(f.router_norm, nn.LayerNorm) and h.res.is_cuda):
+        return None
+    if isinstance(h.out, _LazyLinear):
+        if torch.is_grad_enabled() or h.res.numel() // h.res.shape[-1] > 16:
+            return None
+        h.out = h.out.materialise()
+    if not (_compute_dtype(h.res) == h.out.dtype
             and ops.moe_enter_small_supported(h.out, h.res, f.num_experts, f.experts_per_token)):
         return None
     B, L, H = h.res.shape
diff --git a/apertis_llm_amd/ops/__init__.py b/apertis_llm_amd/ops/__init__.py
--- a/apertis_llm_amd/ops/__init__.py
+++ b/apertis_llm_amd/ops/__init__.py
@@ -9,7 +9,7 @@
     "SCAN_LOOKBACK_MIN_WGS": scan,
     "DWCONV_PAIR": ssm,
     "FUSE_ACT_BWD": moe, "SAVE_ACT_GRAD": moe, "ROWS_GRADIENT": moe, "NT2I": moe,
-    "FUSE_ROUTER_BOUNDARY_BWD": norm, "FUSED_ROUTER_BWD_CALLS": norm, "FUSE_COMBINE_BWD": norm,
+    "FUSE_ROUTER_BOUNDARY_BWD": norm, "FUSED_ROUTER_BWD_CALLS": norm, "FUSE_COMBINE_BWD": norm, "FUSE_OUT_PROJ": norm, "FUSED_OUT_PROJ_CALLS": norm,
     "GEMM_DYNAMIC_QUEUE": gemm, "TN_DYNAMIC_QUEUE": gemm, "DENSE_WGRAD_WIDE": gemm, "_splitk_depth": gemm,
     "TRAIN_PREP": prep, "WEIGHT_EPOCH": prep, "_ACTIVE_TRAIN_PREP": prep, "_prep_scope_depth": prep,
     "_TIMER": _base,
diff --git a/apertis_llm_amd/ops/gemm.py b/apertis_llm_amd/ops/gemm.py
--- a/apertis_llm_amd/ops/gemm.py
+++ b/apertis_llm_amd/ops/gemm.py
@@ -194,6 +194,66 @@
     return f"rows={rows} N={N} K={K}", float(rows) * (N + K) * esize + float(N) * K * esize
 
 
+def _weight_copies(weight, compute_dtype, need_grad):
+    if compute_dtype == torch.float32 and weight.dtype == torch.float32 and weight.is_contiguous():
+        return weight.detach(), (cast_transpose(weight, compute_dtype, want_plain=False)[1] if need_grad else None)
+    return cast_transpose(weight, compute_dtype, want_transposed=need_grad, cache=not need_grad)
+
+
+def _grouped_linear_backward(x, wt, pre, offsets, cfg, dout, need_dx, need_dw):
+    lib = _lib.load()
+    E, N, K, max_rows, act_code, drop_p, seed, has_bias, wdtype = cfg
+    code = dtype_code(x)
+    dout = dout.to(x.dtype).contiguous()
+    if act_code != _lib.ACT_NONE:
+        dpre = torch.empty_like(dout)
+        check(lib.apertis_act_dropout_bwd(ptr(dout), ptr(pre), ptr(dpre), ptr(offsets), max_rows, N, E, act_code,
+                                          drop_p, seed, code, stream_ptr()), "apertis_act_dropout_bwd")
+    else:
+        dpre = dout
+    dx = dw = db = None
+    if need_dx:
+        dx = torch.empty_like(x)
+        _launch_nt("apertis_grouped_gemm_nt" if E > 1 else "apertis_grouped_gemm_nt[dense]", lib,
+                (ptr(dpre), ptr(wt), None, ptr(offsets), ptr(dx), None, None, max_rows, K, N, wt.shape[-1], E, _lib.ACT_NONE,
+                 0.0, 0, code, code, stream_ptr()), _RowsWork(offsets, E, 2.0 * N * K), dpre.device,
+                *_dense_tag(E, max_rows, K, N, x.element_size()))
+    if need_dw:
+        if (E == 1 and max_rows >= 4 * _SPLITK_ROWS and DENSE_WGRAD_WIDE and x.dtype == torch.bfloat16 and not has_bias
+                and lib.apertis_grouped_gemm_tn_dense_variant(N, K) >= 0):
+            dw = torch.empty(1, N, K, device=x.device, dtype=torch.float32)
+            ws, ws_bytes = _tn_workspace(1, 1, x.device, max_rows)
+            _launch("apertis_grouped_gemm_tn[dense]", lib.apertis_grouped_gemm_tn,
+                    (ptr(dpre), ptr(x), ptr(offsets), ptr(dw), None, max_rows, N, K, 1, ptr(ws), ws_bytes, code, stream_ptr()),
+                    2.0 * max_rows * N * K, f"rows={max_rows} M={N} N={K}", float(max_rows) * (N + K) * x.element_size())
+            db = None
+        elif E == 1 and max_rows >= 4 * _SPLITK_ROWS:
+            depth = _splitk_depth(N, K)
+            G = -(-max_rows // depth)
+            soffs = _splitk_offsets(max_rows, G, depth, x.device)
+            part = torch.empty(G, N, K, device=x.device, dtype=torch.float32)
+            bpart = torch.empty(G, N, device=x.device, dtype=torch.float32) if has_bias else None
+            _launch("apertis_grouped_gemm_tn[dense]", lib.apertis_grouped_gemm_tn,
+                    (ptr(dpre), ptr(x), ptr(soffs), ptr(part), ptr(bpart), max_rows, N, K, G, None, 0, code, stream_ptr()),
+                    2.0 * max_rows * N * K, f"rows={max_rows} M={N} N={K}",
+                    float(max_rows) * (N + K) * x.element_size() + 4.0 * G * N * K)
+            dw = torch.empty(1, N, K, device=x.device, dtype=torch.float32)
+            check(lib.apertis_colsum_f32(ptr(part), ptr(dw), G, N * K, stream_ptr()), "apertis_colsum_f32")
+            db = None
+            if has_bias:
+                db = torch.empty(1, N, device=x.device, dtype=torch.float32)
+                check(lib.apertis_colsum_f32(ptr(bpart), ptr(db), G, N, stream_ptr()), "apertis_colsum_f32")
+        else:
+            dw = torch.empty(E, N, K, device=x.device, dtype=torch.float32)
+            db = torch.empty(E, N, device=x.device, dtype=torch.float32) if has_bias else None
+            ws, ws_bytes = _tn_workspace(E, 1, x.device, max_rows)
+            _launch("apertis_grouped_gemm_tn" if E > 1 else "apertis_grouped_gemm_tn[dense]", lib.apertis_grouped_gemm_tn_q,
+                    (ptr(dpre), ptr(x), ptr(offsets), ptr(dw), ptr(db), max_rows, N, K, E, ptr(ws), ws_bytes, code,
+                     int(GEMM_DYNAMIC_QUEUE and TN_DYNAMIC_QUEUE), stream_ptr()), _RowsWork(offsets, E, 2.0 * N * K))
+        dw = dw.to(wdtype)
+    return dx, dw, db
+
+
 class _GroupedLinear(torch.autograd.Function):
     @staticmethod
     def forward(ctx, x, weight, bias, offsets, max_rows, act, drop_p, seed, compute_dtype):
@@ -206,11 +266,7 @@
         if x.shape[1] != K:
             raise ApertisHipError(f"grouped_linear: x {tuple(x.shape)} vs weight {tuple(weight.shape)}")
         need_grad = _grad_wanted(ctx, 3)
-        if compute_dtype == torch.float32 and weight.dtype == torch.float32 and weight.is_contiguous():
-            wc = weight.detach()
-            wt = cast_transpose(weight, compute_dtype, want_plain=False)[1] if need_grad else None
-        else:
-            wc, wt = cast_transpose(weight, compute_dtype, want_transposed=need_grad, cache=not need_grad)
+        wc, wt = _weight_copies(weight, compute_dtype, need_grad)
         bf = None if bias is None else _f32(bias)
         code = dtype_code(x)
         act_code = _ACTS[act]
@@ -226,57 +282,9 @@
 
     @staticmethod
     def backward(ctx, dout):
-        lib = _lib.load()
         x, wt, pre, offsets = ctx.saved_tensors
-        E, N, K, max_rows, act_code, drop_p, seed, has_bias, wdtype = ctx.cfg
-        code = dtype_code(x)
-        dout = dout.to(x.dtype).contiguous()
-        if act_code != _lib.ACT_NONE:
-            dpre = torch.empty_like(dout)
-            check(lib.apertis_act_dropout_bwd(ptr(dout), ptr(pre), ptr(dpre), ptr(offsets), max_rows, N, E, act_code,
-                                              drop_p, seed, code, stream_ptr()), "apertis_act_dropout_bwd")
-        else:
-            dpre = dout
-        dx = dw = db = None
-        if ctx.needs_input_grad[0]:
-            dx = torch.empty_like(x)
-            _launch_nt("apertis_grouped_gemm_nt" if E > 1 else "apertis_grouped_gemm_nt[dense]", lib,
-                    (ptr(dpre), ptr(wt), None, ptr(offsets), ptr(dx), None, None, max_rows, K, N, wt.shape[-1], E, _lib.ACT_NONE,
-                     0.0, 0, code, code, stream_ptr()), _RowsWork(offsets, E, 2.0 * N * K), dpre.device,
-                    *_dense_tag(E, max_rows, K, N, x.element_size()))
-        if ctx.needs_input_grad[1] or ctx.needs_input_grad[2]:
-            if (E == 1 and max_rows >= 4 * _SPLITK_ROWS and DENSE_WGRAD_WIDE and x.dtype == torch.bfloat16 and not has_bias
-                    and lib.apertis_grouped_gemm_tn_dense_variant(N, K) >= 0):
-                dw = torch.empty(1, N, K, device=x.device, dtype=torch.float32)
-                ws, ws_bytes = _tn_workspace(1, 1, x.device, max_rows)
-                _launch("apertis_grouped_gemm_tn[dense]", lib.apertis_grouped_gemm_tn,
-                        (ptr(dpre), ptr(x), ptr(offsets), ptr(dw), None, max_rows, N, K, 1, ptr(ws), ws_bytes, code, stream_ptr()),
-                        2.0 * max_rows * N * K, f"rows={max_rows} M={N} N={K}", float(max_rows) * (N + K) * x.element_size())
-                db = None
-            elif E == 1 and max_rows >= 4 * _SPLITK_ROWS:
-                depth = _splitk_depth(N, K)
-                G = -(-max_rows // depth)
-                soffs = _splitk_offsets(max_rows, G, depth, x.device)
-                part = torch.empty(G, N, K, device=x.device, dtype=torch.float32)
-                bpart = torch.empty(G, N, device=x.device, dtype=torch.float32) if has_bias else None
-                _launch("apertis_grouped_gemm_tn[dense]", lib.apertis_grouped_gemm_tn,
-                        (ptr(dpre), ptr(x), ptr(soffs), ptr(part), ptr(bpart), max_rows, N, K, G, None, 0, code, stream_ptr()),
-                        2.0 * max_rows * N * K, f"rows={max_rows} M={N} N={K}",
-                        float(max_rows) * (N + K) * x.element_size() + 4.0 * G * N * K)
-                dw = torch.empty(1, N, K, device=x.device, dtype=torch.float32)
-                check(lib.apertis_colsum_f32(ptr(part), ptr(dw), G, N * K, stream_ptr()), "apertis_colsum_f32")
-                db = None
-                if has_bias:
-                    db = torch.empty(1, N, device=x.device, dtype=torch.float32)
-                    check(lib.apertis_colsum_f32(ptr(bpart), ptr(db), G, N, stream_ptr()), "apertis_colsum_f32")
-            else:
-                dw = torch.empty(E, N, K, device=x.device, dtype=torch.float32)
-                db = torch.empty(E, N, device=x.device, dtype=torch.float32) if has_bias else None
-                ws, ws_bytes = _tn_workspace(E, 1, x.device, max_rows)
-                _launch("apertis_grouped_gemm_tn" if E > 1 else "apertis_grouped_gemm_tn[dense]", lib.apertis_grouped_gemm_tn_q,
-                        (ptr(dpre), ptr(x), ptr(offsets), ptr(dw), ptr(db), max_rows, N, K, E, ptr(ws), ws_bytes, code,
-                         int(GEMM_DYNAMIC_QUEUE and TN_DYNAMIC_QUEUE), stream_ptr()), _RowsWork(offsets, E, 2.0 * N * K))
-            dw = dw.to(wdtype)
+        dx, dw, db = _grouped_linear_backward(x, wt, pre, offsets, ctx.cfg, dout, ctx.needs_input_grad[0],
+                                              ctx.needs_input_grad[1] or ctx.needs_input_grad[2])
         return dx, dw, db, None, None, None, None, None, None
 
 
diff --git a/apertis_llm_amd/ops/norm.py b/apertis_llm_amd/ops/norm.py
--- a/apertis_llm_amd/ops/norm.py
+++ b/apertis_llm_amd/ops/norm.py
@@ -4,7 +4,8 @@
 
 from .. import _lib
 from .._lib import check, dtype_code, ptr, stream_ptr
-from ._base import _RowsGrad, _f32, _require_gpu
+from ._base import _RowsGrad, _apply, _f32, _grad_wanted, _require_gpu
+from .gemm import _dense_offsets, _grouped_linear_backward, _weight_copies
 
 
 class _RouterLN(torch.autograd.Function):
@@ -246,7 +247,7 @@
     @staticmethod
     def backward(ctx, dy, dxn, dlogits, _dlink=None):
         lib = _lib.load()
-        y, g, mean, rstd, xn, rg, rbe, rmean, rrstd, rw = ctx.saved_tensors
+        y, g, mean, rstd, xn, rg, rbe, rmean, rrstd, rw = ctx.saved_tensors[:10]
         T, H = y.shape
         N = rw.shape[0]
         rows, slot_of, KS = ctx.link.take()
@@ -302,6 +303,84 @@
         return base[:8] + r_grads
 
 
+class _OutProjDropoutAddLN(torch.autograd.Function):
+
+    @staticmethod
+    def forward(ctx, gated, w3, res, weight, bias, eps, p, seed, out_dtype, r_ln_w, r_ln_b, r_eps, r_w, r_b):
+        _require_gpu(gated, w3, res, weight, bias, r_ln_w, r_ln_b, r_w, r_b)
+        lib = _lib.load()
+        shape = res.shape
+        H = shape[-1]
+        Dn = w3.shape[2]
+        N = 0 if r_w is None else r_w.shape[0]
+        x = gated.reshape(-1, Dn).to(out_dtype).contiguous()
+        res2 = res.reshape(-1, H).contiguous()
+        T = res2.shape[0]
+        dev = res.device
+        wc, wt = _weight_copies(w3, out_dtype, _grad_wanted(ctx, 2))
+        g, b = _f32(weight), _f32(bias)
+        y = torch.empty_like(res2)
+        xn = torch.empty(T, H, device=dev, dtype=out_dtype)
+        mean, rstd = torch.empty(T, device=dev, dtype=torch.float32), torch.empty(T, device=dev, dtype=torch.float32)
+        rg = rbe = rw = rbias = rmean = rrstd = logits = None
+        if N:
+            rg, rbe, rw = _f32(r_ln_w), _f32(r_ln_b), _f32(r_w)
+            rbias = None if r_b is None else _f32(r_b)
+            rmean, rrstd = torch.empty(T, device=dev, dtype=torch.float32), torch.empty(T, device=dev, dtype=torch.float32)
+            logits = torch.empty(T, N, device=dev, dtype=torch.float32)
+        check(lib.apertis_outproj_dropout_add_layernorm_router_fwd(
+            ptr(x), ptr(wc), wc.shape[-1], ptr(res2), ptr(g), ptr(b), float(eps), ptr(y), ptr(xn), ptr(mean), ptr(rstd), ptr(rg),
+            ptr(rbe), float(r_eps or 0.0), ptr(rw), ptr(rbias), ptr(logits), ptr(rmean), ptr(rrstd), T, H, Dn, N, float(p),
+            int(seed), dtype_code(res2), dtype_code(xn), stream_ptr()), "apertis_outproj_dropout_add_layernorm_router_fwd")
+        global FUSED_OUT_PROJ_CALLS
+        FUSED_OUT_PROJ_CALLS += 1
+        lin = (x, wt, _dense_offsets(T, dev))
+        if N:
+            ctx.save_for_backward(y, g, mean, rstd, xn, rg, rbe, rmean, rrstd, rw, *lin)
+            ctx.rcfg = (r_ln_w.dtype, r_ln_b.dtype, r_w.dtype, None if r_b is None else r_b.dtype)
+            ctx.link = _RowsGrad()
+        else:
+            ctx.save_for_backward(y, g, mean, rstd, *lin)
+        ctx.plan = None
+        ctx.cfg = (shape, float(p), int(seed), weight.dtype, bias.dtype, out_dtype, out_dtype, tuple(shape))
+        ctx.lin_cfg = (1, H, Dn, T, _lib.ACT_NONE, 0.0, 0, False, w3.dtype)
+        ctx.gcfg = (tuple(gated.shape), gated.dtype)
+        ctx.set_materialize_grads(False)
+        return y.reshape(shape), xn.reshape(shape), logits, (ctx.link if N else None)
+
+    @staticmethod
+    def backward(ctx, dy, dxn, dlogits=None, _dlink=None):
+        if len(ctx.saved_tensors) > 7:
+            base = _DropoutAddLNRouter.backward(ctx, dy, dxn, dlogits)
+        else:
+            base = _DropoutAddLN.backward(ctx, dy, dxn)[:8] + (None,) * 5
+        x, wt, offsets = ctx.saved_tensors[-3:]
+        dgated, dw, _ = _grouped_linear_backward(x, wt, None, offsets, ctx.lin_cfg, base[0].reshape(-1, ctx.lin_cfg[1]),
+                                                 ctx.needs_input_grad[0], ctx.needs_input_grad[1])
+        if dgated is not None:
+            gshape, gdt = ctx.gcfg
+            dgated = dgated.reshape(gshape).to(gdt)
+        return (dgated, dw) + base[1:]
+
+
+def out_proj_boundary_supported(gated, w_out, residual, n_router, out_dtype):
+    H, Dn = w_out.shape
+    return (FUSE_OUT_PROJ and gated.is_cuda and out_dtype == torch.bfloat16 == gated.dtype and H % 4 == 0 and H <= 1024 and
+            Dn % 16 == 0 and 16 <= Dn <= 256 and n_router in (0, 2, 4, 8) and residual.shape[-1] == H and
+            gated.shape[-1] == Dn and residual.dtype in (torch.float32, torch.bfloat16))
+
+
+def out_proj_dropout_add_layer_norm(gated, w_out, residual, weight, bias, eps, p, training, router=None, out_dtype=None):
+    p = float(p) if training else 0.0
+    seed = int(torch.empty((), dtype=torch.int64).random_().item()) if p > 0 else 0
+    r = router if router is not None else (None, None, 0.0, None, None)
+    y, xn, logits, link = _apply(_OutProjDropoutAddLN, gated, w_out.unsqueeze(0), residual, weight, bias, eps, p, seed,
+                                 out_dtype or residual.dtype, *r)
+    if link is not None:
+        xn._apertis_rows_link = link
+    return y, xn, logits
+
+
 def dropout_add_layer_norm_router(blk, residual, weight, bias, eps, p, training, r_ln_w, r_ln_b, r_eps, r_w, r_b, out_dtype=None):
     p = float(p) if training else 0.0
     seed = int(torch.empty((), dtype=torch.int64).random_().item()) if p > 0 else 0
@@ -330,4 +409,8 @@
 FUSE_COMBINE_BWD = _os.environ.get("APERTIS_FUSE_COMBINE_BWD", "1") == "1"
 
 
+FUSE_OUT_PROJ = _os.environ.get("APERTIS_FUSE_OUT_PROJ", "1") == "1"
+
+
+FUSED_OUT_PROJ_CALLS = 0
 FUSED_ROUTER_BWD_CALLS = 0
diff --git a/include/apertis_hip.h b/include/apertis_hip.h
--- a/include/apertis_hip.h
+++ b/include/apertis_hip.h
@@ -261,6 +261,13 @@
                                              const float *W, const float *rb, float *logits, float *rmean,
                                              float *rrstd, int64_t T, int64_t H, int64_t N, float drop_p,
                                              uint64_t seed, int dtype_x, int dtype_y, void *stream);
+int apertis_outproj_dropout_add_layernorm_router_fwd(const void *gated, const void *w_out, int64_t ldw, const void *res,
+                                                     const float *gamma, const float *beta, float eps, void *y, void *xn,
+                                                     float *mean, float *rstd, const float *rgamma, const float *rbeta,
+                                                     float reps, const float *W, const float *rb, float *logits,
+                                                     float *rmean, float *rrstd, int64_t T, int64_t H, int64_t Dn,
+                                                     int64_t N, float drop_p, uint64_t seed, int dtype_x, int dtype_y,
+                                                     void *stream);
 
 int apertis_moe_combine_fwd(const void *yr, const int32_t *slot_of, const float *wk,
                             void *out, int64_t S, int64_t H, int64_t K, int with_weights,
```

Measured after the change: 399,500. 0.987x the previous value.
